# huangwenjie2023/LINR-PCGC

Measured on AMD Instinct MI355X. Metric: encode_sec_per_frame, lower is better.
Workload: dtype f32

## Files before the change

### include/linr_hip.h

```cpp
#ifndef LINR_HIP_H
#define LINR_HIP_H

#include <stddef.h>
#include <stdint.h>

#ifdef __cplusplus
extern "C" {
#endif

#define LINR_ABI_VERSION 13
#define LINR_API __attribute__((visibility("default")))

#define LINR_EINVAL   (-1)
#define LINR_ENOSPC   (-2)
#define LINR_EALIGN   (-3)

#define LINR_RELU      1u
#define LINR_ACCUM     2u
#define LINR_RELU_MASK 4u
#define LINR_NO_BIAS   8u
#define LINR_PAD_ROW  16u

LINR_API int linr_abi_version(void);
LINR_API int64_t linr_param_count(int32_t scale_num, int32_t block_layers);

LINR_API size_t linr_kmap_workspace_bytes(int64_t n);
LINR_API int linr_kmap_build(const int32_t* coords, int64_t n, int32_t* nbr, int64_t ld, int64_t row_base,
                    void* ws, size_t ws_bytes, void* stream);
LINR_API int linr_kmap_compress(const int32_t* nbr, int64_t nbr_ld, int64_t n, int32_t* lo, uint32_t* mask, int64_t ld,
                       void* stream);
LINR_API int linr_kmap_offset_feat(const int32_t* nbr, int64_t ld, int64_t row_base, int64_t n, float* out, void* stream);
LINR_API int linr_octree_occupancy(const int32_t* child, int64_t m, const int32_t* parent, int64_t n, float* occ, void* ws,
                          size_t ws_bytes, void* stream);
LINR_API size_t linr_sort_unique_workspace_bytes(int64_t n);
LINR_API int linr_coords_sort_unique(const int32_t* coords, int64_t n, const int32_t* origin, int32_t shift, int32_t coord_bits, int32_t* out,
                                     int64_t* count, void* ws, size_t ws_bytes, void* stream);
LINR_API int linr_coords_minmax(const int32_t* coords, int64_t n, int32_t* out, void* stream);
LINR_API int linr_octree_level(const int32_t* child, int64_t m, int32_t coord_bits, int32_t* parent, float* occ, int64_t* count, void* ws,
                               size_t ws_bytes, void* stream);
LINR_API int32_t linr_octree_levels_count(int32_t coord_bits, int32_t max_levels);
LINR_API int64_t linr_octree_levels_rows(int64_t m, int32_t coord_bits, int32_t max_levels);
LINR_API size_t linr_octree_levels_workspace_bytes(int64_t m, int32_t coord_bits, int32_t max_levels);
LINR_API int linr_octree_levels(const int32_t* child, int64_t m, const int64_t* m_dev, int32_t coord_bits, int32_t max_levels,
                                int32_t* parents, float* occ, int64_t* counts, void* ws, size_t ws_bytes, void* stream);
LINR_API int linr_kmap_validate(const int32_t* coords, int64_t n, int32_t* bad, void* stream);

LINR_API int linr_spconv_fwd(const float* in, int32_t in_ld, const int32_t* nbr, int64_t nbr_ld, int64_t n,
                    const float* W, const float* bias, int32_t cin, int32_t cout,
                    const float* res, int32_t res_ld, float* out, int32_t out_ld, uint32_t flags, void* stream);
LINR_API int linr_spconv_bwd_data(const float* gout, int32_t gout_ld, const int32_t* nbr, int64_t nbr_ld, int64_t n,
                         const float* W, int32_t cin, int32_t cout,
                         const float* act, int32_t act_ld, float* gin, int32_t gin_ld, uint32_t flags,
                         void* stream);
LINR_API size_t linr_spconv_bwd_weight_workspace_bytes(int64_t n, int32_t cin, int32_t cout);
LINR_API int linr_spconv_bwd_weight(const float* in, int32_t in_ld, const float* gout, int32_t gout_ld,
                           const int32_t* nbr, int64_t nbr_ld, int64_t n, int32_t cin, int32_t cout,
                           float* gW, float* gb, uint32_t flags, void* ws, size_t ws_bytes, void* stream);

LINR_API int linr_spconv_cmap(int32_t bwd, const float* in, int32_t in_ld, const int32_t* lo, const uint32_t* mask,
                     int64_t ld, int64_t n, const float* W, const float* bias, int32_t cin, int32_t cout,
                     const float* res, int32_t res_ld, const float* act, int32_t act_ld, float* out, int32_t out_ld,
                     uint32_t flags, void* stream);
LINR_API int linr_spconv_wide(int32_t bwd, const float* const* in_h, const int32_t* lo, const uint32_t* mask, int64_t ld, int64_t n,
                              const float* W, const float* bias, int32_t cin, int32_t cout, const float* const* res_h,
                              const float* const* act_h, float* const* out_h, uint32_t flags, void* stream);
typedef struct {
    int32_t mode;
    const float* W;
    const float* b;
    const float* const* aux_h;
    float* const* out2_h;
} linr_wide_pw;
LINR_API int linr_spconv_wide_pw(int32_t bwd, const float* const* in_h, const int32_t* lo, const uint32_t* mask, int64_t ld, int64_t n,
                                 const float* W, const float* bias, int32_t cin, int32_t cout, const float* const* res_h,
                                 const float* const* act_h, float* const* out_h, uint32_t flags, const linr_wide_pw* pw, void* stream);
LINR_API size_t linr_spconv_wgrad_wide_slab_bytes(int32_t cin, int32_t cout);
LINR_API int linr_spconv_wgrad_wide(const float* const* in_h, int32_t cin, const float* const* g_h, int32_t cout, const int32_t* nbr,
                                    const int32_t* tile8t, int64_t ld, int64_t n, float* slab, float* gW, float* gb, void* stream);

LINR_API int linr_linear_wide(const float* const* in_h, int32_t cin, int32_t in_blocked, const float* W, int32_t ws_ci, int32_t ws_co,
                              const float* bias, int32_t cout, int32_t out_blocked, const float* const* res_h, const float* const* act_h,
                              float* const* out_h, int64_t n, uint32_t flags, void* stream);
LINR_API size_t linr_linear_wgrad_wide_workspace_bytes(int64_t n, int32_t cin, int32_t cout);
LINR_API int linr_linear_wgrad_wide(const float* const* in_h, int32_t cin, int32_t in_blocked, const float* const* g_h, int32_t cout,
                                    int32_t g_blocked, int64_t n, float* gW, int32_t ws_ci, int32_t ws_co, float* gb, uint32_t flags,
                                    void* ws, size_t ws_bytes, void* stream);

typedef struct {
    int32_t kind, nblocks, cin, cout, ws_ci, ws_co;
    const float* slab;
    float* gW;
    float* gb;
} linr_wide_reduce;
LINR_API int32_t linr_spconv_wgrad_wide_blocks(int32_t cout, int32_t tiled);
LINR_API int linr_spconv_wgrad_wide2(const float* const* inA_h, const float* const* gA_h, const float* const* inB_h, const float* const* gB_h,
                                     int32_t h, const int32_t* tile8t, int64_t n, float* slab, void* stream);
LINR_API int32_t linr_linear_wgrad_wide_blocks(int64_t n);
LINR_API int linr_wide_reduce_many(const linr_wide_reduce* items_h, int32_t count, void* stream);

LINR_API size_t linr_head_wide_workspace_bytes(int64_t n);
LINR_API int linr_bits_finish(const double* partial, int64_t count, double* bits_acc, void* stream);
LINR_API int linr_head_wide_fwd(const float* const* c_h, int32_t C, const float* w1, const float* b1, const float* w2, const float* b2,
                                const float* target, int32_t target_ld, int64_t n, float* p, double* bits_acc, void* ws, size_t ws_bytes,
                                void* stream);
LINR_API size_t linr_head_wide_bwd_slab_bytes(int32_t C, int32_t nstages);
LINR_API int linr_head_wide_bwd(const float* const* c_h, const float* const* p_h, const float* const* target_h, int32_t target_ld,
                                const float* const* w1_h, const float* const* b1_h, const float* const* w2_h, int32_t C, int32_t nstages,
                                float gscale, float* const* gc_h, int64_t n, float* slab, size_t slab_bytes, float* grads, void* stream);

LINR_API int64_t linr_spconv_wgrad_cmap_blocks(void);
LINR_API int linr_spconv_wgrad_cmap(const float* in, int32_t in_ld, const float* gout, int32_t gout_ld, const int32_t* nbr,
                           const int32_t* tile8t, int64_t ld, int64_t n, int32_t cin, int32_t cout, float* slab, void* stream);
LINR_API int linr_slab_reduce(const float* slab, int32_t nblocks, int32_t elems, int32_t split, float* dstA, float* dstB,
                     uint32_t flags, void* stream);
LINR_API size_t linr_kmap_tile8t_bytes(int64_t n);
LINR_API int linr_kmap_tile8t(const int32_t* nbr, int64_t ld, int64_t n, int32_t* tile8t, size_t tile8t_bytes, void* stream);
LINR_API int linr_spconv_bwd_fused(const float* gout, const float* in, const int32_t* lo, const uint32_t* mask, int64_t ld,
                          int64_t n, const float* W, float* gin, float* slab, int32_t nblocks, void* stream);
#define LINR_PROF_KINDS 24
LINR_API int linr_prof_mask(uint32_t mask);
LINR_API int linr_debug_poison(uint32_t kind_mask);
LINR_API int linr_debug_poison_now(void* stream);
LINR_API int linr_prof_enable(int32_t mode);
LINR_API int linr_prof_read(int32_t kind, double* total_ms, int64_t* launches, int64_t* passes);

LINR_API int linr_linear_fwd(const float* in, int32_t in_ld, int64_t n, const float* W, int32_t ws_ci, int32_t ws_co,
                    const float* bias, int32_t cin, int32_t cout, const float* res, int32_t res_ld,
                    float* out, int32_t out_ld, uint32_t flags, void* stream);
LINR_API int linr_linear_bwd_data(const float* gout, int32_t gout_ld, int64_t n, const float* W, int32_t ws_ci,
                         int32_t ws_co, int32_t cin, int32_t cout, const float* act, int32_t act_ld,
                         float* gin, int32_t gin_ld, uint32_t flags, void* stream);
LINR_API size_t linr_linear_bwd_weight_workspace_bytes(int64_t n, int32_t cin, int32_t cout);
LINR_API int linr_linear_bwd_weight(const float* in, int32_t in_ld, const float* gout, int32_t gout_ld, int64_t n,
                           int32_t cin, int32_t cout, float* gW, int32_t ws_ci, int32_t ws_co, float* gb,
                           uint32_t flags, void* ws, size_t ws_bytes, void* stream);
LINR_API int linr_axpy(const float* src, int64_t n, float* dst, int32_t accumulate, void* stream);
LINR_API int linr_sum_many(const float* const* src_h, int32_t count, int64_t n, float* dst, int32_t accumulate, void* stream);

LINR_API size_t linr_bce_workspace_bytes(int64_t n);
LINR_API int linr_bce_bits_fwd(const float* z, const float* target, int32_t target_ld, int64_t n, float* p,
                      double* bits_acc, void* ws, size_t ws_bytes, void* stream);
LINR_API int linr_bce_bits_bwd(const float* p, const float* target, int32_t target_ld, int64_t n, float gscale,
                      float* gz, void* stream);

LINR_API int linr_adam_step(float* params, const float* grads, float* exp_avg, float* exp_avg_sq, int64_t n,
                   double step_size, double bc2_sqrt, double beta1, double beta2, double eps, double weight_decay,
                   void* stream);

#define LINR_FRAME_OCC_PADDED 1
typedef struct linr_frame {
    int64_t rows;
    int32_t n_scales;
    int32_t model_scale_num;
    int32_t block_layers;
    int32_t flags;
    const int64_t* row_off_h;
    const int32_t* scale_idx_h;
    const int32_t* nbr;
    int64_t nbr_ld;
    const int32_t* nbr_lo;
    const uint32_t* nbr_mask;
    const float*   offset_feat;
    const float*   occ;
    const int32_t* nbr8t;
} linr_frame;

LINR_API size_t linr_net_arena_bytes(int64_t rows, int32_t block_layers);
LINR_API int linr_net_forward(const linr_frame* f, const float* params, float* arena, size_t arena_bytes,
                     int32_t stage_begin, int32_t stage_end, float* probs, double* bits_acc, void* stream);
LINR_API int linr_net_backward(const linr_frame* f, const float* params, float* arena, size_t arena_bytes,
                      float gscale, float* grads, void* stream);

LINR_API int linr_net_train_step(const linr_frame* f, float* params, float* arena, size_t arena_bytes, float gscale,
                        float* exp_avg, float* exp_avg_sq, double lr, int64_t step, const int64_t* scale_steps_h,
                        double beta1, double beta2, double eps, double weight_decay, double* bits_acc, void* stream);

LINR_API size_t linr_net_bf16_arena_bytes(int64_t rows, int32_t block_layers);
LINR_API int linr_net_forward_bf16(const linr_frame* f, const uint8_t* codes, float min_param, float max_param, void* arena,
                          size_t arena_bytes, int32_t stage_begin, int32_t stage_end, float* probs, double* bits_acc,
                          void* stream);

LINR_API int64_t linr_wide_bf16_image_elems(int32_t cin, int32_t cout);
LINR_API int linr_wide_bf16_prep(const uint8_t* codes, int64_t n_params, float min_param, float max_param, const int64_t* conv_tab,
                                 int32_t n_conv, int64_t n_img, float* pf, void* img, void* stream);
LINR_API int linr_spconv_wide_bf16(int32_t epi, const uint16_t* in, int64_t in_bs, int32_t cin, const int32_t* lo, const uint32_t* mask,
                                   int64_t ld, int64_t n, const void* img, const float* bias, int32_t cout, const uint16_t* res, int64_t res_bs,
                                   const uint16_t* res2, int64_t res2_bs, const float* pw_w, const float* pw_b, int32_t relu, uint16_t* out,
                                   int64_t out_bs, void* stream);
LINR_API int linr_head_wide_bf16_fwd(const uint16_t* in, int64_t in_bs, int32_t C, const int32_t* lo, const uint32_t* mask, int64_t ld,
                                     int64_t n, const void* img, const float* bias, const float* w1, const float* b1, const float* w2,
                                     const float* b2, const float* target, int32_t t_col, float* p, double* partial, void* stream);
LINR_API int linr_sce_fwd_bf16(const float* pf, const linr_frame* f, uint16_t* x0_padded, void* stream);

LINR_API size_t linr_net_train_bf16_arena_bytes(int64_t rows, int32_t block_layers);
LINR_API int linr_occ_to_bf16(const float* occ, int64_t rows, uint16_t* out_padded, void* stream);
LINR_API int linr_net_forward_train_bf16(const linr_frame* f, const float* params, void* arena, size_t arena_bytes,
                                const uint16_t* occ_bf16, float* probs, double* bits_acc, void* stream);
LINR_API int linr_net_backward_bf16(const linr_frame* f, const float* params, void* arena, size_t arena_bytes,
                           const uint16_t* occ_bf16, float gscale, float* grads, void* stream);
LINR_API int linr_net_train_step_bf16(const linr_frame* f, float* params, void* arena, size_t arena_bytes, const uint16_t* occ_bf16,
                             float gscale, float* exp_avg, float* exp_avg_sq, double lr, int64_t step,
                             const int64_t* scale_steps_h, double beta1, double beta2, double eps, double weight_decay,
                             double* bits_acc, void* stream);
LINR_API int linr_spconv_bwd_fused_bf16(const uint16_t* gout, const uint16_t* in, const int32_t* lo, const uint32_t* mask, int64_t ld,
                               int64_t n, const float* W, uint16_t* gin, float* slab, int32_t nblocks, int32_t* rows_written,
                               void* stream);

LINR_API int linr_net_decode_stages(const linr_frame* f, const float* params, const uint8_t* codes, float min_param,
                           float max_param, void* arena, size_t arena_bytes, const uint8_t* const* streams_h,
                           const int64_t* stream_len_h, float* probs, float* p_pinned, uint8_t* s_pinned, uint8_t* s_dev,
                           void* stream);

LINR_API size_t linr_decode_scale_ws_bytes(int64_t n, int32_t block_layers, int32_t bf16);
LINR_API int linr_decode_scale(const int32_t* coord, int64_t n, int32_t scale_idx, int32_t model_scale_num, int32_t block_layers,
                      int32_t child_bits, const float* params, const uint8_t* codes, float min_param, float max_param,
                      const uint8_t* const* streams_h, const int64_t* stream_len_h, void* ws, size_t ws_bytes,
                      float* p_pinned, uint8_t* s_pinned, int32_t* child_xyz, int64_t child_cap, int64_t* child_n_h,
                      void* stream);

LINR_API int linr_sce_fwd(const float* params, const linr_frame* f, float* mix, float* hid, float* x0, void* stream);
LINR_API int linr_sce_bwd(const float* params, const linr_frame* f, const float* gx0, const float* hid, float* ghid,
                 void* stream);
LINR_API int64_t linr_sce_param_count(int32_t model_scale_num);
LINR_API size_t linr_sce_bwd_params_slab_bytes(int32_t model_scale_num);
LINR_API int linr_sce_bwd_params(const float* params, const linr_frame* f, const float* gx0, const float* hid, float* slab,
                                 size_t slab_bytes, float* grads, void* stream);

LINR_API size_t linr_head_workspace_bytes(int64_t n);
LINR_API int linr_head_fwd(const float* prior, const int32_t* lo, const uint32_t* mask, int64_t ld, int64_t n,
                  const float* Wp, const float* bp, const float* w1, const float* b1, const float* w2, const float* b2,
                  const float* target, int32_t target_ld, float* c_out, float* p_out, double* bits_acc, void* ws,
                  size_t ws_bytes, void* stream);
LINR_API int linr_head_bwd(const float* c, const float* p, const float* target, int32_t target_ld, const float* w1,
                  const float* b1, const float* w2, float gscale, float* gc, int64_t n, float* ghead, void* ws,
                  size_t ws_bytes, void* stream);

typedef struct linr_inception_params {
    const float *w00, *b00;
    const float *w01, *b01;
    const float *w10, *b10;
    const float *w11, *b11;
    const float *w12, *b12;
} linr_inception_params;
LINR_API int linr_inception_fwd(const float* x, const int32_t* lo, const uint32_t* mask, int64_t ld, int64_t n,
                       const linr_inception_params* q, float* H, float* M, float* I, void* stream);
LINR_API int linr_inception_bwd_data(const float* gI, const float* x, const float* H, const float* M, const int32_t* lo,
                            const uint32_t* mask, int64_t ld, int64_t n, const linr_inception_params* q, float* gM,
                            float* gH, float* gX, uint32_t flags, void* stream);
LINR_API int linr_spconv_wgrad_dual44(const float* H, const float* g0, int32_t g0_ld, const float* g1, int32_t g1_ld,
                             const int32_t* nbr, const int32_t* tile8t, int64_t ld, int64_t n, float* slab, void* stream);

LINR_API int linr_inception_bwd_fused(const float* gI, const float* gM, const float* x, const float* H, const int32_t* lo,
                             const uint32_t* mask, int64_t ld, int64_t n, const linr_inception_params* q, float* gH, float* gX,
                             uint32_t flags, float* slab, int32_t nblocks, void* stream);

LINR_API int linr_occ_wgrad7(const float* occ, const float* const* gout7_h, const int32_t* lo, const uint32_t* mask, int64_t ld,
                    int64_t n, float* slab, int32_t nblocks, int32_t* rows_written_h, void* stream);
LINR_API int linr_occ_conv7(const float* occ, const int32_t* lo, const uint32_t* mask, int64_t ld, int64_t n,
                   const float* params, const int64_t* w_off_h, const int64_t* b_off_h, float* out,
                   const int64_t* out_off_h, void* stream);

LINR_API int64_t linr_ac_encode_binary(const float* prob_h, const uint8_t* sym_h, int64_t n, uint8_t* out_h, int64_t cap);
LINR_API int     linr_ac_decode_binary(const float* prob_h, int64_t n, const uint8_t* in_h, int64_t in_len, uint8_t* sym_h);
LINR_API int64_t linr_ac_encode_cdf16(const uint16_t* cdf_h, int32_t lp, int32_t cdf_shared, const int16_t* sym_h,
                             int64_t n, uint8_t* out_h, int64_t cap);
LINR_API int     linr_ac_decode_cdf16(const uint16_t* cdf_h, int32_t lp, int32_t cdf_shared, int64_t n,
                             const uint8_t* in_h, int64_t in_len, int16_t* sym_h);
LINR_API int linr_ac_encode_binary_batch(const float* const* prob_h, const uint8_t* const* sym_h, const int64_t* n,
                                int32_t n_streams, uint8_t* const* out_h, const int64_t* cap,
                                int64_t* out_len, int32_t n_threads);

LINR_API int linr_ply_parse_ascii(const char* text_h, size_t len, int64_t n_rows, int32_t n_cols, int32_t cx, int32_t cy,
                         int32_t cz, int64_t* xyz_h, int64_t* rows_parsed_h);

#ifdef __cplusplus
}
#endif
#endif
```

### linr_pcgc_amd/_lib.py

```python
import ctypes
import os

import torch

_HERE = os.path.dirname(os.path.abspath(__file__))
LIB_PATH = os.environ.get('LINR_HIP_LIB') or os.path.join(_HERE, 'liblinr_hip.so')

LINR_RELU, LINR_ACCUM, LINR_RELU_MASK, LINR_NO_BIAS, LINR_PAD_ROW = 1, 2, 4, 8, 16
LINR_FRAME_OCC_PADDED = 1
ABI_VERSION = 13

c_i32, c_i64, c_u32, c_f32, c_f64 = ctypes.c_int32, ctypes.c_int64, ctypes.c_uint32, ctypes.c_float, ctypes.c_double
c_ptr, c_size = ctypes.c_void_p, ctypes.c_size_t


class LinrWidePw(ctypes.Structure):
    _fields_ = [('mode', ctypes.c_int32), ('W', ctypes.c_void_p), ('b', ctypes.c_void_p), ('aux_h', ctypes.c_void_p), ('out2_h', ctypes.c_void_p)]


class LinrWideReduce(ctypes.Structure):
    _fields_ = [('kind', ctypes.c_int32), ('nblocks', ctypes.c_int32), ('cin', ctypes.c_int32), ('cout', ctypes.c_int32),
                ('ws_ci', ctypes.c_int32), ('ws_co', ctypes.c_int32), ('slab', ctypes.c_void_p), ('gW', ctypes.c_void_p),
                ('gb', ctypes.c_void_p)]


class LinrFrame(ctypes.Structure):
    _fields_ = [('rows', c_i64), ('n_scales', c_i32), ('model_scale_num', c_i32), ('block_layers', c_i32),
                ('flags', c_i32), ('row_off_h', c_ptr),
                ('scale_idx_h', c_ptr), ('nbr', c_ptr), ('nbr_ld', c_i64), ('nbr_lo', c_ptr), ('nbr_mask', c_ptr),
                ('offset_feat', c_ptr), ('occ', c_ptr), ('nbr8t', c_ptr)]


class LinrInceptionParams(ctypes.Structure):
    _fields_ = [(n, ctypes.c_void_p) for n in ('w00', 'b00', 'w01', 'b01', 'w10', 'b10', 'w11', 'b11', 'w12', 'b12')]


_PROTOS = {
    'linr_abi_version': (ctypes.c_int, []),
    'linr_param_count': (c_i64, [c_i32, c_i32]),
    'linr_kmap_workspace_bytes': (c_size, [c_i64]),
    'linr_kmap_build': (ctypes.c_int, [c_ptr, c_i64, c_ptr, c_i64, c_i64, c_ptr, c_size, c_ptr]),
    'linr_kmap_validate': (ctypes.c_int, [c_ptr, c_i64, c_ptr, c_ptr]),
    'linr_spconv_wgrad_cmap_blocks': (ctypes.c_int64, []),
    'linr_spconv_wgrad_cmap': (ctypes.c_int, [c_ptr, c_i32, c_ptr, c_i32, c_ptr, c_ptr, c_i64, c_i64, c_i32, c_i32, c_ptr, c_ptr]),
    'linr_spconv_bwd_fused': (ctypes.c_int, [c_ptr, c_ptr, c_ptr, c_ptr, c_i64, c_i64, c_ptr, c_ptr, c_ptr, c_i32, c_ptr]),
    'linr_inception_bwd_fused': (ctypes.c_int, [c_ptr, c_ptr, c_ptr, c_ptr, c_ptr, c_ptr, c_i64, c_i64,
                                                ctypes.POINTER(LinrInceptionParams), c_ptr, c_ptr, c_u32, c_ptr, c_i32, c_ptr]),
    'linr_slab_reduce': (ctypes.c_int, [c_ptr, c_i32, c_i32, c_i32, c_ptr, c_ptr, c_u32, c_ptr]),
    'linr_axpy': (ctypes.c_int, [c_ptr, c_i64, c_ptr, c_i32, c_ptr]),
    'linr_sum_many': (ctypes.c_int, [c_ptr, c_i32, c_i64, c_ptr, c_i32, c_ptr]),
    'linr_occ_wgrad7': (ctypes.c_int, [c_ptr, c_ptr, c_ptr, c_ptr, c_i64, c_i64, c_ptr, c_i32, c_ptr, c_ptr]),
    'linr_kmap_tile8t_bytes': (c_size, [c_i64]),
    'linr_kmap_tile8t': (ctypes.c_int, [c_ptr, c_i64, c_i64, c_ptr, c_size, c_ptr]),
    'linr_prof_mask': (ctypes.c_int, [c_u32]),
    'linr_prof_enable': (ctypes.c_int, [c_i32]),
    'linr_debug_poison': (ctypes.c_int, [c_u32]),
    'linr_debug_poison_now': (ctypes.c_int, [c_ptr]),
    'linr_prof_read': (ctypes.c_int, [c_i32, c_ptr, c_ptr, c_ptr]),
    'linr_octree_occupancy': (ctypes.c_int, [c_ptr, c_i64, c_ptr, c_i64, c_ptr, c_ptr, ctypes.c_size_t, c_ptr]),
    'linr_sort_unique_workspace_bytes': (ctypes.c_size_t, [c_i64]),
    'linr_coords_sort_unique': (ctypes.c_int, [c_ptr, c_i64, c_ptr, c_i32, c_i32, c_ptr, c_ptr, c_ptr, ctypes.c_size_t, c_ptr]),
    'linr_coords_minmax': (ctypes.c_int, [c_ptr, c_i64, c_ptr, c_ptr]),
    'linr_octree_level': (ctypes.c_int, [c_ptr, c_i64, c_i32, c_ptr, c_ptr, c_ptr, c_ptr, ctypes.c_size_t, c_ptr]),
    'linr_octree_levels_count': (c_i32, [c_i32, c_i32]),
    'linr_octree_levels_rows': (c_i64, [c_i64, c_i32, c_i32]),
    'linr_octree_levels_workspace_bytes': (ctypes.c_size_t, [c_i64, c_i32, c_i32]),
    'linr_octree_levels': (ctypes.c_int, [c_ptr, c_i64, c_ptr, c_i32, c_i32, c_ptr, c_ptr, c_ptr, c_ptr, ctypes.c_size_t, c_ptr]),
    'linr_kmap_offset_feat': (ctypes.c_int, [c_ptr, c_i64, c_i64, c_i64, c_ptr, c_ptr]),
    'linr_kmap_compress': (ctypes.c_int, [c_ptr, c_i64, c_i64, c_ptr, c_ptr, c_i64, c_ptr]),
    'linr_spconv_fwd': (ctypes.c_int, [c_ptr, c_i32, c_ptr, c_i64, c_i64, c_ptr, c_ptr, c_i32, c_i32, c_ptr, c_i32,
                                       c_ptr, c_i32, c_u32, c_ptr]),
    'linr_spconv_bwd_data': (ctypes.c_int, [c_ptr, c_i32, c_ptr, c_i64, c_i64, c_ptr, c_i32, c_i32, c_ptr, c_i32,
                                            c_ptr, c_i32, c_u32, c_ptr]),
    'linr_spconv_wide': (ctypes.c_int, [c_i32, c_ptr, c_ptr, c_ptr, c_i64, c_i64, c_ptr, c_ptr, c_i32, c_i32, c_ptr, c_ptr, c_ptr, ctypes.c_uint32, c_ptr]),
    'linr_spconv_wgrad_wide_slab_bytes': (ctypes.c_size_t, [c_i32, c_i32]),
    'linr_spconv_wgrad_wide': (ctypes.c_int, [c_ptr, c_i32, c_ptr, c_i32, c_ptr, c_ptr, c_i64, c_i64, c_ptr, c_ptr, c_ptr, c_ptr]),
    'linr_linear_wide': (ctypes.c_int, [c_ptr, ctypes.c_int32, ctypes.c_int32, c_ptr, ctypes.c_int32, ctypes.c_int32, c_ptr, ctypes.c_int32,
                                        ctypes.c_int32, c_ptr, c_ptr, c_ptr, c_i64, ctypes.c_uint32, c_ptr]),
    'linr_spconv_wide_pw': (ctypes.c_int, [c_i32, c_ptr, c_ptr, c_ptr, c_i64, c_i64, c_ptr, c_ptr, c_i32, c_i32, c_ptr, c_ptr, c_ptr, c_u32,
                                           ctypes.POINTER(LinrWidePw), c_ptr]),
    'linr_spconv_wgrad_wide2': (ctypes.c_int, [c_ptr, c_ptr, c_ptr, c_ptr, c_i32, c_ptr, c_i64, c_ptr, c_ptr]),
    'linr_spconv_wgrad_wide_blocks': (ctypes.c_int32, [ctypes.c_int32, ctypes.c_int32]),
    'linr_linear_wgrad_wide_blocks': (ctypes.c_int32, [c_i64]),
    'linr_wide_reduce_many': (ctypes.c_int, [ctypes.POINTER(LinrWideReduce), ctypes.c_int32, c_ptr]),
    'linr_head_wide_workspace_bytes': (ctypes.c_size_t, [c_i64]),
    'linr_bits_finish': (ctypes.c_int, [c_ptr, c_i64, c_ptr, c_ptr]),
    'linr_head_wide_fwd': (ctypes.c_int, [c_ptr, ctypes.c_int32, c_ptr, c_ptr, c_ptr, c_ptr, c_ptr, ctypes.c_int32, c_i64, c_ptr, c_ptr, c_ptr,
                                          ctypes.c_size_t, c_ptr]),
    'linr_head_wide_bwd_slab_bytes': (ctypes.c_size_t, [ctypes.c_int32, ctypes.c_int32]),
    'linr_head_wide_bwd': (ctypes.c_int, [c_ptr, c_ptr, c_ptr, ctypes.c_int32, c_ptr, c_ptr, c_ptr, ctypes.c_int32, ctypes.c_int32,
                                          ctypes.c_float, c_ptr, c_i64, c_ptr, ctypes.c_size_t, c_ptr, c_ptr]),
    'linr_linear_wgrad_wide_workspace_bytes': (ctypes.c_size_t, [c_i64, ctypes.c_int32, ctypes.c_int32]),
    'linr_linear_wgrad_wide': (ctypes.c_int, [c_ptr, ctypes.c_int32, ctypes.c_int32, c_ptr, ctypes.c_int32, ctypes.c_int32, c_i64, c_ptr,
                                              ctypes.c_int32, ctypes.c_int32, c_ptr, ctypes.c_uint32, c_ptr, ctypes.c_size_t, c_ptr]),
    'linr_spconv_cmap': (ctypes.c_int, [c_i32, c_ptr, c_i32, c_ptr, c_ptr, c_i64, c_i64, c_ptr, c_ptr, c_i32, c_i32, c_ptr,
                                        c_i32, c_ptr, c_i32, c_ptr, c_i32, c_u32, c_ptr]),
    'linr_spconv_bwd_weight_workspace_bytes': (c_size, [c_i64, c_i32, c_i32]),
    'linr_spconv_bwd_weight': (ctypes.c_int, [c_ptr, c_i32, c_ptr, c_i32, c_ptr, c_i64, c_i64, c_i32, c_i32, c_ptr,
                                              c_ptr, c_u32, c_ptr, c_size, c_ptr]),
    'linr_linear_fwd': (ctypes.c_int, [c_ptr, c_i32, c_i64, c_ptr, c_i32, c_i32, c_ptr, c_i32, c_i32, c_ptr, c_i32,
                                       c_ptr, c_i32, c_u32, c_ptr]),
    'linr_linear_bwd_data': (ctypes.c_int, [c_ptr, c_i32, c_i64, c_ptr, c_i32, c_i32, c_i32, c_i32, c_ptr, c_i32,
                                            c_ptr, c_i32, c_u32, c_ptr]),
    'linr_linear_bwd_weight_workspace_bytes': (c_size, [c_i64, c_i32, c_i32]),
    'linr_linear_bwd_weight': (ctypes.c_int, [c_ptr, c_i32, c_ptr, c_i32, c_i64, c_i32, c_i32, c_ptr, c_i32, c_i32,
                                              c_ptr, c_u32, c_ptr, c_size, c_ptr]),
    'linr_bce_workspace_bytes': (c_size, [c_i64]),
    'linr_bce_bits_fwd': (ctypes.c_int, [c_ptr, c_ptr, c_i32, c_i64, c_ptr, c_ptr, c_ptr, c_size, c_ptr]),
    'linr_bce_bits_bwd': (ctypes.c_int, [c_ptr, c_ptr, c_i32, c_i64, c_f32, c_ptr, c_ptr]),
    'linr_adam_step': (ctypes.c_int, [c_ptr, c_ptr, c_ptr, c_ptr, c_i64, c_f64, c_f64, c_f64, c_f64, c_f64, c_f64,
                                      c_ptr]),
    'linr_net_arena_bytes': (c_size, [c_i64, c_i32]),
    'linr_net_forward': (ctypes.c_int, [ctypes.POINTER(LinrFrame), c_ptr, c_ptr, c_size, c_i32, c_i32, c_ptr, c_ptr,
                                        c_ptr]),
    'linr_net_backward': (ctypes.c_int, [ctypes.POINTER(LinrFrame), c_ptr, c_ptr, c_size, c_f32, c_ptr, c_ptr]),
    'linr_net_train_step': (ctypes.c_int, [ctypes.POINTER(LinrFrame), c_ptr, c_ptr, c_size, c_f32, c_ptr, c_ptr, c_f64,
                                           c_i64, c_ptr, c_f64, c_f64, c_f64, c_f64, c_ptr, c_ptr]),
    'linr_net_bf16_arena_bytes': (c_size, [c_i64, c_i32]),
    'linr_net_forward_bf16': (ctypes.c_int, [ctypes.POINTER(LinrFrame), c_ptr, c_f32, c_f32, c_ptr, c_size, c_i32, c_i32, c_ptr,
                                             c_ptr, c_ptr]),
    'linr_wide_bf16_image_elems': (ctypes.c_int64, [c_i32, c_i32]),
    'linr_wide_bf16_prep': (ctypes.c_int, [c_ptr, c_i64, c_f32, c_f32, c_ptr, c_i32, c_i64, c_ptr, c_ptr, c_ptr]),
    'linr_spconv_wide_bf16': (ctypes.c_int, [c_i32, c_ptr, c_i64, c_i32, c_ptr, c_ptr, c_i64, c_i64, c_ptr, c_ptr, c_i32, c_ptr, c_i64,
                                             c_ptr, c_i64, c_ptr, c_ptr, c_i32, c_ptr, c_i64, c_ptr]),
    'linr_head_wide_bf16_fwd': (ctypes.c_int, [c_ptr, c_i64, c_i32, c_ptr, c_ptr, c_i64, c_i64, c_ptr, c_ptr, c_ptr, c_ptr, c_ptr, c_ptr,
                                               c_ptr, c_i32, c_ptr, c_ptr, c_ptr]),
    'linr_sce_fwd_bf16': (ctypes.c_int, [c_ptr, ctypes.POINTER(LinrFrame), c_ptr, c_ptr]),
    'linr_net_train_bf16_arena_bytes': (c_size, [c_i64, c_i32]),
    'linr_occ_to_bf16': (ctypes.c_int, [c_ptr, c_i64, c_ptr, c_ptr]),
    'linr_net_forward_train_bf16': (ctypes.c_int, [ctypes.POINTER(LinrFrame), c_ptr, c_ptr, c_size, c_ptr, c_ptr, c_ptr, c_ptr]),
    'linr_net_backward_bf16': (ctypes.c_int, [ctypes.POINTER(LinrFrame), c_ptr, c_ptr, c_size, c_ptr, c_f32, c_ptr, c_ptr]),
    'linr_net_train_step_bf16': (ctypes.c_int, [ctypes.POINTER(LinrFrame), c_ptr, c_ptr, c_size, c_ptr, c_f32, c_ptr, c_ptr, c_f64,
                                                c_i64, c_ptr, c_f64, c_f64, c_f64, c_f64, c_ptr, c_ptr]),
    'linr_spconv_bwd_fused_bf16': (ctypes.c_int, [c_ptr, c_ptr, c_ptr, c_ptr, c_i64, c_i64, c_ptr, c_ptr, c_ptr, c_i32, c_ptr, c_ptr]),
    'linr_sce_fwd': (ctypes.c_int, [c_ptr, ctypes.POINTER(LinrFrame), c_ptr, c_ptr, c_ptr, c_ptr]),
    'linr_sce_bwd': (ctypes.c_int, [c_ptr, ctypes.POINTER(LinrFrame), c_ptr, c_ptr, c_ptr, c_ptr]),
    'linr_sce_param_count': (ctypes.c_int64, [ctypes.c_int32]),
    'linr_sce_bwd_params_slab_bytes': (ctypes.c_size_t, [ctypes.c_int32]),
    'linr_sce_bwd_params': (ctypes.c_int, [c_ptr, ctypes.POINTER(LinrFrame), c_ptr, c_ptr, c_ptr, ctypes.c_size_t, c_ptr, c_ptr]),
    'linr_head_workspace_bytes': (c_size, [c_i64]),
    'linr_head_fwd': (ctypes.c_int, [c_ptr, c_ptr, c_ptr, c_i64, c_i64, c_ptr, c_ptr, c_ptr, c_ptr, c_ptr, c_ptr, c_ptr, c_i32,
                                     c_ptr, c_ptr, c_ptr, c_ptr, c_size, c_ptr]),
    'linr_head_bwd': (ctypes.c_int, [c_ptr, c_ptr, c_ptr, c_i32, c_ptr, c_ptr, c_ptr, c_f32, c_ptr, c_i64, c_ptr, c_ptr, c_size,
                                     c_ptr]),
    'linr_inception_fwd': (ctypes.c_int, [c_ptr, c_ptr, c_ptr, c_i64, c_i64, ctypes.POINTER(LinrInceptionParams), c_ptr, c_ptr,
                                          c_ptr, c_ptr]),
    'linr_inception_bwd_data': (ctypes.c_int, [c_ptr, c_ptr, c_ptr, c_ptr, c_ptr, c_ptr, c_i64, c_i64,
                                               ctypes.POINTER(LinrInceptionParams), c_ptr, c_ptr, c_ptr, c_u32, c_ptr]),
    'linr_spconv_wgrad_dual44': (ctypes.c_int, [c_ptr, c_ptr, c_i32, c_ptr, c_i32, c_ptr, c_ptr, c_i64, c_i64, c_ptr, c_ptr]),
    'linr_occ_conv7': (ctypes.c_int, [c_ptr, c_ptr, c_ptr, c_i64, c_i64, c_ptr, c_ptr, c_ptr, c_ptr, c_ptr, c_ptr]),
    'linr_ac_encode_binary': (c_i64, [c_ptr, c_ptr, c_i64, c_ptr, c_i64]),
    'linr_ac_decode_binary': (ctypes.c_int, [c_ptr, c_i64, c_ptr, c_i64, c_ptr]),
    'linr_net_decode_stages': (ctypes.c_int, [ctypes.POINTER(LinrFrame), c_ptr, c_ptr, c_f32, c_f32, c_ptr, c_size, c_ptr, c_ptr, c_ptr,
                                              c_ptr, c_ptr, c_ptr, c_ptr]),
    'linr_decode_scale_ws_bytes': (c_size, [c_i64, c_i32, c_i32]),
    'linr_decode_scale': (ctypes.c_int, [c_ptr, c_i64, c_i32, c_i32, c_i32, c_i32, c_ptr, c_ptr, c_f32, c_f32, c_ptr, c_ptr, c_ptr, c_size,
                                         c_ptr, c_ptr, c_ptr, c_i64, c_ptr, c_ptr]),
    'linr_ac_encode_cdf16': (c_i64, [c_ptr, c_i32, c_i32, c_ptr, c_i64, c_ptr, c_i64]),
    'linr_ac_decode_cdf16': (ctypes.c_int, [c_ptr, c_i32, c_i32, c_i64, c_ptr, c_i64, c_ptr]),
    'linr_ply_parse_ascii': (ctypes.c_int, [c_ptr, c_size, c_i64, c_i32, c_i32, c_i32, c_i32, c_ptr, c_ptr]),
    'linr_ac_encode_binary_batch': (ctypes.c_int, [c_ptr, c_ptr, c_ptr, c_i32, c_ptr, c_ptr, c_ptr, c_i32]),
}

EXPORTS = tuple(_PROTOS)
_lib = None


class LinrError(RuntimeError):
    pass


def lib():
    global _lib
    if _lib is None:
        if not os.path.exists(LIB_PATH):
            raise LinrError('%s not found: build it with linr_pcgc_amd/csrc/build.sh (or __graft_entry__.build()); '
                            'there is no CPU / PyTorch fallback for the coding network' % LIB_PATH)
        handle = ctypes.CDLL(LIB_PATH)
        for name, (res, args) in _PROTOS.items():
            fn = getattr(handle, name)
            fn.restype, fn.argtypes = res, args
        if handle.linr_abi_version() != ABI_VERSION:
            raise LinrError('liblinr_hip.so ABI %d != binding ABI %d' % (handle.linr_abi_version(), ABI_VERSION))
        if os.environ.get('LINR_DEBUG_POISON'):
            handle = _Poisoned(handle)
        _lib = handle
    return _lib


class _Poisoned:
    _HOST = ('linr_ac_', 'linr_prof_', 'linr_debug_', 'linr_abi_version')

    def __init__(self, handle):
        self._h = handle
        handle.linr_debug_poison(0xFFFFFF)

    def __getattr__(self, name):
        fn = getattr(self._h, name)
        if name.startswith(self._HOST) or name.endswith('_bytes'):
            return fn
        h = self._h

        def call(*a):
            import torch
            if torch.cuda.is_available():
                h.linr_debug_poison_now(ctypes.c_void_p(torch.cuda.current_stream().cuda_stream))
            return fn(*a)
        return call


_ERR = {-1: 'LINR_EINVAL (bad argument)', -2: 'LINR_ENOSPC (buffer too small)', -3: 'LINR_EALIGN (misaligned pointer)'}


def check(rc, what):
    if rc != 0:
        raise LinrError('%s failed: %s' % (what, _ERR.get(rc, 'hipError_t %d' % rc)))


def scratch(nbytes, device):
    import torch
    t = torch.empty(int(nbytes), dtype=torch.uint8, device=device)
    if os.environ.get('LINR_DEBUG_POISON'):
        t.fill_(0xFF)
    return t


def current_stream_handle():
    try:
        return torch._C._cuda_getCurrentRawStream(torch._C._cuda_getDevice())
    except AttributeError:
        return torch.cuda.current_stream().cuda_stream
```

### linr_pcgc_amd/codec.py

```python
import glob
import json
import os

import numpy as np
import torch

from .function_utils import pack_bitstream, unpack_bitstream
from .model_codec import Model_Estimate
from .model_core import encode_streams
from .module_utils import octree_level_obj, qscTensor, unique_sorted

ARITH_VERSION = 2


def enc_all_frame_low_xyz(gop):
    chunks = []
    for low in gop.low_xyz:
        mx = int(low.max())
        if int(np.ceil(np.log2(mx + 1))) > 8:
            raise AssertionError('downsampled xyzQ should be less than 8 bit')
        chunks.append(low.cpu().numpy().astype(np.uint8).tobytes())
    chunks.append(np.asarray(gop.coord_mins, dtype=np.int32).reshape(-1).tobytes())
    return pack_bitstream(chunks)


def dec_all_frame_low_xyz(low_byte):
    chunks = unpack_bitstream(low_byte)
    mins = np.frombuffer(chunks.pop(), dtype=np.int32).reshape(-1, 3)
    return [np.frombuffer(c, dtype=np.uint8).reshape(-1, 3) for c in chunks], mins


EXTRA_SIDE_BITS = 40


def model_shape(model):
    return {'scale_num': int(model.scale_num), 'block_layers': int(model.block_layers), 'hidden_channel_conv': int(model.hidden)}


def encode_gop(model, model_ori, gop, bitdepth=8, n_threads=None, precision='f32'):
    if n_threads is None:
        n_threads = max(1, min(16, len(os.sched_getaffinity(0)) if hasattr(os, 'sched_getaffinity') else 8))
    comp = Model_Estimate().compress_model(model, bitdepth, True, model_ori)
    coded_model = comp['new_model']
    coded_model.inference_precision = precision
    side_info = {'mu': comp['mu'], 'b': comp['b'], 'min_param': comp['min_param'], 'max_param': comp['max_param'],
                 'enc_mode': comp['enc_mode'], 'bitdepth': bitdepth}
    if precision != 'f32':
        side_info['precision'] = precision
    side_info['arith_version'] = ARITH_VERSION
    side_info.update(model_shape(model))
    side_info['train_precision'] = getattr(model, 'train_precision', 'f32')
    from concurrent.futures import ThreadPoolExecutor
    workers = 2 if n_threads >= 4 else 1
    per_job = max(1, n_threads // workers)

    def code(p_host, occ_host, row_off, n_scales):
        ps, ss = [], []
        for i in range(n_scales):
            a, b = int(row_off[i]), int(row_off[i + 1])
            for k in range(8):
                ps.append(p_host[k, a:b])
                ss.append(occ_host[k, a:b])
        streams = encode_streams(ps, ss, per_job)
        return [pack_bitstream(streams[8 * i:8 * i + 8]) for i in range(n_scales)]

    RING = 4
    max_rows = max(f.rows for f in gop.frames)
    dev = gop.frames[0].device
    p_pin = [torch.empty(8 * max_rows, dtype=torch.float32, pin_memory=True) for _ in range(RING)]
    o_pin = [torch.empty(8 * max_rows, dtype=torch.uint8, pin_memory=True) for _ in range(RING)]
    copy_stream = torch.cuda.Stream(device=dev)
    jobs, bits_dev, pending = [], [], []

    def hand_over(entry, coder):
        slot, rows, f, keep, ev_c = entry
        ev_c.synchronize()
        p_host = p_pin[slot][:8 * rows].view(8, rows).numpy()
        occ_host = o_pin[slot][:8 * rows].view(8, rows).numpy()
        jobs.append(coder.submit(code, p_host, occ_host, f.row_off, f.n_scales))

    with ThreadPoolExecutor(max_workers=workers) as coder:
        for i, f in enumerate(gop.frames):
            slot = i % RING
            if i >= RING:
                jobs[i - RING].result()
            probs, bits = coded_model.frame_probs(f)
            bits_dev.append(bits)
            occ_t = f.occ.t().to(torch.uint8).contiguous()
            ev_f = torch.cuda.Event()
            ev_f.record()
            with torch.cuda.stream(copy_stream):
                copy_stream.wait_event(ev_f)
                p_pin[slot][:8 * f.rows].view(8, f.rows).copy_(probs, non_blocking=True)
                o_pin[slot][:8 * f.rows].view(8, f.rows).copy_(occ_t, non_blocking=True)
                ev_c = torch.cuda.Event()
                ev_c.record(copy_stream)
            pending.append((slot, f.rows, f, (probs, occ_t), ev_c))
            if len(pending) > 1:
                hand_over(pending.pop(0), coder)
        while pending:
            hand_over(pending.pop(0), coder)
        frames_bytes = [j.result() for j in jobs]
    bits_est = float(torch.stack(bits_dev).sum())
    low = enc_all_frame_low_xyz(gop)
    points = sum(gop.point_nums)
    occ_bits = 8 * sum(len(b) for fb in frames_bytes for b in fb)
    return {'frames': frames_bytes, 'model_bin': comp['final_bytes'], 'side_info': side_info, 'low_enc_bytes': low,
            'point_num': points, 'bits_est': bits_est,
            'bpp': {'point_bpp': occ_bits / points, 'model_bpp': (comp['bit_real'] + EXTRA_SIDE_BITS) / points,
                    'xyzlow_bpp': len(low) * 8 / points,
                    'bpp_all': (occ_bits + comp['bit_real'] + EXTRA_SIDE_BITS + len(low) * 8) / points}}


def decode_one_frame(model, frame_enc_bytes, xyz_low):
    if getattr(model, '_wide', None) is not None:
        return decode_one_frame_stagewise(model, frame_enc_bytes, xyz_low)
    lowx = unique_sorted(xyz_low)
    bits = max(1, int(xyz_low.max()).bit_length()) if xyz_low.numel() else 1
    for s_idx in range(len(frame_enc_bytes) - 1, -1, -1):
        bits = min(bits + 1, 21)
        lowx = model.decode_scale(lowx, s_idx, frame_enc_bytes[s_idx], bits)
    return {'dec_coord': lowx}


def decode_one_frame_stagewise(model, frame_enc_bytes, xyz_low):
    lowx = unique_sorted(xyz_low)
    for s_idx in range(len(frame_enc_bytes) - 1, -1, -1):
        occ_lst = model.decode({'enc_bytes': frame_enc_bytes[s_idx], 'coord': lowx, 'offset_tensor': None,
                                'scale_idx': s_idx})
        lowx = octree_level_obj.upper_layer(lowx, torch.cat(occ_lst, dim=-1))
    return {'dec_coord': lowx}


def decode_gop(model_ori, enc, device='cuda', frames=None, workers=1, timing=None):
    import time
    t_setup = time.time()
    side = dict(enc['side_info'])
    coded_with = int(side.pop('arith_version', 1))
    if coded_with != ARITH_VERSION:
        from ._lib import LinrError
        raise LinrError('this stream was coded with network arithmetic version %d; this build decodes version %d (the fp32 '
                        'accumulation order of the convolutions is part of the stream format: decode with the build that '
                        'encoded it)' % (coded_with, ARITH_VERSION))
    want = {k: side[k] for k in ('scale_num', 'block_layers', 'hidden_channel_conv') if k in side}
    have = model_shape(model_ori)
    if any(int(v) != have[k] for k, v in want.items()):
        raise ValueError('the stream was coded with a model of shape %s; the model handed to the decoder has %s' % (want, have))
    side['final_bytes'] = enc['model_bin']
    model, _ = Model_Estimate().decompress_model(model_ori, side)
    model.inference_precision = side.get('precision', 'f32')
    lows, mins = dec_all_frame_low_xyz(enc['low_enc_bytes'])
    todo = list(range(len(enc['frames'])) if frames is None else frames)
    if timing is not None:
        if device != 'cpu':
            torch.cuda.synchronize()
        timing['setup_s'] = time.time() - t_setup

    def one(i):
        xyz_low = torch.tensor(lows[i].astype(np.int32), device=device)
        dec = decode_one_frame(model, list(enc['frames'][i]), xyz_low)['dec_coord']
        return dec + torch.tensor(mins[i], device=device, dtype=torch.int32)

    if getattr(model, '_wide', None) is not None:
        workers = 1
    if workers <= 1 or len(todo) <= 1:
        return [one(i) for i in todo]
    from concurrent.futures import ThreadPoolExecutor
    main_stream = torch.cuda.current_stream()
    dev_index = torch.cuda.current_device()

    def job(i):
        torch.cuda.set_device(dev_index)
        st = torch.cuda.Stream()
        st.wait_stream(main_stream)
        with torch.cuda.stream(st):
            out = one(i)
        st.synchronize()
        return out

    with ThreadPoolExecutor(max_workers=workers) as pool:
        return list(pool.map(job, todo))


def write_gop(enc, result_dir):
    bins = os.path.join(result_dir, 'bins')
    os.makedirs(bins, exist_ok=True)
    for fi, scales in enumerate(enc['frames']):
        for si, b in enumerate(scales):
            with open(os.path.join(bins, 'frame%s_scale%d.bin' % (str(fi).zfill(4), si)), 'wb') as f:
                f.write(b)
    with open(os.path.join(bins, 'model.bin'), 'wb') as f:
        f.write(enc['model_bin'])
    with open(os.path.join(bins, 'low_enc_bytes.bin'), 'wb') as f:
        f.write(enc['low_enc_bytes'])
    with open(os.path.join(result_dir, 'side_info.json'), 'w') as f:
        json.dump(enc['side_info'], f, indent=4)


def read_gop(result_dir):
    bins = os.path.join(result_dir, 'bins')
    frames, fi = [], 0
    while True:
        files = glob.glob(os.path.join(bins, 'frame%s_scale*.bin' % str(fi).zfill(4)))
        if not files:
            break
        scales = []
        for si in range(len(files)):
            with open(os.path.join(bins, 'frame%s_scale%d.bin' % (str(fi).zfill(4), si)), 'rb') as f:
                scales.append(f.read())
        frames.append(scales)
        fi += 1
    with open(os.path.join(bins, 'model.bin'), 'rb') as f:
        model_bin = f.read()
    with open(os.path.join(bins, 'low_enc_bytes.bin'), 'rb') as f:
        low = f.read()
    with open(os.path.join(result_dir, 'side_info.json')) as f:
        side = json.load(f)
    return {'frames': frames, 'model_bin': model_bin, 'low_enc_bytes': low, 'side_info': side}
```

### linr_pcgc_amd/csrc/ac.cpp

```cpp
#include <cmath>
#include <cstdint>
#include <cstring>
#include <thread>
#include <vector>
#include <atomic>
#if defined(__SSE2__)
#include <emmintrin.h>
#endif
#include "../../include/linr_hip.h"

namespace {

struct BitSink {
    uint8_t* out; int64_t cap; int64_t len = 0; uint32_t acc = 0; int nacc = 0;
    BitSink(uint8_t* o, int64_t c) : out(o), cap(c) {}
    inline void put(uint32_t bit) {
        acc = (acc << 1) | bit;
        if (++nacc == 8) { if (len < cap) out[len] = (uint8_t)acc; ++len; acc = 0; nacc = 0; }
    }
    inline void put_with_pending(uint32_t bit, uint64_t& pending) {
        put(bit);
        for (; pending > 0; --pending) put(bit ^ 1u);
    }
    inline void finish() { while (nacc != 0) put(0); }
};

struct RangeEncoder {
    uint32_t low = 0, high = 0xFFFFFFFFu; uint64_t pending = 0; BitSink sink;
    RangeEncoder(uint8_t* o, int64_t c) : sink(o, c) {}
    inline void encode(uint32_t c_low, uint32_t c_high) {
        const uint64_t span = (uint64_t)high - (uint64_t)low + 1;
        high = (low - 1) + (uint32_t)((span * c_high) >> 16);
        low = low + (uint32_t)((span * c_low) >> 16);
        for (;;) {
            if (high < 0x80000000u) {
                sink.put_with_pending(0, pending);
            } else if (low >= 0x80000000u) {
                sink.put_with_pending(1, pending);
            } else if (low >= 0x40000000u && high < 0xC0000000u) {
                ++pending;
                low = (low << 1) & 0x7FFFFFFFu;
                high = (high << 1) | 0x80000001u;
                continue;
            } else {
                break;
            }
            low <<= 1;
            high = (high << 1) | 1u;
        }
    }
    inline int64_t finish() {
        ++pending;
        sink.put_with_pending(low < 0x40000000u ? 0u : 1u, pending);
        sink.finish();
        return sink.len;
    }
};

struct BitSource {
    const uint8_t* in; int64_t len; int64_t pos = 0; uint64_t buf = 0; int nbuf = 0;
    BitSource(const uint8_t* i, int64_t l) : in(i), len(l) {}
    inline uint32_t bits(int n) {
        while (nbuf <= 56) {
            const uint64_t byte = pos < len ? in[pos] : 0u;
            ++pos;
            buf |= byte << (56 - nbuf);
            nbuf += 8;
        }
        const uint32_t v = (uint32_t)(buf >> (64 - n));
        buf <<= n;
        nbuf -= n;
        return v;
    }
};

struct RangeDecoder {
    uint32_t low = 0, high = 0xFFFFFFFFu, value = 0; BitSource src;
    RangeDecoder(const uint8_t* i, int64_t l) : src(i, l) { value = src.bits(32); }
    inline uint32_t target() const {
        const uint64_t span = (uint64_t)high - (uint64_t)low + 1;
        return (uint32_t)(uint16_t)((((uint64_t)value - (uint64_t)low + 1) * 0x10000u - 1) / span);
    }
    inline void consume(uint32_t c_low, uint32_t c_high) {
        const uint64_t span = (uint64_t)high - (uint64_t)low + 1;
        high = (low - 1) + (uint32_t)((span * c_high) >> 16);
        low = low + (uint32_t)((span * c_low) >> 16);
        for (;;) {
            const uint32_t diff = low ^ high;
            if (diff < 0x80000000u) {
                int n = diff ? __builtin_clz(diff) : 31;
                if (n > 31) n = 31;
                low <<= n;
                high = (high << n) | ((1u << n) - 1u);
                value = (value << n) | src.bits(n);
            } else if (low >= 0x40000000u && high < 0xC0000000u) {
                low = (low << 1) & 0x7FFFFFFFu;
                high = (high << 1) | 0x80000001u;
                value -= 0x40000000u;
                value = (value << 1) | src.bits(1);
            } else {
                break;
            }
        }
    }
};

inline uint32_t binary_c1(float p) {
    const long scaled = lrintf((1.0f - p) * 65534.0f);
    return (uint32_t)((scaled + 1) & 0xFFFF);
}

}

namespace {

struct BitSinkFast {
    uint8_t* out; int64_t cap; int64_t len = 0; uint64_t acc = 0; int nacc = 0;
    BitSinkFast(uint8_t* o, int64_t c) : out(o), cap(c) {}
    inline void put_bits(uint32_t v, int n) {
        acc = (acc << n) | v;
        nacc += n;
        while (nacc >= 8) {
            nacc -= 8;
            if (len < cap) out[len] = (uint8_t)(acc >> nacc);
            ++len;
        }
    }
    inline void put_run(uint32_t bit, uint64_t count) {
        const uint32_t word = bit ? 0xFFFFFFFFu : 0u;
        while (count >= 32) { put_bits(word, 32); count -= 32; }
        if (count) put_bits(word >> (32 - (int)count), (int)count);
    }
    inline void finish() { if (nacc) put_bits(0, 8 - nacc); }
};

constexpr int AC_CHUNK = 256;

inline void c1_block(const float* p, int n, uint32_t* c1) {
    int i = 0;
#if defined(__SSE2__)
    const __m128 one = _mm_set1_ps(1.0f), scale = _mm_set1_ps(65534.0f);
    const __m128i inc = _mm_set1_epi32(1), m16 = _mm_set1_epi32(0xFFFF);
    for (; i + 4 <= n; i += 4) {
        const __m128i v = _mm_cvtps_epi32(_mm_mul_ps(_mm_sub_ps(one, _mm_loadu_ps(p + i)), scale));
        _mm_storeu_si128(reinterpret_cast<__m128i*>(c1 + i), _mm_and_si128(_mm_add_epi32(v, inc), m16));
    }
#endif
    for (; i < n; ++i) c1[i] = binary_c1(p[i]);
}

}

extern "C" int64_t linr_ac_encode_binary(const float* prob_h, const uint8_t* sym_h, int64_t n, uint8_t* out_h, int64_t cap) {
    if (n < 0 || cap < 0 || (n > 0 && (!prob_h || !sym_h)) || (cap > 0 && !out_h)) return LINR_EINVAL;
    BitSinkFast sink(out_h, cap);
    uint32_t low = 0, high = 0xFFFFFFFFu;
    uint64_t pending = 0;
    uint32_t c1[AC_CHUNK];
    for (int64_t base = 0; base < n; base += AC_CHUNK) {
        const int m = (int)(n - base < AC_CHUNK ? n - base : AC_CHUNK);
        c1_block(prob_h + base, m, c1);
        for (int i = 0; i < m; ++i) {
            const uint64_t span = (uint64_t)high - (uint64_t)low + 1;
            const uint32_t t = (uint32_t)((span * c1[i]) >> 16);
            const uint32_t one = sym_h[base + i] ? 0xFFFFFFFFu : 0u;
            const uint32_t lt = low + t;
            high = (high & one) | ((lt - 1u) & ~one);
            low = (lt & one) | (low & ~one);
            for (;;) {
                const uint32_t diff = low ^ high;
                if (diff < 0x80000000u) {
                    int k = diff ? __builtin_clz(diff) : 31;
                    if (k > 31) k = 31;
                    const uint32_t first = low >> 31;
                    if (pending) {
                        sink.put_bits(first, 1);
                        sink.put_run(first ^ 1u, pending);
                        pending = 0;
                        if (k > 1) sink.put_bits((low << 1) >> (33 - k), k - 1);
                    } else {
                        sink.put_bits(low >> (32 - k), k);
                    }
                    low <<= k;
                    high = (high << k) | ((1u << k) - 1u);
                } else if (low >= 0x40000000u && high < 0xC0000000u) {
                    ++pending;
                    low = (low << 1) & 0x7FFFFFFFu;
                    high = (high << 1) | 0x80000001u;
                } else {
                    break;
                }
            }
        }
    }
    ++pending;
    const uint32_t last = low < 0x40000000u ? 0u : 1u;
    sink.put_bits(last, 1);
    sink.put_run(last ^ 1u, pending);
    sink.finish();
    return sink.len <= cap ? sink.len : (int64_t)LINR_ENOSPC;
}

namespace {

struct BitWindow {
    const uint8_t* in; int64_t len; int64_t pos = 0; uint64_t buf = 0; int nbuf = 0;
    BitWindow(const uint8_t* i, int64_t l) : in(i), len(l) {}
    inline void refill() {
        if (__builtin_expect(pos + 8 <= len, 1)) {
            uint64_t w;
            std::memcpy(&w, in + pos, 8);
            buf |= __builtin_bswap64(w) >> nbuf;
            pos += (63 - nbuf) >> 3;
            nbuf |= 56;
        } else {
            while (nbuf <= 56) {
                const uint64_t byte = pos < len ? in[pos] : 0u;
                ++pos;
                buf |= byte << (56 - nbuf);
                nbuf += 8;
            }
        }
    }
    inline uint32_t take(int n) {
        const uint32_t v = (uint32_t)((buf >> 1) >> (63 - n));
        buf <<= n;
        nbuf -= n;
        return v;
    }
};

}

extern "C" int linr_ac_decode_binary(const float* prob_h, int64_t n, const uint8_t* in_h, int64_t in_len, uint8_t* sym_h) {
    if (n < 0 || in_len < 0 || (n > 0 && (!prob_h || !sym_h)) || (in_len > 0 && !in_h)) return LINR_EINVAL;
    BitWindow src(in_h, in_len);
    src.refill();
    uint32_t low = 0, high = 0xFFFFFFFFu, value = src.take(32);
    uint32_t c1[AC_CHUNK];
    for (int64_t base = 0; base < n; base += AC_CHUNK) {
        const int m = (int)(n - base < AC_CHUNK ? n - base : AC_CHUNK);
        c1_block(prob_h + base, m, c1);
        for (int i = 0; i < m; ++i) {
            const uint64_t span = (uint64_t)high - (uint64_t)low + 1;
            const uint32_t t = (uint32_t)((span * c1[i]) >> 16);
            const uint32_t s = (value - low >= t) ? 1u : 0u;
            sym_h[base + i] = (uint8_t)s;
            if (base + i == n - 1) break;
            const uint32_t one = 0u - s;
            const uint32_t lt = low + t;
            high = (high & one) | ((lt - 1u) & ~one);
            low = (lt & one) | (low & ~one);
            while (__builtin_expect((((low ^ high) ^ 0x80000000u) | ((low & ~high) << 1)) & 0x80000000u, 0)) {
                if (src.nbuf < 32) src.refill();
                const uint32_t diff = low ^ high;
                int k = __builtin_clz(diff | 1u);
                low <<= k;
                high = (high << k) | ((1u << k) - 1u);
                value = (value << k) | src.take(k);
                if (src.nbuf < 32) src.refill();
                const int j = __builtin_clz(~((low & ~high) << 1));
                low = (low << j) & 0x7FFFFFFFu;
                high = (high << j) | 0x80000000u | ((1u << j) - 1u);
                value = ((value << j) | src.take(j)) ^ (j ? 0x80000000u : 0u);
            }
        }
    }
    return 0;
}

extern "C" int64_t linr_ac_encode_cdf16(const uint16_t* cdf_h, int32_t lp, int32_t cdf_shared, const int16_t* sym_h,
                                        int64_t n, uint8_t* out_h, int64_t cap) {
    if (n < 0 || cap < 0 || lp < 2 || (n > 0 && (!cdf_h || !sym_h)) || (cap > 0 && !out_h)) return LINR_EINVAL;
    RangeEncoder enc(out_h, cap);
    const int max_symbol = lp - 2;
    for (int64_t i = 0; i < n; ++i) {
        const uint16_t* row = cdf_shared ? cdf_h : cdf_h + i * (int64_t)lp;
        const int s = sym_h[i];
        if (s < 0 || s > max_symbol) return LINR_EINVAL;
        enc.encode(row[s], s == max_symbol ? 0x10000u : (uint32_t)row[s + 1]);
    }
    const int64_t len = enc.finish();
    return len <= cap ? len : (int64_t)LINR_ENOSPC;
}

extern "C" int linr_ac_decode_cdf16(const uint16_t* cdf_h, int32_t lp, int32_t cdf_shared, int64_t n, const uint8_t* in_h,
                                    int64_t in_len, int16_t* sym_h) {
    if (n < 0 || in_len < 0 || lp < 2 || (n > 0 && (!cdf_h || !sym_h)) || (in_len > 0 && !in_h)) return LINR_EINVAL;
    RangeDecoder dec(in_h, in_len);
    const int max_symbol = lp - 2;
    for (int64_t i = 0; i < n; ++i) {
        const uint16_t* row = cdf_shared ? cdf_h : cdf_h + i * (int64_t)lp;
        const uint16_t t = (uint16_t)dec.target();
        int left = 0, right = max_symbol + 1;
        while (left + 1 < right) {
            const int m = (left + right) / 2;
            const uint16_t v = row[m];
            if (v < t) left = m; else if (v > t) right = m; else { left = m; break; }
        }
        sym_h[i] = (int16_t)left;
        if (i == n - 1) break;
        dec.consume(row[left], left == max_symbol ? 0x10000u : (uint32_t)row[left + 1]);
    }
    return 0;
}

extern "C" int linr_ac_encode_binary_batch(const float* const* prob_h, const uint8_t* const* sym_h, const int64_t* n,
                                           int32_t n_streams, uint8_t* const* out_h, const int64_t* cap, int64_t* out_len,
                                           int32_t n_threads) {
    if (n_streams < 0 || (n_streams > 0 && (!prob_h || !sym_h || !n || !out_h || !cap || !out_len))) return LINR_EINVAL;
    if (n_threads < 1) n_threads = 1;
    if (n_threads > n_streams) n_threads = n_streams;
    std::atomic<int> next(0);
    std::atomic<int> err(0);
    auto work = [&]() {
        for (;;) {
            const int i = next.fetch_add(1);
            if (i >= n_streams) return;
            const int64_t r = linr_ac_encode_binary(prob_h[i], sym_h[i], n[i], out_h[i], cap[i]);
            out_len[i] = r;
            if (r < 0) err.store((int)r);
        }
    };
    if (n_threads <= 1) {
        work();
    } else {
        std::vector<std::thread> pool;
        for (int t = 0; t < n_threads; ++t) pool.emplace_back(work);
        for (auto& t : pool) t.join();
    }
    return err.load();
}
```

### linr_pcgc_amd/csrc/common.h

```cpp
#pragma once
#include <hip/hip_runtime.h>
#include <stdint.h>
#include "../../include/linr_hip.h"

#define LINR_BLOCK 256
#define LINR_WAVE 64

static inline int linr_hip_rc(hipError_t e) { return e == hipSuccess ? 0 : (int)e; }
static inline int linr_launch_rc() { return linr_hip_rc(hipGetLastError()); }
#define LINR_TAP(kk) (((kk) / 9) + 3 * (((kk) / 3) % 3) + 9 * ((kk) % 3))

static inline bool linr_aligned16(const void* p) { return (((uintptr_t)p) & 15u) == 0; }
static inline bool linr_rows_fit32(int64_t n, int64_t row_bytes = 32) { return n < ((int64_t)1 << 32) / row_bytes - 1; }
static inline bool linr_cmap_fits32(int64_t ld) { return ld < ((int64_t)1 << 26); }
static inline unsigned linr_grid(int64_t n, int per_block) { return (unsigned)((n + per_block - 1) / per_block); }

static inline int linr_reduce_blocks(int64_t n, int rows_per_tile) {
    int64_t tiles = (n + rows_per_tile - 1) / rows_per_tile;
    int64_t nb = tiles < 512 ? tiles : 512;
    return (int)(nb < 1 ? 1 : nb);
}

struct LinrWgradDst {
    float* base;
    int64_t block_stride;
    int64_t w_off;
    int64_t b_off;
    int cin_valid;
};
struct LinrLinDst {
    float* base;
    int64_t block_stride;
    int64_t w_off;
    int ws_ci, ws_co;
    int64_t b_off;
};
struct LinrAdamRanges {
    int count;
    int64_t begin, len;
    int active[16];
    float step_size[16], bc2_sqrt[16];
};
__device__ __forceinline__ float linr_adam_update(float p, float grad, float& m, float& v, float step_size, float bc2_sqrt, float beta1,
                                                  float omb1, float beta2, float omb2, float eps, float wd) {
#pragma clang fp contract(off)
    const float g = fmaf(wd, p, grad);
    const float mi = m * beta1 + omb1 * g;
    const float vi = v * beta2 + (omb2 * g) * g;
    m = mi;
    v = vi;
    const float denom = sqrtf(vi) / bc2_sqrt + eps;
    return fmaf(-step_size, mi / denom, p);
}
__attribute__((visibility("hidden")))
int linr_adam_launch(float* params, const float* grads, float* exp_avg, float* exp_avg_sq, int64_t n, double step_size,
                     double bc2_sqrt, double beta1, double beta2, double eps, double weight_decay,
                     const LinrAdamRanges* rg, hipStream_t s);
#define LINR_WG_BLOCKS 512

#define LINR_MAXG 8
struct Grp {
    int64_t in[LINR_MAXG], w[LINR_MAXG], b[LINR_MAXG], res[LINR_MAXG], act[LINR_MAXG], out[LINR_MAXG];
    int64_t e0[LINR_MAXG], e1[LINR_MAXG], e2[LINR_MAXG], e3[LINR_MAXG], e4[LINR_MAXG], e5[LINR_MAXG], e6[LINR_MAXG];
    int64_t n[LINR_MAXG];
};

struct LinrCmap { const int32_t* lo; const uint32_t* mask; int64_t ld, n; };

struct ConvGroup {
    const float *in, *W, *bias, *res, *act;
    float* out;
};
struct HeadFwdGroup {
    const float *in, *W, *bias;
    float* c_out;
    const float *w1, *b1, *w2, *b2;
    const float* target;
    float* p_out;
    double* partial;
};
struct HeadBwdGroup {
    const float *c, *p, *target, *w1, *b1, *w2;
    float* gc;
    int64_t w1_off, b1_off, w2_off, b2_off;
};
struct ConvPwGroup {
    const float *A, *w00, *b00, *w10, *b10;
    float* H;
};
struct Dual44FwdGroup {
    const float *H, *w01, *b01, *w11, *b11, *A, *w12, *b12;
    float *M, *I;
};
struct Dual44BwdGroup {
    const float *gI, *gM, *H, *w01, *w11;
    float* gH;
    int64_t w01_off, b01_off, w11_off, b11_off;
};
struct Conv88BwdGroup {
    const float *g, *xin, *W;
    float* out;
    int64_t w_off, b_off;
    const float *w12, *M;
    float* gM;
    int64_t w12_off, b12_off;
};
struct Conv84BwdGroup {
    const float *gH, *A, *gI, *w00, *w10;
    float* gA;
    int64_t w00_off, b00_off, w10_off, b10_off;
};
struct WgradGroup {
    const float *in, *gout;
    int64_t w_off, b_off;
    int cin_live;
};

__attribute__((visibility("hidden")))
int linr_conv3_launch(bool bwd, const float* in, int in_ld, const int32_t* nbr, int64_t nbr_ld, int64_t n,
                      const float* W, const float* bias, int cin, int cout, const float* res, int res_ld,
                      const float* act, int act_ld, float* out, int out_ld, unsigned flags, hipStream_t s);
__attribute__((visibility("hidden")))
int linr_linear_launch(const float* in, int in_ld, int64_t n, const float* W, int ws_ci, int ws_co, const float* bias,
                       int cin, int cout, const float* res, int res_ld, const float* act, int act_ld, float* out,
                       int out_ld, unsigned flags, hipStream_t s);
__attribute__((visibility("hidden")))
int linr_conv3_wgrad_partial(const float* in, int in_ld, const float* gout, int gout_ld, const int32_t* nbr,
                             int64_t nbr_ld, int64_t n, int cin, int cout, LinrWgradDst d, int nblocks, unsigned flags,
                             hipStream_t s);
__attribute__((visibility("hidden")))
int linr_linear_wgrad_partial(const WgradGroup* g, int ng, int in_ld, int gout_ld, int64_t n, int cin, int cout, float* big,
                              int64_t block_stride, int ws_ci, int ws_co, int nblocks, hipStream_t s);
__attribute__((visibility("hidden"))) int linr_lin_blocks(int64_t n);
__attribute__((visibility("hidden")))
int linr_linear_slab_reduce_launch(const float* slab, int nblocks, int64_t stride, int cin, int cout, float* gW, int ws_ci, int ws_co,
                                   float* gb, unsigned flags, hipStream_t s);
__attribute__((visibility("hidden")))
int linr_cconv_launch(bool bwd, LinrCmap m, const ConvGroup* g, int ng, int in_ld, int cin, int cout, int res_ld, int act_ld,
                      int out_ld, unsigned flags, hipStream_t s);
__attribute__((visibility("hidden")))
int linr_cconv_head_launch(LinrCmap m, const HeadFwdGroup* g, int ng, int target_ld, hipStream_t s);
__attribute__((visibility("hidden")))
int linr_head_bwd_launch(const HeadBwdGroup* g, int ng, int target_ld, float gscale, int64_t n, float* big, int64_t block_stride,
                         int nblocks, int* rows_written, hipStream_t s);
__attribute__((visibility("hidden")))
int linr_slab_reduce_launch(const float* big, int nblocks, int64_t total, float* gsum, hipStream_t s);
__attribute__((visibility("hidden")))
int linr_bits_finish_launch(const double* partial, int count, double* bits_acc, hipStream_t s);
__attribute__((visibility("hidden")))
int linr_dual44_fwd_launch(LinrCmap m, const Dual44FwdGroup* g, int ng, hipStream_t s);
__attribute__((visibility("hidden")))
int linr_dual44_bwd_launch(LinrCmap m, const Dual44BwdGroup* g, int ng, hipStream_t s);
__attribute__((visibility("hidden")))
int linr_conv_pw_fwd_launch(LinrCmap m, const ConvPwGroup* g, int ng, hipStream_t s);
__attribute__((visibility("hidden")))
int linr_conv_bwd_gm_launch(LinrCmap m, const Conv88BwdGroup* g, int ng, hipStream_t s);
__attribute__((visibility("hidden")))
int linr_conv_bwd_ga_launch(LinrCmap m, const Conv84BwdGroup* g, int ng, unsigned flags, hipStream_t s);
__attribute__((visibility("hidden")))
int linr_occ_conv7_launch(const float* occ, LinrCmap m, const float* P, const int64_t* w_off, const int64_t* b_off, float* out,
                          const int64_t* out_off, hipStream_t s);
__attribute__((visibility("hidden")))
int linr_conv3_wgrad_mfma(const WgradGroup* g, int ng, int in_ld, int gout_ld, const int32_t* nbr, int64_t nbr_ld, int64_t n,
                          const int32_t* tile8t, int cin, int cout, float* big, int64_t block_stride, int nblocks, hipStream_t s);
__attribute__((visibility("hidden")))
int linr_fused_bwd_rows(int64_t n, int nb, int ngroups);
__attribute__((visibility("hidden")))
int linr_conv88_bwd_wgrad_launch(LinrCmap m, const Conv88BwdGroup* g, int ng, float* big, int64_t block_stride, int nb,
                                 int* rows_written, hipStream_t s);
__attribute__((visibility("hidden")))
int linr_dual44_bwd_wgrad_launch(LinrCmap m, const Dual44BwdGroup* g, int ng, float* big, int64_t block_stride, int nb,
                                 int* rows_written, hipStream_t s);
__attribute__((visibility("hidden")))
int linr_conv84_bwd_wgrad_launch(LinrCmap m, const Conv84BwdGroup* g, int ng, unsigned flags, float* big, int64_t block_stride,
                                 int nb, int* rows_written, hipStream_t s);
__attribute__((visibility("hidden")))
int linr_conv3_wgrad_dual44(const Dual44BwdGroup* g, int ng, int gI_ld, int gM_ld, const int32_t* nbr, int64_t nbr_ld, int64_t n,
                            const int32_t* tile8t, float* big, int64_t block_stride, int nblocks, hipStream_t s);

__attribute__((visibility("hidden"))) void linr_poison_hook(hipStream_t s, int kind);
__attribute__((visibility("hidden")))
int linr_occ_wgrad7_launch(const float* occ, const float* const* g, LinrCmap m, float* big, int64_t block_stride,
                           const int64_t* w_off, const int64_t* b_off, int nb, hipStream_t s, int* rows_written);
```

### linr_pcgc_amd/csrc/fused.hip

```cpp
#include "common.h"
#include "conv_common.h"
#include "head_bwd.h"
#define WG_WAVES 4

__global__ __launch_bounds__(LINR_BLOCK) void kmap_compress_k(const int32_t* __restrict__ nbr, int64_t nbr_ld, int64_t n,
                                                              int32_t* __restrict__ lo, uint32_t* __restrict__ mask,
                                                              int64_t ld) {
    const int64_t row = (int64_t)blockIdx.x * LINR_BLOCK + threadIdx.x;
    if (row >= n) return;
    uint32_t m = 0;
#pragma unroll
    for (int q = 0; q < 9; ++q) {
        const int32_t a = nbr[(int64_t)q * nbr_ld + row];
        const int32_t b = nbr[(int64_t)(q + 9) * nbr_ld + row];
        const int32_t c = nbr[(int64_t)(q + 18) * nbr_ld + row];
        const uint32_t m3 = (a >= 0 ? 1u : 0u) | (b >= 0 ? 2u : 0u) | (c >= 0 ? 4u : 0u);
        lo[(int64_t)q * ld + row] = a >= 0 ? a : (b >= 0 ? b : (c >= 0 ? c : 0));
        m |= m3 << (3 * q);
    }
    mask[row] = m;
}

extern "C" int linr_kmap_compress(const int32_t* nbr, int64_t nbr_ld, int64_t n, int32_t* lo, uint32_t* mask, int64_t ld,
                                  void* stream) {
    if (n < 0 || nbr_ld < n || ld < n) return LINR_EINVAL;
    if (n == 0) return 0;
    if (!nbr || !lo || !mask) return LINR_EINVAL;
    kmap_compress_k<<<linr_grid(n, LINR_BLOCK), LINR_BLOCK, 0, (hipStream_t)stream>>>(nbr, nbr_ld, n, lo, mask, ld);
    return linr_launch_rc();
}

struct HeadArgs {
    const float* w1;
    const float* b1;
    const float* w2;
    const float* b2;
    const float* target;
    int target_ld;
    float* p_out;
    double* partial;
};

#ifndef LINR_CONV_BLOCK
#define LINR_CONV_BLOCK 256
#endif
template <int GIN, int GOUT, bool BWD, int LOADW, int EPI = 0>
__global__ __launch_bounds__(LINR_CONV_BLOCK) void cconv_mfma_k(const float* __restrict__ in, int in_ld,
                                                           const int32_t* __restrict__ lo, const uint32_t* __restrict__ mask,
                                                           int64_t ld, int64_t n, const float* __restrict__ W,
                                                           const float* __restrict__ bias, const float* __restrict__ res,
                                                           int res_ld, const float* __restrict__ act, int act_ld,
                                                           float* __restrict__ out, int out_ld, unsigned flags,
                                                           HeadArgs hd = HeadArgs(), PwArgs pw = PwArgs(), Grp gp = Grp()) {
    static_assert(GOUT == 4 || GOUT == 8, "output channels must fill 1 or 2 MFMA blocks");
    {
        const int gi = blockIdx.y;
        in += gp.in[gi]; W += gp.w[gi]; out += gp.out[gi];
        if (bias) bias += gp.b[gi];
        if (res) res += gp.res[gi];
        if (act) act += gp.act[gi];
        if constexpr (EPI == 1) {
            hd.w1 += gp.e0[gi]; hd.b1 += gp.e1[gi]; hd.w2 += gp.e2[gi]; hd.b2 += gp.e3[gi];
            if (hd.target) hd.target += gp.e4[gi];
            hd.p_out += gp.e5[gi];
            if (hd.partial) hd.partial += gp.e6[gi];
        }
        if constexpr (EPI == 2) { pw.w += gp.e0[gi]; pw.b += gp.e1[gi]; }
        if constexpr (EPI == 3) { pw.w += gp.e0[gi]; pw.aux += gp.e1[gi]; pw.aux_out += gp.e2[gi]; }
        if constexpr (EPI == 4) { pw.w += gp.e0[gi]; pw.aux += gp.e1[gi]; }
    }
    constexpr int HB = GOUT / 4;
    constexpr int KPV = 16 / HB;
    constexpr int NG = (27 + KPV - 1) / KPV;
    const int lane = threadIdx.x & 63;
    float wv[NG][GIN];
    {
        const int blk = lane >> 2, j = lane & 3;
        const int kl = blk / HB, co = 4 * (blk % HB) + j;
#pragma unroll
        for (int g = 0; g < NG; ++g) {
            const int k = g * KPV + kl;
#pragma unroll
            for (int i = 0; i < GIN; ++i)
                wv[g][i] = (k < 27) ? (BWD ? W[(k * GOUT + co) * GIN + i] : W[(k * GIN + i) * GOUT + co]) : 0.0f;
        }
    }
    const int64_t row_raw = (int64_t)blockIdx.x * LINR_CONV_BLOCK + threadIdx.x;
    const bool live = row_raw < n;
    const int64_t row = live ? row_raw : n - 1;
    const char* pad = reinterpret_cast<const char*>(in - in_ld);
    const uint32_t rowbytes = (uint32_t)in_ld * 4u;
    uint32_t off[27];
    decode_offsets<BWD>(lo, mask, ld, row, rowbytes, off);
    f32x4 acc[GOUT / 4];
#pragma unroll
    for (int h = 0; h < GOUT / 4; ++h)
#pragma unroll
        for (int j = 0; j < 4; ++j) acc[h][j] = (bias != nullptr) ? bias[4 * h + j] : 0.0f;
    constexpr int PF = 4;
    float x[PF + 1][LOADW];
#pragma unroll
    for (int u = 0; u < PF; ++u) RowLoadF<LOADW>::run(pad + off[LINR_TAP(u)], x[u]);
    __builtin_amdgcn_sched_barrier(0);
    static_for<27>([&](auto kc) {
        constexpr int kk = decltype(kc)::value;
        constexpr int k = LINR_TAP(kk);
        constexpr int g = k / KPV, ab = (k % KPV) * HB;
        if constexpr (kk + PF < 27) RowLoadF<LOADW>::run(pad + off[LINR_TAP(kk + PF)], x[(kk + PF) % (PF + 1)]);
        __builtin_amdgcn_sched_barrier(0);
#pragma unroll
        for (int i = 0; i < GIN; ++i) {
            acc[0] = __builtin_amdgcn_mfma_f32_4x4x1f32(wv[g][i], x[kk % (PF + 1)][i], acc[0], 4, ab, 0);
            if constexpr (GOUT == 8)
                acc[1] = __builtin_amdgcn_mfma_f32_4x4x1f32(wv[g][i], x[kk % (PF + 1)][i], acc[1], 4, ab + 1, 0);
        }
        __builtin_amdgcn_sched_barrier(0);
    });
    float a[GOUT];
#pragma unroll
    for (int h = 0; h < GOUT / 4; ++h)
#pragma unroll
        for (int j = 0; j < 4; ++j) a[4 * h + j] = acc[h][j];
    if constexpr (EPI == 1) {
        float* op = out + row * out_ld;
        if (live) {
            *reinterpret_cast<float4*>(op) = make_float4(a[0], a[1], a[2], a[3]);
            *reinterpret_cast<float4*>(op + 4) = make_float4(a[4], a[5], a[6], a[7]);
        }
        float z = hd.b2[0];
#pragma unroll
        for (int j = 0; j < 24; ++j) {
            float hj = hd.b1[j];
#pragma unroll
            for (int i = 0; i < 8; ++i) hj = fmaf(a[i], hd.w1[j * 8 + i], hj);
            z = fmaf(fmaxf(hj, 0.0f), hd.w2[j], z);
        }
        const float p = 1.0f / (1.0f + expf(-z));
        if (live) hd.p_out[row] = p;
        if (hd.partial != nullptr) {
            __shared__ double sred[LINR_CONV_BLOCK / 64];
            double nats = 0.0;
            if (live) {
                const float t = hd.target[row * hd.target_ld];
                nats = (double)((t - 1.0f) * fmaxf(logf(1.0f - p), -100.0f) - t * fmaxf(logf(p), -100.0f));
            }
#pragma unroll
            for (int d = 32; d > 0; d >>= 1) nats += __shfl_xor(nats, d, 64);
            if (lane == 0) sred[threadIdx.x >> 6] = nats;
            __syncthreads();
            if (threadIdx.x == 0) {
                double tot = sred[0];
                for (int w = 1; w < LINR_CONV_BLOCK / 64; ++w) tot += sred[w];
                hd.partial[blockIdx.x] = tot;
            }
        }
        return;
    } else {
    if (!live) return;
    if (res != nullptr) {
        const float* r = res + row * res_ld;
#pragma unroll
        for (int o = 0; o < GOUT; ++o) a[o] += r[o];
    }
    float* op = out + row * out_ld;
    if (flags & LINR_ACCUM) {
#pragma unroll
        for (int o = 0; o < GOUT; ++o) a[o] += op[o];
    }
    if constexpr (EPI == 4) {
        const float4 g4 = *reinterpret_cast<const float4*>(pw.aux + row * 8 + 4);
        const float g[4] = {g4.x, g4.y, g4.z, g4.w};
#pragma unroll
        for (int i = 0; i < 8; ++i) {
            float t = 0.0f;
#pragma unroll
            for (int o = 0; o < 4; ++o) t = fmaf(g[o], pw.w[i * 4 + o], t);
            a[i] += t;
        }
    }
    if constexpr (EPI == 3) {
        const float4 m4 = *reinterpret_cast<const float4*>(pw.aux + row * 4);
        const float mv[4] = {m4.x, m4.y, m4.z, m4.w};
        float gm[4];
#pragma unroll
        for (int i = 0; i < 4; ++i) {
            float t = 0.0f;
#pragma unroll
            for (int o = 0; o < 4; ++o) t = fmaf(a[4 + o], pw.w[i * 4 + o], t);
            gm[i] = mv[i] > 0.0f ? t : 0.0f;
        }
        *reinterpret_cast<float4*>(pw.aux_out + row * 4) = make_float4(gm[0], gm[1], gm[2], gm[3]);
    }
    if constexpr (EPI == 2) {
        const char* self = reinterpret_cast<const char*>(in) + (uint32_t)row * ((uint32_t)in_ld * 4u);
        float xc[8];
        RowLoadF<8>::run(self, xc);
        float h1[4];
#pragma unroll
        for (int o = 0; o < 4; ++o) h1[o] = pw.b[o];
#pragma unroll
        for (int i = 0; i < 8; ++i)
#pragma unroll
            for (int o = 0; o < 4; ++o) h1[o] = fmaf(xc[i], pw.w[i * 4 + o], h1[o]);
        *reinterpret_cast<float4*>(op) = make_float4(fmaxf(a[0], 0.0f), fmaxf(a[1], 0.0f), fmaxf(a[2], 0.0f), fmaxf(a[3], 0.0f));
        *reinterpret_cast<float4*>(op + 4) = make_float4(fmaxf(h1[0], 0.0f), fmaxf(h1[1], 0.0f), fmaxf(h1[2], 0.0f), fmaxf(h1[3], 0.0f));
        return;
    }
    if (flags & LINR_RELU_MASK) {
        const float* m = act + row * act_ld;
#pragma unroll
        for (int o = 0; o < GOUT; ++o) a[o] = m[o] > 0.0f ? a[o] : 0.0f;
    }
    if (flags & LINR_RELU) {
#pragma unroll
        for (int o = 0; o < GOUT; ++o) a[o] = fmaxf(a[o], 0.0f);
    }
    if (out_ld % 4 == 0) {
#pragma unroll
        for (int v = 0; v < GOUT / 4; ++v)
            *reinterpret_cast<float4*>(op + 4 * v) = make_float4(a[4 * v], a[4 * v + 1], a[4 * v + 2], a[4 * v + 3]);
    } else {
#pragma unroll
        for (int o = 0; o < GOUT; ++o) op[o] = a[o];
    }
    }
}

extern "C" int linr_spconv_cmap(int32_t bwd, const float* in, int32_t in_ld, const int32_t* lo, const uint32_t* mask, int64_t ld,
                                int64_t n, const float* W, const float* bias, int32_t cin, int32_t cout, const float* res,
                                int32_t res_ld, const float* act, int32_t act_ld, float* out, int32_t out_ld, uint32_t flags,
                                void* stream) {
    if (n < 0 || ld < n || (in_ld != 4 && in_ld != 8)) return LINR_EINVAL;
    if (n == 0) return 0;
    if (!in || !lo || !mask || !W || !out) return LINR_EINVAL;
    if (!linr_aligned16(in) || !linr_aligned16(out)) return LINR_EALIGN;
    const int gin = bwd ? cout : cin, gout = bwd ? cin : cout;
    if (in_ld < gin || out_ld < gout || (gout != 4 && gout != 8)) return LINR_EINVAL;
    if ((flags & LINR_RELU_MASK) && (!act || act_ld < gout)) return LINR_EINVAL;
    if (res && res_ld < gout) return LINR_EINVAL;
    if (!linr_rows_fit32(n, 4 * in_ld)) return LINR_EINVAL;
    const ConvGroup g = {in, W, bias, res, act, out};
    return linr_cconv_launch(bwd != 0, {lo, mask, ld, n}, &g, 1, in_ld, cin, cout, res_ld, act_ld, out_ld, flags, (hipStream_t)stream);
}

extern "C" int64_t linr_spconv_wgrad_cmap_blocks(void) { return LINR_WG_BLOCKS; }

extern "C" int linr_spconv_wgrad_cmap(const float* in, int32_t in_ld, const float* gout, int32_t gout_ld, const int32_t* nbr,
                                      const int32_t* tile8t, int64_t ld, int64_t n, int32_t cin, int32_t cout, float* slab,
                                      void* stream) {
    if (n < 0 || ld < n || in_ld != 8 || gout_ld < cout) return LINR_EINVAL;
    if (n == 0) return 0;
    if (!in || !gout || !nbr || !slab) return LINR_EINVAL;
    if (!linr_aligned16(in)) return LINR_EALIGN;
    if (!((cin == 8 && (cout == 8 || cout == 4)) || (cin < 8 && cin >= 1 && cout == 8))) return LINR_EINVAL;
    if (!linr_rows_fit32(n)) return LINR_EINVAL;
    const int64_t elems = (int64_t)(27 * cin + 1) * cout;
    if (tile8t && !linr_aligned16(tile8t)) return LINR_EALIGN;
    const WgradGroup g = {in, gout, 0, (int64_t)27 * cin * cout, 0};
    return linr_conv3_wgrad_mfma(&g, 1, in_ld, gout_ld, nbr, ld, n, tile8t, cin, cout, slab, elems, LINR_WG_BLOCKS, (hipStream_t)stream);
}

int linr_cconv_head_launch(LinrCmap m, const HeadFwdGroup* g, int ng, int target_ld, hipStream_t s) {
    if (ng < 1 || ng > LINR_MAXG) return LINR_EINVAL;
    if (m.n == 0) return 0;
    Grp gp = Grp();
    for (int i = 0; i < ng; ++i) {
        gp.in[i] = g[i].in - g[0].in; gp.w[i] = g[i].W - g[0].W; gp.b[i] = g[i].bias - g[0].bias; gp.out[i] = g[i].c_out - g[0].c_out;
        gp.e0[i] = g[i].w1 - g[0].w1; gp.e1[i] = g[i].b1 - g[0].b1; gp.e2[i] = g[i].w2 - g[0].w2; gp.e3[i] = g[i].b2 - g[0].b2;
        gp.e4[i] = g[i].target - g[0].target; gp.e5[i] = g[i].p_out - g[0].p_out; gp.e6[i] = g[i].partial - g[0].partial;
    }
    HeadArgs hd = {g[0].w1, g[0].b1, g[0].w2, g[0].b2, g[0].target, target_ld, g[0].p_out, g[0].partial};
    cconv_mfma_k<8, 8, false, 8, 1><<<dim3(linr_grid(m.n, LINR_CONV_BLOCK), ng), LINR_CONV_BLOCK, 0, s>>>(
        g[0].in, 8, m.lo, m.mask, m.ld, m.n, g[0].W, g[0].bias, nullptr, 0, nullptr, 0, g[0].c_out, 8, 0, hd, PwArgs(), gp);
    return linr_launch_rc();
}

struct DualArgs {
    const float* in2; int in2_ld;
    const float* w01; const float* w11;
    const float* b01; const float* b11;
    const float* a_res;
    const float* w12; const float* b12;
    float* m_out;
    const float* act;
};

template <bool BWD>
__global__ __launch_bounds__(LINR_BLOCK) void cconv_dual44_k(const float* __restrict__ in, int in_ld,
                                                             const int32_t* __restrict__ lo, const uint32_t* __restrict__ mask,
                                                             int64_t ld, int64_t n, DualArgs d, float* __restrict__ out,
                                                             Grp gp = Grp()) {
    {
        const int gi = blockIdx.y;
        in += gp.in[gi]; out += gp.out[gi];
        if (d.in2) d.in2 += gp.e0[gi];
        d.w01 += gp.w[gi]; d.w11 += gp.e1[gi];
        if (d.b01) d.b01 += gp.b[gi];
        if (d.b11) d.b11 += gp.e2[gi];
        if (d.a_res) d.a_res += gp.res[gi];
        if (d.w12) d.w12 += gp.e3[gi];
        if (d.b12) d.b12 += gp.e4[gi];
        if (d.m_out) d.m_out += gp.e5[gi];
        if (d.act) d.act += gp.act[gi];
    }
    const int lane = threadIdx.x & 63;
    float wv[4][4];
    {
        const int blk = lane >> 2, j = lane & 3;
        const int kl = blk >> 1;
        const float* Wsel = (blk & 1) ? d.w11 : d.w01;
#pragma unroll
        for (int g = 0; g < 4; ++g) {
            const int k = g * 8 + kl;
#pragma unroll
            for (int i = 0; i < 4; ++i) wv[g][i] = (k < 27) ? (BWD ? Wsel[(k * 4 + j) * 4 + i] : Wsel[(k * 4 + i) * 4 + j]) : 0.0f;
        }
    }
    const int64_t row_raw = (int64_t)blockIdx.x * LINR_BLOCK + threadIdx.x;
    const bool live = row_raw < n;
    const int64_t row = live ? row_raw : n - 1;
    uint32_t off[27];
    decode_offsets<BWD>(lo, mask, ld, row, 1u, off);
    const char* pad0 = reinterpret_cast<const char*>(in - in_ld);
    const uint32_t rb0 = __builtin_amdgcn_readfirstlane(in_ld == 8 ? 5u : 4u);
    const char* pad1 = BWD ? reinterpret_cast<const char*>(d.in2 - d.in2_ld) : pad0 + 16;
    const uint32_t rb1 = BWD ? __builtin_amdgcn_readfirstlane(d.in2_ld == 8 ? 5u : 4u) : rb0;
    f32x4 acc0, acc1;
#pragma unroll
    for (int j = 0; j < 4; ++j) { acc0[j] = BWD ? 0.0f : d.b01[j]; acc1[j] = BWD ? 0.0f : d.b11[j]; }
    constexpr int PF = 3;
    float x0[PF + 1][4], x1[PF + 1][4];
#pragma unroll
    for (int u = 0; u < PF; ++u) {
        RowLoadF<4>::run(pad0 + (off[LINR_TAP(u)] << rb0), x0[u]);
        RowLoadF<4>::run(pad1 + (off[LINR_TAP(u)] << rb1), x1[u]);
    }
    __builtin_amdgcn_sched_barrier(0);
    static_for<27>([&](auto kc) {
        constexpr int kk = decltype(kc)::value;
        constexpr int k = LINR_TAP(kk);
        constexpr int g = k / 8, ab = (k % 8) * 2;
        if constexpr (kk + PF < 27) {
            RowLoadF<4>::run(pad0 + (off[LINR_TAP(kk + PF)] << rb0), x0[(kk + PF) % (PF + 1)]);
            RowLoadF<4>::run(pad1 + (off[LINR_TAP(kk + PF)] << rb1), x1[(kk + PF) % (PF + 1)]);
        }
        __builtin_amdgcn_sched_barrier(0);
#pragma unroll
        for (int i = 0; i < 4; ++i) {
            acc0 = __builtin_amdgcn_mfma_f32_4x4x1f32(wv[g][i], x0[kk % (PF + 1)][i], acc0, 4, ab, 0);
            acc1 = __builtin_amdgcn_mfma_f32_4x4x1f32(wv[g][i], x1[kk % (PF + 1)][i], acc1, 4, ab + 1, 0);
        }
        __builtin_amdgcn_sched_barrier(0);
    });
    if (!live) return;
    float* op = out + row * 8;
    if (BWD) {
        const float4 h0 = *reinterpret_cast<const float4*>(d.act + row * 8);
        const float4 h1 = *reinterpret_cast<const float4*>(d.act + row * 8 + 4);
        *reinterpret_cast<float4*>(op) = make_float4(h0.x > 0.0f ? acc0[0] : 0.0f, h0.y > 0.0f ? acc0[1] : 0.0f,
                                                     h0.z > 0.0f ? acc0[2] : 0.0f, h0.w > 0.0f ? acc0[3] : 0.0f);
        *reinterpret_cast<float4*>(op + 4) = make_float4(h1.x > 0.0f ? acc1[0] : 0.0f, h1.y > 0.0f ? acc1[1] : 0.0f,
                                                         h1.z > 0.0f ? acc1[2] : 0.0f, h1.w > 0.0f ? acc1[3] : 0.0f);
    } else {
        const float4 a0 = *reinterpret_cast<const float4*>(d.a_res + row * 8);
        const float4 a1 = *reinterpret_cast<const float4*>(d.a_res + row * 8 + 4);
        const float m[4] = {fmaxf(acc1[0], 0.0f), fmaxf(acc1[1], 0.0f), fmaxf(acc1[2], 0.0f), fmaxf(acc1[3], 0.0f)};
        *reinterpret_cast<float4*>(d.m_out + row * 4) = make_float4(m[0], m[1], m[2], m[3]);
        float i1[4];
#pragma unroll
        for (int o = 0; o < 4; ++o) i1[o] = d.b12[o];
#pragma unroll
        for (int i = 0; i < 4; ++i)
#pragma unroll
            for (int o = 0; o < 4; ++o) i1[o] = fmaf(m[i], d.w12[i * 4 + o], i1[o]);
        *reinterpret_cast<float4*>(op) = make_float4(acc0[0] + a0.x, acc0[1] + a0.y, acc0[2] + a0.z, acc0[3] + a0.w);
        *reinterpret_cast<float4*>(op + 4) = make_float4(i1[0] + a1.x, i1[1] + a1.y, i1[2] + a1.z, i1[3] + a1.w);
    }
}

int linr_dual44_fwd_launch(LinrCmap m, const Dual44FwdGroup* g, int ng, hipStream_t s) {
    if (ng < 1 || ng > LINR_MAXG) return LINR_EINVAL;
    if (m.n == 0) return 0;
    Grp gp = Grp();
    for (int i = 0; i < ng; ++i) {
        gp.in[i] = g[i].H - g[0].H; gp.w[i] = g[i].w01 - g[0].w01; gp.b[i] = g[i].b01 - g[0].b01; gp.e1[i] = g[i].w11 - g[0].w11;
        gp.e2[i] = g[i].b11 - g[0].b11; gp.res[i] = g[i].A - g[0].A; gp.e3[i] = g[i].w12 - g[0].w12; gp.e4[i] = g[i].b12 - g[0].b12;
        gp.e5[i] = g[i].M - g[0].M; gp.out[i] = g[i].I - g[0].I;
    }
    DualArgs d = {nullptr, 0, g[0].w01, g[0].w11, g[0].b01, g[0].b11, g[0].A, g[0].w12, g[0].b12, g[0].M, nullptr};
    cconv_dual44_k<false><<<dim3(linr_grid(m.n, LINR_BLOCK), ng), LINR_BLOCK, 0, s>>>(g[0].H, 8, m.lo, m.mask, m.ld, m.n, d, g[0].I, gp);
    return linr_launch_rc();
}

int linr_dual44_bwd_launch(LinrCmap m, const Dual44BwdGroup* g, int ng, hipStream_t s) {
    if (ng < 1 || ng > LINR_MAXG) return LINR_EINVAL;
    if (m.n == 0) return 0;
    Grp gp = Grp();
    for (int i = 0; i < ng; ++i) {
        gp.in[i] = g[i].gI - g[0].gI; gp.e0[i] = g[i].gM - g[0].gM; gp.w[i] = g[i].w01 - g[0].w01; gp.e1[i] = g[i].w11 - g[0].w11;
        gp.act[i] = g[i].H - g[0].H; gp.out[i] = g[i].gH - g[0].gH;
    }
    DualArgs d = {g[0].gM, 4, g[0].w01, g[0].w11, nullptr, nullptr, nullptr, nullptr, nullptr, nullptr, g[0].H};
    cconv_dual44_k<true><<<dim3(linr_grid(m.n, LINR_BLOCK), ng), LINR_BLOCK, 0, s>>>(g[0].gI, 8, m.lo, m.mask, m.ld, m.n, d, g[0].gH, gp);
    return linr_launch_rc();
}

int linr_conv_pw_fwd_launch(LinrCmap m, const ConvPwGroup* g, int ng, hipStream_t s) {
    if (ng < 1 || ng > LINR_MAXG) return LINR_EINVAL;
    if (m.n == 0) return 0;
    Grp gp = Grp();
    for (int i = 0; i < ng; ++i) {
        gp.in[i] = g[i].A - g[0].A; gp.w[i] = g[i].w00 - g[0].w00; gp.b[i] = g[i].b00 - g[0].b00; gp.out[i] = g[i].H - g[0].H;
        gp.e0[i] = g[i].w10 - g[0].w10; gp.e1[i] = g[i].b10 - g[0].b10;
    }
    PwArgs pw = {g[0].w10, g[0].b10, nullptr, nullptr};
    cconv_mfma_k<8, 4, false, 8, 2><<<dim3(linr_grid(m.n, LINR_CONV_BLOCK), ng), LINR_CONV_BLOCK, 0, s>>>(
        g[0].A, 8, m.lo, m.mask, m.ld, m.n, g[0].w00, g[0].b00, nullptr, 0, nullptr, 0, g[0].H, 8, 0, HeadArgs(), pw, gp);
    return linr_launch_rc();
}

int linr_conv_bwd_gm_launch(LinrCmap m, const Conv88BwdGroup* g, int ng, hipStream_t s) {
    if (ng < 1 || ng > LINR_MAXG) return LINR_EINVAL;
    if (m.n == 0) return 0;
    Grp gp = Grp();
    for (int i = 0; i < ng; ++i) {
        gp.in[i] = g[i].g - g[0].g; gp.w[i] = g[i].W - g[0].W; gp.out[i] = g[i].out - g[0].out;
// ... 709 lines not shown
```

### linr_pcgc_amd/csrc/net.hip

```cpp
#include "common.h"
#include "conv_common.h"
#include "layout.h"
#include "sce.h"
#include "net_shared.h"
#include <math.h>
#include <stdlib.h>
#include <vector>
#include <mutex>
#include <atomic>

#define TRY(e) do { int rc_ = (e); if (rc_) return rc_; } while (0)

extern "C" int linr_abi_version(void) { return LINR_ABI_VERSION; }

extern "C" int64_t linr_param_count(int32_t scale_num, int32_t block_layers) {
    Layout L;
    return make_layout(L, scale_num, block_layers) ? L.total : (int64_t)LINR_EINVAL;
}

struct Arena {
    int64_t rows;
    float* base;
    int64_t cur;
    int64_t pad_off[200];
// ... 482 lines not shown
        float ms = 0.0f;
        TRY(linr_hip_rc(hipEventElapsedTime(&ms, r.ev0, r.ev1)));
        t += ms;
        np += r.passes;
    }
    *total_ms = t; *launches = (int64_t)g_prof[kind].size(); *passes = np;
    return 0;
}

static LinrCmap cmap(const Ctx& c) { return {c.f->nbr_lo, c.f->nbr_mask, c.nbr_ld, c.R}; }

static bool join_block_in(const Ctx& c) { return c.L.block_in.nl == 1; }

static bool fused_bwd(const Ctx& c) {
    static const int v = getenv("LINR_FUSED_BWD") ? atoi(getenv("LINR_FUSED_BWD")) : 1;
    return v != 0 && linr_cmap_fits32(c.nbr_ld);
}

static int conv3(Ctx& c, bool bwd, const float* in, int in_ld, const float* W, const float* bias, int cin, int cout,
                 const float* res, int res_ld, const float* act, int act_ld, float* out, int out_ld, unsigned flags) {
    ProfScope ps(c.s, bwd ? PK_BWD_DATA : PK_CONV88, 1);
    const ConvGroup g = {in, W, bias, res, act, out};
    return linr_cconv_launch(bwd, cmap(c), &g, 1, in_ld, cin, cout, res_ld, act_ld, out_ld, flags, c.s);
}

static const int32_t* wg_t8t(const Ctx& c) { return c.f->nbr8t; }
static int conv3_wgrad(Ctx& c, const float* in, int in_ld, const float* gout, int gout_ld, int cin, int cout,
                       int64_t w_off, int64_t b_off) {
    ProfScope ps(c.s, PK_WGRAD, 1);
    const WgradGroup g = {in, gout, w_off, b_off, 0};
    return linr_conv3_wgrad_mfma(&g, 1, in_ld, gout_ld, c.f->nbr, c.nbr_ld, c.R, wg_t8t(c), cin, cout, c.A.BIG, c.L.total, c.nb, c.s);
}

static int linear(Ctx& c, const float* in, int in_ld, int64_t n, const float* W, int ws_ci, int ws_co, const float* bias,
                  int cin, int cout, const float* res, int res_ld, const float* act, int act_ld, float* out, int out_ld,
                  unsigned flags) {
    return linr_linear_launch(in, in_ld, n, W, ws_ci, ws_co, bias, cin, cout, res, res_ld, act, act_ld, out, out_ld, flags,
                              c.s);
}

static int linear_wgrad(Ctx& c, const float* in, int in_ld, const float* gout, int gout_ld, int64_t n, int cin, int cout,
                        int64_t w_off, int ws_ci, int ws_co, int64_t b_off) {
    ProfScope ps(c.s, PK_LIN_WGRAD, 1);
    const WgradGroup g = {in, gout, w_off, b_off, 0};
    return linr_linear_wgrad_partial(&g, 1, in_ld, gout_ld, n, cin, cout, c.A.BIG, c.L.total, ws_ci, ws_co, c.nb, c.s);
}

struct LayerBufs { float *H, *M, *I, *gI, *gM, *gH; };
static LayerBufs layer_bufs(Arena& a, int b, int l) {
    if (l == 0) return {a.H[b], a.M[b], a.I[b], a.gI[b], a.gM[b], a.gH[b]};
    return {a.Hx[l - 1], a.Mx[l - 1], a.Ix[l - 1], a.gIx[l - 1], a.gMx[l - 1], a.gHx[l - 1]};
}

static const BlockP& slot_block(const Layout& L, int b) { return b == 0 ? L.block_in : L.outter[b - 1]; }
static ConvPwGroup pw_fwd_group(const float* P, const IncP& q, const float* X, const LayerBufs& t) {
    return {X, P + q.c00_w, P + q.c00_b, P + q.c10_w, P + q.c10_b, t.H};
}
static Dual44FwdGroup dual_fwd_group(const float* P, const IncP& q, const float* X, const LayerBufs& t) {
    return {t.H, P + q.c01_w, P + q.c01_b, P + q.c11_w, P + q.c11_b, X, P + q.c12_w, P + q.c12_b, t.M, t.I};
}
static Conv88BwdGroup tail_bwd_group(const float* P, const BlockP& bp, const IncP& q, const float* gO, const LayerBufs& t) {
    return {gO, t.I, P + bp.b_w, t.gI, bp.b_w, bp.b_b, P + q.c12_w, t.M, t.gM, q.c12_w, q.c12_b};
}
static Dual44BwdGroup dual_bwd_group(const float* P, const IncP& q, const LayerBufs& t) {
    return {t.gI, t.gM, t.H, P + q.c01_w, P + q.c11_w, t.gH, q.c01_w, q.c01_b, q.c11_w, q.c11_b};
}
static Conv84BwdGroup c00_bwd_group(const float* P, const IncP& q, const float* A, const LayerBufs& t, float* gA) {
    return {t.gH, A, t.gI, P + q.c00_w, P + q.c10_w, gA, q.c00_w, q.c00_b, q.c10_w, q.c10_b};
}
static HeadFwdGroup head_fwd_group(Ctx& c, int k, bool bits) {
    const Arena& a = c.A;
    const Layout& L = c.L;
    double* part = bits ? (double*)a.slab + (int64_t)k * linr_grid(c.R, LINR_BLOCK) : nullptr;
    return {a.O[k], c.P + L.pr_w[k], c.P + L.pr_b[k], a.C[k], c.P + L.h0_w[k], c.P + L.h0_b[k], c.P + L.h2_w[k], c.P + L.h2_b[k],
            a.OCC + k, a.P[k], part};
}
static WgradGroup wgrad_of(const Conv88BwdGroup& g) { return {g.xin, g.g, g.w_off, g.b_off, 0}; }
static ConvGroup bwd_data_of(const Conv88BwdGroup& g) { return {g.g, g.W, nullptr, nullptr, nullptr, g.out}; }

static int block_fwd(Ctx& c, const BlockP& bp, const float* in, int in_ld, int b, const float* res) {
    Arena& a = c.A;
    const float* P = c.P;
    TRY(conv3(c, false, in, in_ld, P + bp.a_w, P + bp.a_b, bp.cin, 8, nullptr, 0, nullptr, 0, a.A[b], 8, LINR_RELU));
    const float* X = a.A[b];
    for (int l = 0; l < bp.nl; ++l) {
        const IncP& q = bp.inc[l];
        const LayerBufs t = layer_bufs(a, b, l);
        const ConvPwGroup g0 = pw_fwd_group(P, q, X, t);
        TRY(linr_conv_pw_fwd_launch(cmap(c), &g0, 1, c.s));
        const Dual44FwdGroup g1 = dual_fwd_group(P, q, X, t);
        TRY(linr_dual44_fwd_launch(cmap(c), &g1, 1, c.s));
        X = t.I;
    }
    float* Il = layer_bufs(a, b, bp.nl - 1).I;
    if (bp.nl > 1)
        axpy_k<<<linr_grid(c.R * 8, LINR_BLOCK), LINR_BLOCK, 0, c.s>>>(a.A[b], c.R * 8, Il, 1);
    TRY(conv3(c, false, Il, 8, P + bp.b_w, P + bp.b_b, 8, 8, res, 8, nullptr, 0, a.O[b], 8, 0));
    return 0;
}

static int block_bwd(Ctx& c, const BlockP& bp, const float* in, int in_ld, int b, const float* gO, float* gin) {
    Arena& a = c.A;
    const float* P = c.P;
    const int nl = bp.nl;
    const LayerBufs last = layer_bufs(a, b, nl - 1);
    TRY(conv3_wgrad(c, last.I, 8, gO, 8, 8, 8, bp.b_w, bp.b_b));
    for (int l = nl - 1; l >= 0; --l) {
        const IncP& q = bp.inc[l];
        const LayerBufs t = layer_bufs(a, b, l);
        const float* X = l == 0 ? a.A[b] : layer_bufs(a, b, l - 1).I;
        float* gX = l == 0 ? a.gA[b] : layer_bufs(a, b, l - 1).gI;
        if (l == nl - 1) {
            const Conv88BwdGroup g = tail_bwd_group(P, bp, q, gO, t);
            TRY(linr_conv_bwd_gm_launch(cmap(c), &g, 1, c.s));
        } else
            TRY(linear(c, t.gI + 4, 8, c.R, P + q.c12_w, 1, 4, nullptr, 4, 4, nullptr, 0, t.M, 4, t.gM, 4, LINR_RELU_MASK));
        TRY(linear_wgrad(c, t.M, 4, t.gI + 4, 8, c.R, 4, 4, q.c12_w, 4, 1, q.c12_b));
        const Dual44BwdGroup gd = dual_bwd_group(P, q, t);
        TRY(linr_conv3_wgrad_dual44(&gd, 1, 8, 4, c.f->nbr, c.nbr_ld, c.R, wg_t8t(c), a.BIG, c.L.total, c.nb, c.s));
        TRY(linr_dual44_bwd_launch(cmap(c), &gd, 1, c.s));
        TRY(conv3_wgrad(c, X, 8, t.gH, 8, 8, 4, q.c00_w, q.c00_b));
        TRY(linear_wgrad(c, X, 8, t.gH + 4, 8, c.R, 8, 4, q.c10_w, 4, 1, q.c10_b));
        const bool skip = (l == 0 && nl > 1);
        if (skip)
            TRY(linr_hip_rc(hipMemcpyAsync(gX, last.gI, (size_t)c.R * 8 * sizeof(float), hipMemcpyDeviceToDevice, c.s)));
        const Conv84BwdGroup ga = c00_bwd_group(P, q, l == 0 ? a.A[b] : nullptr, t, gX);
        TRY(linr_conv_bwd_ga_launch(cmap(c), &ga, 1, (l == 0 ? LINR_RELU_MASK : 0u) | (skip ? LINR_ACCUM : 0u), c.s));
    }
    TRY(conv3_wgrad(c, in, in_ld, a.gA[b], 8, bp.cin, 8, bp.a_w, bp.a_b));
    if (gin) TRY(conv3(c, true, a.gA[b], 8, P + bp.a_w, nullptr, bp.cin, 8, nullptr, 0, nullptr, 0, gin, 8, 0));
    return 0;
}

static int check_frame(const linr_frame* f, const void* params, const void* arena, size_t arena_bytes, Ctx& c) {
    if (!params || !arena) return LINR_EINVAL;
    TRY(linr_frame_layout(f, 0, c.L));
    if (f->rows > 0 && (!f->nbr || !f->nbr_lo || !f->nbr_mask || !f->offset_feat || !f->occ)) return LINR_EINVAL;
    if (!linr_rows_fit32(f->rows) || f->nbr_ld < f->rows) return LINR_EINVAL;
    if (arena_bytes < linr_net_arena_bytes(f->rows, c.L.BL)) return LINR_ENOSPC;
    if (!linr_aligned16(arena)) return LINR_EALIGN;
    c.f = f;
    c.P = (const float*)params;
    c.R = f->rows;
    c.nbr_ld = f->nbr_ld;
    c.nb = wg_blocks_for(f->rows);
    make_arena(c.A, f->rows, (float*)arena, c.L.total, c.L.BL);
    if (f->flags & LINR_FRAME_OCC_PADDED) {
        if (!f->occ || !linr_aligned16(f->occ)) return LINR_EINVAL;
        c.A.OCC = const_cast<float*>(f->occ);
    }
    return 0;
}

static int forward_batched(Ctx& c, float* probs, double* bits_acc) {
    Arena& a = c.A;
    const float* P = c.P;
    const Layout& L = c.L;
    const LinrCmap m = cmap(c);
    const int64_t nblk = linr_grid(c.R, LINR_BLOCK);
    const bool join = join_block_in(c);
    const int g0 = join ? 0 : 1, ng = 8 - g0;
    {
        int64_t w_off[7], b_off[7], o_off[7];
        for (int g = 0; g < 7; ++g) { w_off[g] = L.outter[g].a_w; b_off[g] = L.outter[g].a_b; o_off[g] = a.A[g + 1] - a.A[1]; }
        ProfScope ps(c.s, PK_OCC7, 7);
        TRY(linr_occ_conv7_launch(a.OCC, m, P, w_off, b_off, a.A[1], o_off, c.s));
    }
    {
        ConvPwGroup g[8];
        for (int i = 0; i < ng; ++i) g[i] = pw_fwd_group(P, slot_block(L, g0 + i).inc[0], a.A[g0 + i], layer_bufs(a, g0 + i, 0));
        ProfScope ps(c.s, PK_CONVPW_FWD, ng);
        TRY(linr_conv_pw_fwd_launch(m, g, ng, c.s));
    }
    {
        Dual44FwdGroup g[8];
        for (int i = 0; i < ng; ++i) g[i] = dual_fwd_group(P, slot_block(L, g0 + i).inc[0], a.A[g0 + i], layer_bufs(a, g0 + i, 0));
        ProfScope ps(c.s, PK_DUAL_FWD, ng);
        TRY(linr_dual44_fwd_launch(m, g, ng, c.s));
    }
    if (join)
        TRY(conv3(c, false, a.I[0], 8, P + L.block_in.b_w, P + L.block_in.b_b, 8, 8, nullptr, 0, nullptr, 0, a.O[0], 8, 0));
    {
        ConvGroup g[7];
        for (int b = 1; b < 8; ++b) g[b - 1] = {a.I[b], P + L.outter[b - 1].b_w, P + L.outter[b - 1].b_b, a.O[0], nullptr, a.O[b]};
        ProfScope ps(c.s, PK_CONV88, 7);
        TRY(linr_cconv_launch(false, m, g, 7, 8, 8, 8, 8, 0, 8, 0, c.s));
    }
    {
        HeadFwdGroup g[8];
        for (int k = 0; k < 8; ++k) g[k] = head_fwd_group(c, k, bits_acc != nullptr);
        ProfScope ps(c.s, PK_HEAD_FWD, 8);
        TRY(linr_cconv_head_launch(m, g, 8, 8, c.s));
    }
    if (bits_acc) {
        ProfScope ps(c.s, PK_MISC, 0);
        TRY(linr_bits_finish_launch((const double*)a.slab, (int)(8 * nblk), bits_acc, c.s));
    }
    if (probs)
        for (int k = 0; k < 8; ++k)
            TRY(linr_hip_rc(hipMemcpyAsync(probs + (int64_t)k * c.R, a.P[k], (size_t)c.R * sizeof(float), hipMemcpyDeviceToDevice, c.s)));
    return linr_launch_rc();
}

extern "C" int linr_net_forward(const linr_frame* f, const float* params, float* arena, size_t arena_bytes,
                                int32_t stage_begin, int32_t stage_end, float* probs, double* bits_acc, void* stream) {
    Ctx c;
    TRY(check_frame(f, params, arena, arena_bytes, c));
    if (stage_begin < 0 || stage_end > 8 || stage_begin >= stage_end) return LINR_EINVAL;
    c.s = (hipStream_t)stream;
    if (c.R == 0) return 0;
    Arena& a = c.A;
    const float* P = c.P;
    if (!(f->flags & LINR_FRAME_OCC_PADDED))
        TRY(linr_hip_rc(hipMemcpyAsync(a.OCC, f->occ, (size_t)c.R * 8 * sizeof(float), hipMemcpyDeviceToDevice, c.s)));
    const bool all_stages = stage_begin == 0 && stage_end == 8;
    if (stage_begin == 0) {
        PadList pl;
        pl.n = a.npad;
        for (int i = 0; i < a.npad; ++i) { pl.off[i] = a.pad_off[i]; pl.w[i] = a.pad_w[i]; }
        {
            ProfScope ps(c.s, PK_SCE, 1);
            const SceArgs sa = sce_args(c.f, c.L);
            sce_fwd_k<float><<<sa.blk_off[sa.n_scales] + (a.npad + LINR_BLOCK / 32 - 1) / (LINR_BLOCK / 32), LINR_BLOCK, 0, c.s>>>(
                P, f->offset_feat, sa, c.R, nullptr, nullptr, a.X0, a.base, pl);
        }
        if (all_stages && join_block_in(c)) {
            const BlockP& bi = c.L.block_in;
            TRY(conv3(c, false, a.X0, 8, P + bi.a_w, P + bi.a_b, bi.cin, 8, nullptr, 0, nullptr, 0, a.A[0], 8, LINR_RELU));
        } else {
            TRY(block_fwd(c, c.L.block_in, a.X0, 8, 0, nullptr));
        }
    }
    if (all_stages) return forward_batched(c, probs, bits_acc);
    const int64_t nblk = linr_grid(c.R, LINR_BLOCK);
    for (int k = stage_begin; k < stage_end; ++k) {
        if (k > 0) TRY(block_fwd(c, c.L.outter[k - 1], a.OCC, 8, k, a.O[0]));
        const HeadFwdGroup g = head_fwd_group(c, k, bits_acc != nullptr);
        TRY(linr_cconv_head_launch(cmap(c), &g, 1, 8, c.s));
        if (probs)
            TRY(linr_hip_rc(hipMemcpyAsync(probs + (int64_t)k * c.R, a.P[k], (size_t)c.R * sizeof(float),
                                           hipMemcpyDeviceToDevice, c.s)));
    }
    if (bits_acc)
        TRY(linr_bits_finish_launch((const double*)a.slab + (int64_t)stage_begin * nblk, (int)((stage_end - stage_begin) * nblk),
                                    bits_acc, c.s));
    return linr_launch_rc();
}

extern "C" int linr_sce_fwd(const float* params, const linr_frame* f, float* mix, float* hid, float* x0, void* stream) {
    Layout L;
    TRY(linr_frame_layout(f, 0, L));
    if (f->rows == 0) return 0;
    if (!params || !f->offset_feat || !hid || !x0) return LINR_EINVAL;
    if ((mix && !linr_aligned16(mix)) || !linr_aligned16(hid) || !linr_aligned16(x0)) return LINR_EALIGN;
    const SceArgs sa = sce_args(f, L);
    sce_fwd_k<float><<<sa.blk_off[sa.n_scales], LINR_BLOCK, 0, (hipStream_t)stream>>>(params, f->offset_feat, sa, f->rows, mix, hid, x0, nullptr,
                                                                              PadList{{}, {}, 0});
    return linr_launch_rc();
}

extern "C" int linr_sce_bwd(const float* params, const linr_frame* f, const float* gx0, const float* hid, float* ghid,
                            void* stream) {
    Layout L;
    TRY(linr_frame_layout(f, 0, L));
    if (f->rows == 0) return 0;
    if (!params || !gx0 || !hid || !ghid) return LINR_EINVAL;
    if (!linr_aligned16(gx0) || !linr_aligned16(hid) || !linr_aligned16(ghid)) return LINR_EALIGN;
    const SceArgs sa = sce_args(f, L);
    sce_bwd_k<<<sa.blk_off[sa.n_scales], LINR_BLOCK, 0, (hipStream_t)stream>>>(params, sa, f->rows, gx0, hid, ghid);
    return linr_launch_rc();
}

struct SceBwdPlan { SceArgs sa; ZeroRanges zr; ShortRanges sr; EmbArgs ea; int ns; };
static void short_push(ShortRanges& sr, int64_t b, int64_t e, int rows) {
    if (sr.n >= MAX_SHORT) abort();
    sr.b[sr.n] = b; sr.e[sr.n] = e; sr.rows[sr.n] = rows; ++sr.n;
}
static bool sce_bwd_plan(const linr_frame* f, const Layout& L, int nb, const LinrShortRange* sh, int nsh, SceBwdPlan& p) {
    p.sr.n = 0;
    for (int i = 0; i < nsh; ++i)
        if (sh[i].rows < nb) short_push(p.sr, sh[i].b, sh[i].e, sh[i].rows);
    const int64_t total = L.block_in.a_w;
    p.sa = sce_args(f, L);
    p.zr.n = 0; p.zr.prefix = total;
    p.zr.b[p.zr.n] = L.emb; p.zr.e[p.zr.n] = L.emb + (int64_t)L.S * 8; ++p.zr.n;
    p.ns = 0;
    bool present[MAX_SCALES] = {}, distinct = true;
    p.sa.wg_off[0] = 0;
    for (int j = 0; j < f->n_scales; ++j) {
        const int64_t nj = f->row_off_h[j + 1] - f->row_off_h[j];
        int64_t wg = nj > 0 ? (nj + LINR_BLOCK - 1) / LINR_BLOCK : 0;
        if (wg > nb) wg = nb;
        p.sa.wg_off[j + 1] = p.sa.wg_off[j] + (int)wg;
        if (wg == 0) continue;
        const int si = f->scale_idx_h[j];
        if (present[si]) distinct = false;
        present[si] = true;
        if (wg < nb) short_push(p.sr, L.m0_w[si], L.m2_b[si] + 8, (int)wg);
        p.ea.gb1[p.ns] = L.m0_b[si]; p.ea.w1[p.ns] = L.m0_w[si]; p.ea.gemb[p.ns] = L.emb + si * 8; ++p.ns;
    }
    for (int si = 0; si < L.S; ++si)
        if (!present[si]) {
            p.zr.b[p.zr.n] = L.m0_w[si];
            p.zr.e[p.zr.n] = si + 1 < L.S ? L.m0_w[si + 1] : total;
            ++p.zr.n;
        }
    return distinct;
}

#define SCE_SLAB_ROWS 256
extern "C" int64_t linr_sce_param_count(int32_t model_scale_num) {
    Layout L;
    return make_layout(L, model_scale_num, 1) ? L.block_in.a_w : (int64_t)LINR_EINVAL;
}
extern "C" size_t linr_sce_bwd_params_slab_bytes(int32_t model_scale_num) {
    const int64_t t = linr_sce_param_count(model_scale_num);
    return t > 0 ? (size_t)SCE_SLAB_ROWS * (size_t)t * sizeof(float) : 0;
}
extern "C" int linr_sce_bwd_params(const float* params, const linr_frame* f, const float* gx0, const float* hid, float* slab,
                                   size_t slab_bytes, float* grads, void* stream) {
    Layout L;
    TRY(linr_frame_layout(f, 0, L));
    if (!params || !gx0 || !hid || !slab || !grads) return LINR_EINVAL;
    if (f->rows > 0 && !f->offset_feat) return LINR_EINVAL;
    if (!linr_aligned16(gx0) || !linr_aligned16(hid)) return LINR_EALIGN;
    const int64_t total = L.block_in.a_w;
    if (slab_bytes < (size_t)SCE_SLAB_ROWS * (size_t)total * sizeof(float)) return LINR_ENOSPC;
    hipStream_t s = (hipStream_t)stream;
    const int nb = SCE_SLAB_ROWS;
    SceBwdPlan pl;
    if (!sce_bwd_plan(f, L, nb, nullptr, 0, pl)) return LINR_EINVAL;
    if (pl.ns > 0) sce_bwd_all_k<<<pl.sa.wg_off[f->n_scales], SB_WAVES * 64, 0, s>>>(params, f->offset_feat, pl.sa, gx0, hid, slab, total);
    wgrad_reduce_k<<<linr_grid(total, LINR_BLOCK / RED_SPLIT), LINR_BLOCK, 0, s>>>(slab, nb, total, grads, pl.zr, pl.sr);
    if (pl.ns > 0) sce_emb_grad_all_k<<<pl.ns, LINR_WAVE, 0, s>>>(params, grads, pl.ea);
    return linr_launch_rc();
}

int linr_slab_reduce_launch(const float* big, int nblocks, int64_t total, float* gsum, hipStream_t s) {
    if (total <= 0) return 0;
    ZeroRanges zr;
    zr.n = 0; zr.prefix = 0;
    ShortRanges sr;
    sr.n = 0;
    wgrad_reduce_k<<<linr_grid(total, LINR_BLOCK / RED_SPLIT), LINR_BLOCK, 0, s>>>(big, nblocks, total, gsum, zr, sr);
    return linr_launch_rc();
}

struct Ptr8 { const float* p[8]; };
__global__ __launch_bounds__(LINR_BLOCK) void sum8_k(Ptr8 src, int64_t n, float* __restrict__ dst) {
    const int64_t i = (int64_t)blockIdx.x * LINR_BLOCK + threadIdx.x;
    if (i >= n) return;
    float t = src.p[7][i];
#pragma unroll
    for (int k = 6; k >= 0; --k) t = t + src.p[k][i];
    dst[i] = t;
}

static int backward_batched(Ctx& c, float gz_scale) {
    Arena& a = c.A;
    const float* P = c.P;
    const Layout& L = c.L;
    const LinrCmap m = cmap(c);
    {
        {
            HeadBwdGroup g[8];
            for (int k = 0; k < 8; ++k)
                g[k] = {a.C[k], a.P[k], a.OCC + k, P + L.h0_w[k], P + L.h0_b[k], P + L.h2_w[k], a.gC[k], L.h0_w[k], L.h0_b[k], L.h2_w[k], L.h2_b[k]};
            ProfScope ps(c.s, PK_HEAD_BWD, 8);
            int hrows = 0;
            TRY(linr_head_bwd_launch(g, 8, 8, gz_scale, c.R, a.BIG, L.total, c.nb, &hrows, c.s));
            c.note_short(L.h0_w[0], L.h2_b[7] + 1, hrows);
        }
        Conv88BwdGroup pr[8];
        for (int k = 0; k < 8; ++k) pr[k] = {a.gC[k], a.O[k], P + L.pr_w[k], a.gO[k], L.pr_w[k], L.pr_b[k], nullptr, nullptr, nullptr, 0, 0};
        if (fused_bwd(c)) {
            ProfScope ps(c.s, PK_FUSED88, 8);
            int rows = 0;
            TRY(linr_conv88_bwd_wgrad_launch(m, pr, 8, a.BIG, L.total, c.nb, &rows, c.s));
            c.note_short(L.pr_w[0], L.pr_b[7] + 8, rows);
        } else {
        {
            WgradGroup g[8];
            for (int k = 0; k < 8; ++k) g[k] = wgrad_of(pr[k]);
            ProfScope ps(c.s, PK_WGRAD, 8);
            TRY(linr_conv3_wgrad_mfma(g, 8, 8, 8, c.f->nbr, c.nbr_ld, c.R, wg_t8t(c), 8, 8, a.BIG, L.total, c.nb, c.s));
        }
        {
            ConvGroup g[8];
            for (int k = 0; k < 8; ++k) g[k] = bwd_data_of(pr[k]);
            ProfScope ps(c.s, PK_BWD_DATA, 8);
            TRY(linr_cconv_launch(true, m, g, 8, 8, 8, 8, 0, 0, 8, 0, c.s));
        }
        }
        Ptr8 src;
        for (int k = 0; k < 8; ++k) src.p[k] = a.gO[k];
        ProfScope ps(c.s, PK_MISC, 0);
        sum8_k<<<linr_grid(c.R * 8, LINR_BLOCK), LINR_BLOCK, 0, c.s>>>(src, c.R * 8, a.gXG);
    }
    const bool join = join_block_in(c);
// ... 207 lines not shown
```

### linr_pcgc_amd/engine.py

```python
import ctypes

import numpy as np
import torch

from . import _lib, ops
from ._lib import check


class Frame:

    def __init__(self, scales, model_scale_num, device='cuda', validate=True, with_arena=True, block_layers=1):
        device = torch.device(device)
        if device.type != 'cuda':
            raise _lib.LinrError('Frame needs a GPU device: the coding network has no CPU path')
        self.device = device
        self.model_scale_num = int(model_scale_num)
        self.block_layers = int(block_layers)
        for i, s in enumerate(scales):
            c = s['coord']
            n = int(c.shape[0])
            if c.ndim != 2 or c.shape[1] != 3:
                raise ValueError("scale %d: 'coord' must be [N, 3], got %s" % (i, tuple(c.shape)))
            if not 0 <= int(s['scale_idx']) < self.model_scale_num:
                raise ValueError("scale %d: 'scale_idx' %d is outside the model's 0..%d" % (i, int(s['scale_idx']), self.model_scale_num - 1))
            off = s.get('offset_tensor')
            if off is not None and tuple(off.shape) != (n, 7):
                raise ValueError("scale %d: 'offset_tensor' must be [%d, 7], got %s" % (i, n, tuple(off.shape)))
            if s.get('occ') is not None:
                if tuple(s['occ'].shape) != (n, 8):
                    raise ValueError("scale %d: 'occ' must be [%d, 8], got %s" % (i, n, tuple(s['occ'].shape)))
            elif s.get('occ_lst') is not None:
                lst = s['occ_lst']
                if len(lst) != 8 or any(int(torch.as_tensor(o).numel()) != n for o in lst):
                    raise ValueError("scale %d: 'occ_lst' must hold 8 columns of %d values, got %d entries of sizes %s"
                                     % (i, n, len(lst), sorted({int(torch.as_tensor(o).numel()) for o in lst})))
        ns = [int(s['coord'].shape[0]) for s in scales]
        self.row_off = np.zeros(len(scales) + 1, dtype=np.int64)
        self.row_off[1:] = np.cumsum(ns)
        self.rows = int(self.row_off[-1])
        self.scale_idx = np.asarray([int(s['scale_idx']) for s in scales], dtype=np.int32)
        self.n_scales = len(scales)
        R = self.rows
        self.nbr_ld = (R + 63) // 64 * 64
        self.nbr = torch.empty((27, self.nbr_ld), dtype=torch.int32, device=device)
        if self.nbr_ld > R:
            self.nbr[:, R:] = -1
        self.offset_feat = torch.empty((R, 7), dtype=torch.float32, device=device)
        self._occ_buf = torch.empty((R + 1, 8), dtype=torch.float32, device=device)
        self._occ_buf[0].zero_()
        self.occ = self._occ_buf[1:]
        bad = torch.zeros(1, dtype=torch.int32, device=device) if validate else None
        have_occ = [('occ' in s and s['occ'] is not None) or ('occ_lst' in s and s['occ_lst'] is not None) for s in scales]
        if not all(have_occ):
            self.occ.zero_()
        need_feat = []
        L = _lib.lib()
        for i, s in enumerate(scales):
            r0, r1 = int(self.row_off[i]), int(self.row_off[i + 1])
            if r1 == r0:
                continue
            coord = torch.as_tensor(s['coord']).to(device=device, dtype=torch.int32).contiguous()
            if validate:
                check(L.linr_kmap_validate(coord.data_ptr(), r1 - r0, bad.data_ptr(), _stream()), 'linr_kmap_validate')
            ops.kmap_build_into(coord, self.nbr, r0, False)
            if s.get('offset_tensor') is None:
                need_feat.append((r0, r1))
            else:
                self.offset_feat[r0:r1] = torch.as_tensor(s['offset_tensor']).to(device=device, dtype=torch.float32)
            if 'occ' in s and s['occ'] is not None:
                self.occ[r0:r1] = torch.as_tensor(s['occ']).to(device=device, dtype=torch.float32)
            elif 'occ_lst' in s and s['occ_lst'] is not None:
                self.occ[r0:r1] = torch.cat([torch.as_tensor(o).reshape(-1, 1) for o in s['occ_lst']], dim=1).to(
                    device=device, dtype=torch.float32)
        merged = []
        for r0, r1 in need_feat:
            if merged and merged[-1][1] == r0:
                merged[-1][1] = r1
            else:
                merged.append([r0, r1])
        for r0, r1 in merged:
            check(L.linr_kmap_offset_feat(self.nbr.data_ptr(), self.nbr_ld, r0, r1 - r0, self.offset_feat[r0:r1].data_ptr(), _stream()),
                  'linr_kmap_offset_feat')
        self.nbr_lo = torch.empty((9, self.nbr_ld), dtype=torch.int32, device=device)
        self.nbr_mask = torch.empty((self.nbr_ld,), dtype=torch.int32, device=device)
        if self.nbr_ld > R:
            self.nbr_lo[:, R:] = 0
            self.nbr_mask[R:] = 0
        check(_lib.lib().linr_kmap_compress(self.nbr.data_ptr(), self.nbr_ld, R, self.nbr_lo.data_ptr(),
                                            self.nbr_mask.data_ptr(), self.nbr_ld, _stream()), 'linr_kmap_compress')
        nb8t = _lib.lib().linr_kmap_tile8t_bytes(R)
        self.nbr8t = torch.empty(max(4, (nb8t + 3) // 4), dtype=torch.int32, device=device)
        check(_lib.lib().linr_kmap_tile8t(self.nbr.data_ptr(), self.nbr_ld, R, self.nbr8t.data_ptr(), self.nbr8t.numel() * 4,
                                          _stream()), 'linr_kmap_tile8t')
        if validate and int(bad.item()) != 0:
            raise ValueError('coord must be unique, non-negative (< 2^20) and sorted by the x-major ravel key '
                             '(models/module_utils.py:246-256)')
        self.arena = None
        if with_arena:
            self.alloc_arena()
        self._c = _lib.LinrFrame(rows=R, n_scales=self.n_scales, model_scale_num=self.model_scale_num,
                                 block_layers=self.block_layers, flags=_lib.LINR_FRAME_OCC_PADDED,
                                 row_off_h=self.row_off.ctypes.data, scale_idx_h=self.scale_idx.ctypes.data,
                                 nbr=self.nbr.data_ptr(), nbr_ld=self.nbr_ld, nbr_lo=self.nbr_lo.data_ptr(),
                                 nbr_mask=self.nbr_mask.data_ptr(), offset_feat=self.offset_feat.data_ptr(),
                                 occ=self.occ.data_ptr(), nbr8t=self.nbr8t.data_ptr())

    def alloc_arena(self):
        nbytes = _lib.lib().linr_net_arena_bytes(self.rows, self.block_layers)
        self.arena = _lib.scratch(nbytes, self.device)

    def bf16_arena(self):
        if getattr(self, '_arena_bf16', None) is None:
            nbytes = _lib.lib().linr_net_bf16_arena_bytes(self.rows, self.block_layers)
            self._arena_bf16 = _lib.scratch(nbytes + 64, self.device)
        return self._arena_bf16

    def train_bf16_arena(self):
        if getattr(self, 'arena_train_bf16', None) is None:
            nbytes = _lib.lib().linr_net_train_bf16_arena_bytes(self.rows, self.block_layers)
            if nbytes == 0:
                raise _lib.LinrError('the bf16 training executor supports block_layers=1 only')
            self.arena_train_bf16 = _lib.scratch(nbytes + 64, self.device)
        a = self.arena_train_bf16
        base = (a.data_ptr() + 63) & ~63
        return base, a.numel() - (base - a.data_ptr())

    def invalidate_occ(self):
        self._occ_bf16 = None

    def occ_bf16(self):
        if getattr(self, '_occ_bf16', None) is None:
            t = torch.empty((self.rows + 1, 8), dtype=torch.int16, device=self.device)
            check(_lib.lib().linr_occ_to_bf16(self.occ.data_ptr(), self.rows, t.data_ptr(), _stream()), 'linr_occ_to_bf16')
            self._occ_bf16 = t
        return self._occ_bf16.data_ptr()

    def cref(self):
        return ctypes.byref(self._c)

    def scale_slice(self, i):
        return slice(int(self.row_off[i]), int(self.row_off[i + 1]))


def _stream():
    return _lib.current_stream_handle()


def net_forward(frame, flat_params, stage_begin=0, stage_end=8, probs=None, bits=None, arena=None):
    arena = frame.arena if arena is None else arena
    check(_lib.lib().linr_net_forward(frame.cref(), flat_params.data_ptr(), arena.data_ptr(), arena.numel(), stage_begin,
                                      stage_end, 0 if probs is None else probs.data_ptr(),
                                      0 if bits is None else bits.data_ptr(), _stream()), 'linr_net_forward')


def net_forward_bf16(frame, codes, min_param, max_param, stage_begin, stage_end, probs, bits=None):
    arena = frame.bf16_arena()
    base = (arena.data_ptr() + 63) & ~63
    check(_lib.lib().linr_net_forward_bf16(frame.cref(), codes.data_ptr(), float(min_param), float(max_param), base,
                                           arena.numel() - (base - arena.data_ptr()), stage_begin, stage_end, probs.data_ptr(),
                                           0 if bits is None else bits.data_ptr(), _stream()), 'linr_net_forward_bf16')


def net_decode_stages(frame, flat_params, streams_per_scale, probs, p_pinned, s_pinned, s_dev, qcodes=None, qrange=None):
    n = frame.n_scales
    bufs = [np.frombuffer(streams_per_scale[i][k], dtype=np.uint8) for i in range(n) for k in range(8)]
    ptrs = (ctypes.c_void_p * (8 * n))(*[b.ctypes.data if b.size else None for b in bufs])
    lens = (ctypes.c_int64 * (8 * n))(*[int(b.size) for b in bufs])
    if qcodes is None:
        arena, codes, lo, hi = frame.arena, None, 0.0, 0.0
        base, nbytes = arena.data_ptr(), arena.numel()
    else:
        arena = frame.bf16_arena()
        base = (arena.data_ptr() + 63) & ~63
        nbytes = arena.numel() - (base - arena.data_ptr())
        codes, lo, hi = qcodes.data_ptr(), float(qrange[0]), float(qrange[1])
    frame.invalidate_occ()
    check(_lib.lib().linr_net_decode_stages(frame.cref(), None if flat_params is None else flat_params.data_ptr(), codes, lo, hi,
                                            base, nbytes, ptrs, lens, probs.data_ptr(), p_pinned.data_ptr(), s_pinned.data_ptr(),
                                            s_dev.data_ptr(), _stream()), 'linr_net_decode_stages')


def net_backward(frame, flat_params, flat_grads, gscale, arena=None):
    arena = frame.arena if arena is None else arena
    check(_lib.lib().linr_net_backward(frame.cref(), flat_params.data_ptr(), arena.data_ptr(), arena.numel(), float(gscale),
                                       flat_grads.data_ptr(), _stream()), 'linr_net_backward')


def net_train_step(frame, flat_params, exp_avg, exp_avg_sq, gscale, step, lr, beta1, beta2, eps, weight_decay, bits,
                   arena=None, scale_steps=None):
    arena = frame.arena if arena is None else arena
    check(_lib.lib().linr_net_train_step(frame.cref(), flat_params.data_ptr(), arena.data_ptr(), arena.numel(),
                                         float(gscale), exp_avg.data_ptr(), exp_avg_sq.data_ptr(), float(lr), int(step),
                                         None if scale_steps is None else scale_steps.ctypes.data,
                                         beta1, beta2, eps, weight_decay, bits.data_ptr(), _stream()),
          'linr_net_train_step')


def net_forward_train_bf16(frame, flat_params, probs=None, bits=None):
    base, nbytes = frame.train_bf16_arena()
    check(_lib.lib().linr_net_forward_train_bf16(frame.cref(), flat_params.data_ptr(), base, nbytes, frame.occ_bf16(),
                                                 0 if probs is None else probs.data_ptr(), 0 if bits is None else bits.data_ptr(),
                                                 _stream()), 'linr_net_forward_train_bf16')


def net_backward_bf16(frame, flat_params, flat_grads, gscale):
    base, nbytes = frame.train_bf16_arena()
    check(_lib.lib().linr_net_backward_bf16(frame.cref(), flat_params.data_ptr(), base, nbytes, frame.occ_bf16(), float(gscale),
                                            flat_grads.data_ptr(), _stream()), 'linr_net_backward_bf16')


def net_train_step_bf16(frame, flat_params, exp_avg, exp_avg_sq, gscale, step, lr, beta1, beta2, eps, weight_decay, bits,
                        scale_steps=None):
    base, nbytes = frame.train_bf16_arena()
    check(_lib.lib().linr_net_train_step_bf16(frame.cref(), flat_params.data_ptr(), base, nbytes, frame.occ_bf16(),
                                              float(gscale), exp_avg.data_ptr(), exp_avg_sq.data_ptr(), float(lr), int(step),
                                              None if scale_steps is None else scale_steps.ctypes.data,
                                              beta1, beta2, eps, weight_decay, bits.data_ptr(), _stream()),
          'linr_net_train_step_bf16')
```

### linr_pcgc_amd/model_core.py

```python
import time

import numpy as np
import torch
from torch import nn

from . import _lib, engine, ops
from .function_utils import pack_bitstream, unpack_bitstream
from .module_utils import BinaryArithmeticCoding, PointwiseMLP
from .upsample import CNP


class _NetBits(torch.autograd.Function):

    @staticmethod
    def forward(ctx, model, frame, *params):
        bits = torch.zeros(1, dtype=torch.float64, device=frame.device)
        engine.net_forward(frame, model._flat, 0, 8, None, bits)
        ctx.model, ctx.frame = model, frame
        return bits[0].to(torch.float32)

    @staticmethod
    def backward(ctx, gout):
        model, frame = ctx.model, ctx.frame
        tmp = torch.zeros_like(model._flat)
# ... 46 lines not shown
                             'width cannot be loaded' % hidden)
        self.hidden = hidden
        if not 1 <= block_layers <= 4:
            raise ValueError('block_layers must be in 1..4 (main.py:521 default 1), got %d' % block_layers)
        self.block_layers = block_layers
        self.scale_emb = nn.Embedding(self.scale_num, 8)
        self.scale_mlp = nn.ModuleList([PointwiseMLP([8 + in_channel, 16, 8]) for _ in range(self.scale_num)])
        self.upsampler = CNP(in_channels=8, channels=hidden, block_layers=block_layers, outstage=8, instage=1)
        self.sigmoid = nn.Sigmoid()
        self._flat = None
        self._flat_grad = None
        self._plist = []
        self._frame_cache = {}
        self.inference_precision = 'f32'
        self.train_precision = 'f32'
        self._qcodes = None
        self._qrange = None
        self._wide = None
        if hidden != 8:
            from .wide_net import WideNet
            self._wide = WideNet(self, hidden)
        self._flatten()

    def _flatten(self):
        plist = list(self.parameters())
        total = sum(p.numel() for p in plist)
        if plist and plist[0].is_cuda and self.hidden == 8 and total != _lib.lib().linr_param_count(self.scale_num, self.block_layers):
            raise _lib.LinrError('parameter layout mismatch with liblinr_hip.so')
        flat = torch.empty(total, dtype=torch.float32, device=plist[0].device)
        off = 0
        with torch.no_grad():
            for p in plist:
                n = p.numel()
                flat[off:off + n].copy_(p.detach().reshape(-1))
                p.data = flat[off:off + n].view(p.shape)
                p.grad = None
                off += n
        self._flat, self._plist, self._flat_grad = flat, plist, None
        self._frame_cache = {}
        if getattr(self, '_wide', None) is not None:
            self._wide._built = False

    def _apply(self, fn, *args, **kwargs):
        flat = None
        if self._flat is not None and not any(True for _ in self.buffers()):
            with torch.no_grad():
                flat = fn(self._flat)
            if flat.dtype != torch.float32 or flat.numel() != self._flat.numel() or not flat.is_contiguous():
                flat = None
        if flat is None:
            out = super()._apply(fn, *args, **kwargs)
            self._flatten()
            return out
        if flat.is_cuda and self.hidden == 8 and flat.numel() != _lib.lib().linr_param_count(self.scale_num, self.block_layers):
            raise _lib.LinrError('parameter layout mismatch with liblinr_hip.so')
        off = 0
        with torch.no_grad():
            for q in self._plist:
                n = q.numel()
                q.data = flat[off:off + n].view(q.shape)
                q.grad = None
                off += n
        self._flat, self._flat_grad, self._frame_cache = flat, None, {}
        if self._qcodes is not None:
            self._qcodes = self._qcodes.to(flat.device)
        if getattr(self, '_wide', None) is not None:
            self._wide._built = False
        return self

    def _ensure_grad_views(self):
        if self._flat_grad is None or self._flat_grad.device != self._flat.device:
            self._flat_grad = torch.zeros_like(self._flat)
        off = 0
        for p in self._plist:
            n = p.numel()
            if p.grad is None or p.grad.data_ptr() != self._flat_grad.data_ptr() + 4 * off:
                if p.grad is None:
                    self._flat_grad[off:off + n].zero_()
                else:
                    self._flat_grad[off:off + n].copy_(p.grad.reshape(-1))
                p.grad = self._flat_grad[off:off + n].view(p.shape)
            off += n

    def set_quantised(self, codes, min_param, max_param):
        if codes.numel() != self._flat.numel():
            raise ValueError('expected %d codes, got %d' % (self._flat.numel(), codes.numel()))
        self._qcodes = codes.to(device=self._flat.device, dtype=torch.uint8).contiguous()
        self._qrange = (float(min_param), float(max_param))

    def _precision(self, precision):
        precision = self.inference_precision if precision is None else precision
        if precision not in ('f32', 'bf16'):
            raise ValueError("precision must be 'f32' or 'bf16'")
        if precision == 'bf16' and self._qcodes is None:
            raise _lib.LinrError('the bf16 path runs from the 8-bit weight codes: quantise the model first, at bitdepth 8 '
                                 '(Model_Estimate.compress_model(model, 8, derive_new_model=True) / decompress_model)')
        return precision

    def flat_parameters(self):
        return self._flat

    def make_frame(self, scales, validate=True, with_arena=True):
        return engine.Frame(scales, self.scale_num, self._flat.device, validate, with_arena and self._wide is None, self.block_layers)

    def _scale_frame(self, d, need_occ=True):
        coord = d['coord']
        s = {'coord': coord, 'offset_tensor': d.get('offset_tensor'), 'scale_idx': d['scale_idx']}
        if not need_occ:
            return self.make_frame([s])
        occ_lst, off = d.get('occ_lst'), d.get('offset_tensor')
        if occ_lst is None:
            occ_lst = list(d['occ'].split(1, dim=1))
        occ0 = occ_lst[0]
        key = (coord.data_ptr(), tuple(coord.shape), int(d['scale_idx']), None if off is None else (off.data_ptr(), tuple(off.shape)),
               occ0.data_ptr(), len(occ_lst), tuple(tuple(o.shape) for o in occ_lst))
        hit = self._frame_cache.get(key)
        if hit is None:
            if len(self._frame_cache) >= 1024:
                self._frame_cache.pop(next(iter(self._frame_cache)))
            s['occ_lst'] = occ_lst
            hit = (self.make_frame([s]), coord, off, list(occ_lst))
            self._frame_cache[key] = hit
        return hit[0]

    def forward(self, inargs):
        if int(inargs['coord'].shape[0]) == 0:
            return self._flat.sum() * 0.0
        frame = self._scale_frame(inargs)
        if torch.is_grad_enabled() and any(p.requires_grad for p in self._plist):
            return (_WideBits if self._wide is not None else _NetBits).apply(self, frame, *self._plist)
        bits = torch.zeros(1, dtype=torch.float64, device=frame.device)
        self._stage_forward(frame, 0, 8, None, bits, 'f32')
        return bits[0].to(torch.float32)

    def _stage_forward(self, frame, k0, k1, probs, bits, precision):
        if self._wide is not None:
            with torch.no_grad():
                if precision == 'bf16':
                    self._wide.forward_bf16(frame, k0, k1, probs, bits)
                else:
                    self._wide.forward(frame, k0, k1, probs, bits)
        elif precision == 'bf16':
            engine.net_forward_bf16(frame, self._qcodes, self._qrange[0], self._qrange[1], k0, k1, probs, bits)
        else:
            engine.net_forward(frame, self._flat, k0, k1, probs, bits)

    @torch.no_grad()
    def frame_probs(self, frame, precision=None):
        probs = torch.empty((8, frame.rows), dtype=torch.float32, device=frame.device)
        bits = torch.zeros(1, dtype=torch.float64, device=frame.device)
        self._stage_forward(frame, 0, 8, probs, bits, self._precision(precision))
        return probs, bits

    @torch.no_grad()
    def codec(self, inargs):
        st1 = time.time()
        frame = self._scale_frame(inargs)
        probs, bits_t = self.frame_probs(frame)
        p_host = probs.reshape(-1).cpu()
        sym = frame.occ.t().contiguous().reshape(-1).to(torch.int16).cpu()
        bac = BinaryArithmeticCoding()
        st2 = time.time()
        enc_bytes = bac.encode(p_host, sym)
        st3 = time.time()
        recon = bac.decode(p_host, enc_bytes)
        st4 = time.time()
        assert bool((recon == sym).all())
        return {'bits': len(enc_bytes) * 8, 'enc_bytes': enc_bytes, 'enc_time': st3 - st1,
                'dec_time': (st2 - st1) + (st4 - st3), 'bits_t': bits_t[0].to(torch.float32)}

    @torch.no_grad()
    def encode(self, in_args, DBG=False):
        frame = self._scale_frame(in_args)
        probs, _ = self.frame_probs(frame)
        p_host = probs.cpu().numpy()
        occ_host = frame.occ.t().contiguous().cpu().numpy().astype(np.uint8)
        streams = encode_streams([p_host[k] for k in range(8)], [occ_host[k] for k in range(8)])
        if DBG:
            bac = BinaryArithmeticCoding()
            for k in range(8):
                assert (bac.decode(p_host[k], streams[k]).numpy() == occ_host[k]).all()
        enc_bytes = pack_bitstream(streams)
        return {'enc_bytes': enc_bytes, 'bits': len(enc_bytes) * 8, 'x_low': None}

    @torch.no_grad()
    def decode(self, inagrs):
        streams = unpack_bitstream(inagrs['enc_bytes'])
        s = {'coord': inagrs['coord'], 'offset_tensor': inagrs.get('offset_tensor'), 'scale_idx': inagrs['scale_idx']}
        frame = self.make_frame([s], with_arena=self._precision(None) == 'f32')
        return self.decode_frame(frame, [streams])

    @torch.no_grad()
    def decode_scale(self, coord, scale_idx, enc_bytes, child_bits):
        import ctypes
        L = _lib.lib()
        n = int(coord.shape[0])
        if n == 0:
            return coord.new_zeros((0, 3))
        coord = coord.contiguous()
        streams = unpack_bitstream(enc_bytes)
        bufs = [np.frombuffer(b, dtype=np.uint8) for b in streams]
        ptrs = (ctypes.c_void_p * 8)(*[b.ctypes.data if b.size else None for b in bufs])
        lens = (ctypes.c_int64 * 8)(*[int(b.size) for b in bufs])
        bf16 = self._precision(None) == 'bf16'
        need = L.linr_decode_scale_ws_bytes(n, self.block_layers, 1 if bf16 else 0)
        ws = _lib.scratch(need + 256, coord.device)
        base = (ws.data_ptr() + 255) & ~255
        child = torch.empty((8 * n, 3), dtype=torch.int32, device=coord.device)
        p_host, s_host = self._host_buffers(n)
        m = ctypes.c_int64(0)
        codes, lo, hi, params = (self._qcodes.data_ptr(), float(self._qrange[0]), float(self._qrange[1]), None) if bf16 else \
            (None, 0.0, 0.0, self._flat.data_ptr())
        _lib.check(L.linr_decode_scale(coord.data_ptr(), n, int(scale_idx), self.scale_num, self.block_layers, int(child_bits), params,
                                       codes, lo, hi, ptrs, lens, base, need, p_host.data_ptr(), s_host.data_ptr(),
                                       child.data_ptr(), 8 * n, ctypes.byref(m), torch.cuda.current_stream().cuda_stream),
                   'linr_decode_scale')
        return child[:m.value]

    def _host_buffers(self, rows):
        import threading
        tls = self.__dict__.setdefault('_dec_tls', threading.local())
        buf = getattr(tls, 'buf', None)
        if buf is None or buf[0].numel() < rows:
            cap = max(rows, 1 << 16)
            buf = (torch.empty(cap, dtype=torch.float32, pin_memory=True), torch.empty(cap, dtype=torch.uint8, pin_memory=True))
            tls.buf = buf
        return buf

    @torch.no_grad()
    def decode_frame(self, frame, streams_per_scale, precision=None):
        frame.occ.zero_()
        frame.invalidate_occ()
        rows = frame.rows
        probs = torch.empty((8, rows), dtype=torch.float32, device=frame.device)
        s_dev = torch.empty(max(rows, 1), dtype=torch.uint8, device=frame.device)
        p_host, s_host = self._host_buffers(rows)
        precision = self._precision(precision)
        if self._wide is not None:
            L = _lib.lib()
            import ctypes
            for k in range(8):
                self._stage_forward(frame, k, k + 1, probs, None, precision)
                p_host[:rows].copy_(probs[k])
                for i in range(frame.n_scales):
                    r0, r1 = int(frame.row_off[i]), int(frame.row_off[i + 1])
                    if r1 == r0:
                        continue
                    buf = np.frombuffer(streams_per_scale[i][k], dtype=np.uint8)
                    _lib.check(L.linr_ac_decode_binary(ctypes.c_void_p(p_host.data_ptr() + 4 * r0), r1 - r0,
                                                       ctypes.c_void_p(buf.ctypes.data if buf.size else None), int(buf.size),
                                                       ctypes.c_void_p(s_host.data_ptr() + r0)), 'linr_ac_decode_binary')
                frame.occ[:, k].copy_(s_host[:rows].to(frame.device, torch.float32))
            return [frame.occ[:, k:k + 1].clone() for k in range(8)]
        if precision == 'bf16':
            engine.net_decode_stages(frame, None, streams_per_scale, probs, p_host, s_host, s_dev, self._qcodes, self._qrange)
        else:
            engine.net_decode_stages(frame, self._flat, streams_per_scale, probs, p_host, s_host, s_dev)
        return [frame.occ[:, k:k + 1].clone() for k in range(8)]


def encode_streams(probs, symbols, n_threads=8):
    import ctypes
    n = len(probs)
    probs = [np.ascontiguousarray(p, dtype=np.float32).reshape(-1) for p in probs]
    symbols = [np.ascontiguousarray(s, dtype=np.uint8).reshape(-1) for s in symbols]
    outs = [np.empty(2 * p.size + 64, dtype=np.uint8) for p in probs]
    arr_p = (ctypes.c_void_p * n)(*[p.ctypes.data for p in probs])
    arr_s = (ctypes.c_void_p * n)(*[s.ctypes.data for s in symbols])
    arr_o = (ctypes.c_void_p * n)(*[o.ctypes.data for o in outs])
    arr_n = (ctypes.c_int64 * n)(*[p.size for p in probs])
    arr_c = (ctypes.c_int64 * n)(*[o.size for o in outs])
    arr_l = (ctypes.c_int64 * n)()
    _lib.check(_lib.lib().linr_ac_encode_binary_batch(arr_p, arr_s, arr_n, n, arr_o, arr_c, arr_l, n_threads),
               'linr_ac_encode_binary_batch')
    return [outs[i][:arr_l[i]].tobytes() for i in range(n)]


class FlatAdam:

    def __init__(self, model, lr=0.01, betas=(0.9, 0.999), eps=1e-8, weight_decay=1e-4, step_size=32, gamma=0.992):
        self.model = model
        self.lr, self.initial_lr = float(lr), float(lr)
        self.betas, self.eps, self.weight_decay = tuple(betas), float(eps), float(weight_decay)
        self.step_size, self.gamma = int(step_size), float(gamma)
        flat = model.flat_parameters()
        self.exp_avg = torch.zeros_like(flat)
        self.exp_avg_sq = torch.zeros_like(flat)
        self.grad = torch.zeros_like(flat)
        self.t = 0
        self.sched_steps = 0
        self.t_scale = np.zeros(model.scale_num, dtype=np.int64)
        self._segments = None

    def zero_grad(self):
        self.grad.zero_()

    def reset(self):
        self.exp_avg.zero_()
        self.exp_avg_sq.zero_()
        self.grad.zero_()
        self.lr = self.initial_lr
        self.t = 0
        self.sched_steps = 0
        self.t_scale[:] = 0

    def advance(self, frame=None):
        t_scale = self.t_scale.copy()
        if frame is None:
            t_scale += 1
        else:
            present = np.zeros(len(t_scale), dtype=bool)
            for i in range(frame.n_scales):
                if frame.row_off[i + 1] > frame.row_off[i]:
                    present[frame.scale_idx[i]] = True
            t_scale[present | (t_scale > 0)] += 1
        return self.t + 1, t_scale

    def _param_segments(self):
        if self._segments is None:
            segs, off = [], 0
            for own, p in zip(self._scale_of_param(), self.model._plist):
                n = p.numel()
                if segs and segs[-1][2] == own:
                    segs[-1][1] = off + n
                else:
                    segs.append([off, off + n, own])
                off += n
            self._segments = [tuple(x) for x in segs]
        return self._segments

    def step(self, frame=None):
        t, t_scale = self.advance(frame)
        flat = self.model.flat_parameters()
        runs = []
        for b, e, own in self._param_segments():
            ts = t if own < 0 else int(t_scale[own])
            if ts < 1:
                continue
            if runs and runs[-1][1] == b and runs[-1][2] == ts:
                runs[-1][1] = e
            else:
                runs.append([b, e, ts])
        for b, e, ts in runs:
            ops.adam_step(flat[b:e], self.grad[b:e], self.exp_avg[b:e], self.exp_avg_sq[b:e], ts, self.lr,
                          self.betas[0], self.betas[1], self.eps, self.weight_decay)
        self.t, self.t_scale = t, t_scale

    def scheduler_step(self):
        self.sched_steps += 1
        if self.sched_steps % self.step_size == 0:
            self.lr *= self.gamma

    def clamp_lr(self, min_lr):
        if self.lr < min_lr:
            self.lr = min_lr

    def _scale_of_param(self):
        out = []
        for name, _ in self.model.named_parameters():
            out.append(int(name.split('.')[1]) if name.startswith('scale_mlp.') else -1)
        return out

    def state_dict(self):
        state, off = {}, 0
        owner = self._scale_of_param()
        for i, p in enumerate(self.model._plist):
            n = p.numel()
            t = self.t if owner[i] < 0 else int(self.t_scale[owner[i]])
            if t > 0:
                state[i] = {'step': torch.tensor(float(t)), 'exp_avg': self.exp_avg[off:off + n].view(p.shape).clone(),
                            'exp_avg_sq': self.exp_avg_sq[off:off + n].view(p.shape).clone()}
            off += n
        group = {'lr': self.lr, 'betas': self.betas, 'eps': self.eps, 'weight_decay': self.weight_decay,
                 'amsgrad': False, 'maximize': False, 'foreach': None, 'capturable': False,
                 'initial_lr': self.initial_lr, 'params': list(range(len(self.model._plist)))}
        return {'state': state, 'param_groups': [group]}

    def load_state_dict(self, sd):
        g = sd['param_groups'][0]
        self.lr = float(g['lr'])
        self.initial_lr = float(g.get('initial_lr', self.initial_lr))
        self.betas, self.eps, self.weight_decay = tuple(g['betas']), float(g['eps']), float(g['weight_decay'])
        off = 0
        steps = set()
        owner = self._scale_of_param()
        self.t_scale[:] = 0
        self.exp_avg.zero_()
        self.exp_avg_sq.zero_()
        for i, p in enumerate(self.model._plist):
            n = p.numel()
            st = sd['state'].get(i)
            if st is not None:
                self.exp_avg[off:off + n].copy_(st['exp_avg'].reshape(-1))
                self.exp_avg_sq[off:off + n].copy_(st['exp_avg_sq'].reshape(-1))
                t = int(float(st['step']))
                if owner[i] < 0:
                    steps.add(t)
                else:
                    if self.t_scale[owner[i]] not in (0, t):
                        raise ValueError('step counts differ inside scale_mlp.%d' % owner[i])
                    self.t_scale[owner[i]] = t
            off += n
        if len(steps) > 1:
            raise ValueError('step counts of the shared parameters differ; the fused Adam keeps one counter for them')
        self.t = steps.pop() if steps else 0


def train_step(model, opt, frame, point_num, out=None):
    bits = torch.zeros(1, dtype=torch.float64, device=frame.device) if out is None else out
    if model._wide is not None:
        if model.train_precision != 'f32':
            raise _lib.LinrError('the bf16 training executor exists for hidden_channel_conv=8 only')
        with torch.no_grad(), model._wide.lock:
            tape = model._wide.forward(frame, 0, 8, None, bits, keep=True, pool=True)
            model._ensure_grad_views()
            model._flat_grad.zero_()
            if tape is not None:
                model._wide.backward(frame, tape, 1.0 / float(point_num), pool=True)
            opt.grad.copy_(model._flat_grad)
            opt.step(frame)
        opt.scheduler_step()
        return bits
    t, t_scale = opt.advance(frame)
    if model.train_precision == 'bf16':
        if model.block_layers != 1:
            raise _lib.LinrError('the bf16 training executor supports block_layers=1 only')
        engine.net_train_step_bf16(frame, model.flat_parameters(), opt.exp_avg, opt.exp_avg_sq, 1.0 / float(point_num), t,
# ... 10 lines not shown
```

### linr_pcgc_amd/ops.py

```python
import torch

from . import _lib
from ._lib import LINR_ACCUM, LINR_NO_BIAS, LINR_PAD_ROW, LINR_RELU, LINR_RELU_MASK, check


def _stream():
    return _lib.current_stream_handle()


def _dev(t, dtype, name):
    if not t.is_cuda:
        raise _lib.LinrError('%s must be a GPU tensor: the coding network has no CPU path' % name)
    if t.dtype != dtype or not t.is_contiguous():
        raise ValueError('%s must be contiguous %s' % (name, dtype))
    return t


def _ptr(t):
    return 0 if t is None else t.data_ptr()


def kmap_build(coords, validate=True):
    _dev(coords, torch.int32, 'coords')
    n = coords.shape[0]
    nbr = torch.empty((27, n), dtype=torch.int32, device=coords.device)
    kmap_build_into(coords, nbr, 0, validate)
    return nbr


def kmap_build_into(coords, nbr, row_base, validate=True):
    L = _lib.lib()
    n = coords.shape[0]
    if n == 0:
        return
    if validate:
        bad = torch.zeros(1, dtype=torch.int32, device=coords.device)
        check(L.linr_kmap_validate(coords.data_ptr(), n, bad.data_ptr(), _stream()), 'linr_kmap_validate')
        if int(bad.item()) != 0:
            raise ValueError('coord must be unique, non-negative (< 2^20) and sorted by the x-major ravel key '
                             '(models/module_utils.py:246-256)')
    ws = _lib.scratch(L.linr_kmap_workspace_bytes(n), coords.device)
    check(L.linr_kmap_build(coords.data_ptr(), n, nbr.data_ptr(), nbr.shape[1], row_base, ws.data_ptr(), ws.numel(),
                            _stream()), 'linr_kmap_build')


def spconv_fwd(x, nbr, kernel, bias, res=None, relu=False, out=None, pad_row=False):
    n, cin, cout = nbr.shape[1], kernel.shape[1], kernel.shape[2]
    if out is None:
        out = torch.empty((n, cout), dtype=torch.float32, device=x.device)
    flags = (LINR_RELU if relu else 0) | (LINR_PAD_ROW if pad_row else 0)
    check(_lib.lib().linr_spconv_fwd(x.data_ptr(), x.stride(0), nbr.data_ptr(), nbr.stride(0), n, kernel.data_ptr(),
                                     bias.data_ptr(), cin, cout, _ptr(res), 0 if res is None else res.stride(0),
                                     out.data_ptr(), out.stride(0), flags, _stream()), 'linr_spconv_fwd')
    return out


def spconv_bwd_data(gout, nbr, kernel, act=None, out=None, accumulate=False, pad_row=False):
    n, cin = nbr.shape[1], kernel.shape[1]
    cout = kernel.shape[2]
    if out is None:
        out = torch.empty((n, cin), dtype=torch.float32, device=gout.device)
    flags = (LINR_ACCUM if accumulate else 0) | (LINR_RELU_MASK if act is not None else 0) | \
            (LINR_PAD_ROW if pad_row else 0)
    check(_lib.lib().linr_spconv_bwd_data(gout.data_ptr(), gout.stride(0), nbr.data_ptr(), nbr.stride(0), n,
                                          kernel.data_ptr(), cin, cout, _ptr(act),
                                          0 if act is None else act.stride(0), out.data_ptr(), out.stride(0), flags,
                                          _stream()), 'linr_spconv_bwd_data')
    return out


def spconv_bwd_weight(x, gout, nbr, cin, cout, pad_row=False):
    n = nbr.shape[1]
    L = _lib.lib()
    gw = torch.empty((27, cin, cout), dtype=torch.float32, device=x.device)
    gb = torch.empty((1, cout), dtype=torch.float32, device=x.device)
    ws = _lib.scratch(max(L.linr_spconv_bwd_weight_workspace_bytes(n, cin, cout), 4), x.device)
    check(L.linr_spconv_bwd_weight(x.data_ptr(), x.stride(0), gout.data_ptr(), gout.stride(0), nbr.data_ptr(),
                                   nbr.stride(0), n, cin, cout, gw.data_ptr(), gb.data_ptr(), LINR_PAD_ROW if pad_row else 0,
                                   ws.data_ptr(),
                                   ws.numel(), _stream()), 'linr_spconv_bwd_weight')
    return gw, gb


def linear_fwd(x, weight, bias, cin, cout, layout, res=None, relu=False, out=None):
    n = x.shape[0]
    ws_ci, ws_co = (cout, 1) if layout == 'me' else (1, cin)
    if out is None:
        out = torch.empty((n, cout), dtype=torch.float32, device=x.device)
    flags = (LINR_RELU if relu else 0) | (LINR_NO_BIAS if bias is None else 0)
    check(_lib.lib().linr_linear_fwd(x.data_ptr(), x.stride(0), n, weight.data_ptr(), ws_ci, ws_co, _ptr(bias), cin, cout,
                                     _ptr(res), 0 if res is None else res.stride(0), out.data_ptr(), out.stride(0),
                                     flags, _stream()), 'linr_linear_fwd')
    return out


def linear_bwd_data(gout, weight, cin, cout, layout, act=None, out=None, accumulate=False):
    n = gout.shape[0]
    ws_ci, ws_co = (cout, 1) if layout == 'me' else (1, cin)
    if out is None:
        out = torch.empty((n, cin), dtype=torch.float32, device=gout.device)
    flags = (LINR_ACCUM if accumulate else 0) | (LINR_RELU_MASK if act is not None else 0)
    check(_lib.lib().linr_linear_bwd_data(gout.data_ptr(), gout.stride(0), n, weight.data_ptr(), ws_ci, ws_co, cin, cout,
                                          _ptr(act), 0 if act is None else act.stride(0), out.data_ptr(),
                                          out.stride(0), flags, _stream()), 'linr_linear_bwd_data')
    return out


def linear_bwd_weight(x, gout, cin, cout, layout):
    n = x.shape[0]
    L = _lib.lib()
    ws_ci, ws_co = (cout, 1) if layout == 'me' else (1, cin)
    gw = torch.empty((cin, cout) if layout == 'me' else (cout, cin), dtype=torch.float32, device=x.device)
    gb = torch.empty((cout,), dtype=torch.float32, device=x.device)
    ws = _lib.scratch(max(L.linr_linear_bwd_weight_workspace_bytes(n, cin, cout), 4), x.device)
    check(L.linr_linear_bwd_weight(x.data_ptr(), x.stride(0), gout.data_ptr(), gout.stride(0), n, cin, cout,
                                   gw.data_ptr(), ws_ci, ws_co, gb.data_ptr(), 0, ws.data_ptr(), ws.numel(),
                                   _stream()), 'linr_linear_bwd_weight')
    return gw, gb


def bce_bits_fwd(z, target):
    n = z.shape[0]
    L = _lib.lib()
    p = torch.empty((n,), dtype=torch.float32, device=z.device)
    bits = torch.zeros(1, dtype=torch.float64, device=z.device)
    ws = _lib.scratch(max(L.linr_bce_workspace_bytes(n), 8), z.device)
    check(L.linr_bce_bits_fwd(z.data_ptr(), target.data_ptr(), target.stride(0), n, p.data_ptr(), bits.data_ptr(),
                              ws.data_ptr(), ws.numel(), _stream()), 'linr_bce_bits_fwd')
    return p, bits


def bce_bits_bwd(p, target, gscale):
    n = p.shape[0]
    gz = torch.empty((n,), dtype=torch.float32, device=p.device)
    check(_lib.lib().linr_bce_bits_bwd(p.data_ptr(), target.data_ptr(), target.stride(0), n, gscale, gz.data_ptr(),
                                       _stream()), 'linr_bce_bits_bwd')
    return gz


def adam_step(params, grads, exp_avg, exp_avg_sq, step, lr, beta1=0.9, beta2=0.999, eps=1e-8, weight_decay=1e-4):
    bc1 = 1.0 - beta1 ** step
    bc2_sqrt = (1.0 - beta2 ** step) ** 0.5
    check(_lib.lib().linr_adam_step(params.data_ptr(), grads.data_ptr(), exp_avg.data_ptr(), exp_avg_sq.data_ptr(),
                                    params.numel(), lr / bc1, bc2_sqrt, beta1, beta2, eps, weight_decay, _stream()),
          'linr_adam_step')


def kmap_compress(nbr, n=None):
    ld = nbr.shape[1]
    n = ld if n is None else n
    lo = torch.zeros((9, ld), dtype=torch.int32, device=nbr.device)
    mask = torch.zeros((ld,), dtype=torch.int32, device=nbr.device)
    check(_lib.lib().linr_kmap_compress(nbr.data_ptr(), nbr.stride(0), n, lo.data_ptr(), mask.data_ptr(), ld, _stream()),
          'linr_kmap_compress')
    return lo, mask


def spconv_cmap(x, lo, mask, n, kernel, bias=None, bwd=False, res=None, act=None, relu=False, out=None, accumulate=False):
    cin, cout = kernel.shape[1], kernel.shape[2]
    width = cin if bwd else cout
    if out is None:
        out = torch.empty((n, width), dtype=torch.float32, device=x.device)
    flags = (LINR_RELU if relu else 0) | (LINR_ACCUM if accumulate else 0) | (LINR_RELU_MASK if act is not None else 0) | \
        LINR_PAD_ROW
    check(_lib.lib().linr_spconv_cmap(1 if bwd else 0, x.data_ptr(), x.stride(0), lo.data_ptr(), mask.data_ptr(),
                                      lo.stride(0), n, kernel.data_ptr(), _ptr(bias), cin, cout, _ptr(res),
                                      0 if res is None else res.stride(0), _ptr(act), 0 if act is None else act.stride(0),
                                      out.data_ptr(), out.stride(0), flags, _stream()), 'linr_spconv_cmap')
    return out


def _ptr_array(blocks):
    import ctypes
    return (ctypes.c_void_p * len(blocks))(*[b.data_ptr() for b in blocks])


def spconv_wide(xs, lo, mask, n, kernel, bias=None, bwd=False, res=None, act=None, relu=False, outs=None, accumulate=False, pw=None):
    import ctypes
    cin, cout = kernel.shape[1], kernel.shape[2]
    npb = (cin if bwd else cout) // 8
    if outs is None:
        outs = [torch.empty((n, 8), dtype=torch.float32, device=xs[0].device) for _ in range(npb)]
    flags = (LINR_RELU if relu else 0) | (LINR_ACCUM if accumulate else 0) | (LINR_RELU_MASK if act is not None else 0)
    args = (1 if bwd else 0, _ptr_array(xs), lo.data_ptr(), mask.data_ptr(), lo.stride(0), n, kernel.data_ptr(), _ptr(bias), cin, cout,
            None if res is None else _ptr_array(res), None if act is None else _ptr_array(act), _ptr_array(outs), flags)
    if pw is None:
        check(_lib.lib().linr_spconv_wide(*args, _stream()), 'linr_spconv_wide')
    else:
        mode, w, b, aux, out2 = pw
        aux_a = None if aux is None else _ptr_array(aux)
        out_a = None if out2 is None else _ptr_array(out2)
        st = _lib.LinrWidePw(mode, w.data_ptr(), _ptr(b), None if aux_a is None else ctypes.cast(aux_a, ctypes.c_void_p),
                             None if out_a is None else ctypes.cast(out_a, ctypes.c_void_p))
        check(_lib.lib().linr_spconv_wide_pw(*args, ctypes.byref(st), _stream()), 'linr_spconv_wide_pw')
    return outs


def spconv_wgrad_wide(xs, gouts, nbr, tile8t, n, cin, cout, gw=None, gb=None, defer=None):
    L = _lib.lib()
    dev = xs[0].device
    if gw is None:
        gw = torch.empty((27, cin, cout), dtype=torch.float32, device=dev)
    if gb is None:
        gb = torch.empty((cout,), dtype=torch.float32, device=dev)
    assert gw.is_contiguous() and gb.is_contiguous()
    slab = _lib.scratch(L.linr_spconv_wgrad_wide_slab_bytes(cin, cout), dev)
    deferred = defer is not None and n > 0
    check(L.linr_spconv_wgrad_wide(_ptr_array(xs), cin, _ptr_array(gouts), cout, nbr.data_ptr(), _ptr(tile8t), nbr.stride(0), n,
                                   slab.data_ptr(), None if deferred else gw.data_ptr(), gb.data_ptr(), _stream()), 'linr_spconv_wgrad_wide')
    if deferred:
        nblk = int(L.linr_spconv_wgrad_wide_blocks(cout, 1 if tile8t is not None else 0))
        defer.append((_lib.LinrWideReduce(0, nblk, cin, cout, 0, 0, slab.data_ptr(), gw.data_ptr(), gb.data_ptr()), slab, gw, gb))
    return gw, gb


def spconv_wgrad_wide2(xsA, gsA, gwA, gbA, xsB, gsB, gwB, gbB, tile8t, n, defer):
    L = _lib.lib()
    nb = len(xsA)
    h = 8 * nb
    stride = 2 * nb * nb * 1736
    slab = _lib.scratch(256 * stride * 4, xsA[0].device)
    check(L.linr_spconv_wgrad_wide2(_ptr_array(xsA), _ptr_array(gsA), _ptr_array(xsB), _ptr_array(gsB), h, tile8t.data_ptr(), n,
                                    slab.data_ptr(), _stream()), 'linr_spconv_wgrad_wide2')
    for cv, (gw, gb) in enumerate(((gwA, gbA), (gwB, gbB))):
        assert gw.is_contiguous() and gb.is_contiguous()
        defer.append((_lib.LinrWideReduce(0, 256, h, h, stride, 0, slab.data_ptr() + 4 * cv * nb * nb * 1736, gw.data_ptr(), gb.data_ptr()),
                      slab, gw, gb))


def wide_reduce_many(deferred):
    if not deferred:
        return
    arr = (_lib.LinrWideReduce * len(deferred))(*[d[0] for d in deferred])
    check(_lib.lib().linr_wide_reduce_many(arr, len(deferred), _stream()), 'linr_wide_reduce_many')
    deferred.clear()


def linear_wide(xs, cin, w, ws_ci, ws_co, bias, cout, outs, in_blocked=True, out_blocked=True, res=None, act=None, relu=False,
                accumulate=False):
    n = xs[0].shape[0]
    flags = (LINR_RELU if relu else 0) | (LINR_ACCUM if accumulate else 0) | (LINR_RELU_MASK if act is not None else 0) | \
        (_lib.LINR_NO_BIAS if bias is None else 0)
    check(_lib.lib().linr_linear_wide(_ptr_array(xs), cin, 1 if in_blocked else 0, w.data_ptr(), ws_ci, ws_co, _ptr(bias), cout,
                                      1 if out_blocked else 0, None if res is None else _ptr_array(res),
                                      None if act is None else _ptr_array(act), _ptr_array(outs), n, flags, _stream()), 'linr_linear_wide')
    return outs


def linear_wgrad_wide(xs, cin, gouts, cout, gw, ws_ci, ws_co, gb, in_blocked=True, g_blocked=True, accumulate=False, defer=None):
    L = _lib.lib()
    n = xs[0].shape[0]
    ws = _lib.scratch(max(L.linr_linear_wgrad_wide_workspace_bytes(n, cin, cout), 4), xs[0].device)
    deferred = defer is not None and n > 0 and not accumulate
    check(L.linr_linear_wgrad_wide(_ptr_array(xs), cin, 1 if in_blocked else 0, _ptr_array(gouts), cout, 1 if g_blocked else 0, n,
                                   None if deferred else gw.data_ptr(), ws_ci, ws_co, _ptr(gb), LINR_ACCUM if accumulate else 0,
                                   ws.data_ptr(), ws.numel(), _stream()), 'linr_linear_wgrad_wide')
    if deferred:
        defer.append((_lib.LinrWideReduce(1, int(L.linr_linear_wgrad_wide_blocks(n)), cin, cout, ws_ci, ws_co, ws.data_ptr(), gw.data_ptr(),
                                          _ptr(gb)), ws, gw, gb))


def head_wide_fwd(cs, w1, b1, w2, b2, target, p, bits=None, partial=None):
    L = _lib.lib()
    n, C = cs[0].shape[0], 8 * len(cs)
    ws = partial
    if bits is not None and ws is None:
        ws = _lib.scratch(max(L.linr_head_wide_workspace_bytes(n), 8), cs[0].device)
    check(L.linr_head_wide_fwd(_ptr_array(cs), C, w1.data_ptr(), b1.data_ptr(), w2.data_ptr(), b2.data_ptr(), _ptr(target),
                               1 if target is None else target.stride(0), n, p.data_ptr(), _ptr(bits) if partial is None else None,
                               _ptr(ws), 0 if ws is None else ws.numel() * ws.element_size(), _stream()), 'linr_head_wide_fwd')
    return p


def bits_finish(partial, count, bits):
    check(_lib.lib().linr_bits_finish(partial.data_ptr(), count, bits.data_ptr(), _stream()), 'linr_bits_finish')


def head_wide_bwd(cs, ps, targets, w1s, b1s, w2s, gscale, gcs, grads):
    import ctypes
    L = _lib.lib()
    ns, nb = len(ps), len(cs[0])
    n, C = cs[0][0].shape[0], 8 * nb

    def arr(ts):
        return (ctypes.c_void_p * len(ts))(*[t.data_ptr() for t in ts])
    slab = _lib.scratch(L.linr_head_wide_bwd_slab_bytes(C, ns), cs[0][0].device)
    assert grads.is_contiguous() and grads.numel() == ns * (24 * C + 49)
    check(L.linr_head_wide_bwd(arr([b for c in cs for b in c]), arr(ps), arr(targets), targets[0].stride(0), arr(w1s), arr(b1s), arr(w2s),
                               C, ns, float(gscale), arr([b for g in gcs for b in g]), n, slab.data_ptr(), slab.numel(), grads.data_ptr(),
                               _stream()), 'linr_head_wide_bwd')
# ... 153 lines not shown
```

Baseline: 0.01692.

## Fuse coder quantization into head kernel and stream compact codes to host

Adds a codec epilogue to the fused head conv kernel that writes 16-bit arithmetic-coder thresholds and uint8 symbols directly instead of float probabilities. A new native frame-encode entry runs the full forward, then issues the device-to-host copies on a copy stream from C++, and a new batch arithmetic encoder consumes the precomputed thresholds. The aim is to halve probability transfer bytes, drop the separate occupancy transpose/cast and Python-side event juggling, and skip host-side probability-to-threshold conversion. It relies on the device rounding matching the host c1_block exactly, or bitstreams could diverge.

After: 0.01695, median of 2. Within noise of the previous version (+0.2%).

```diff
diff --git a/include/linr_hip.h b/include/linr_hip.h
--- a/include/linr_hip.h
+++ b/include/linr_hip.h
@@ -8,7 +8,7 @@
 extern "C" {
 #endif
 
-#define LINR_ABI_VERSION 13
+#define LINR_ABI_VERSION 14
 #define LINR_API __attribute__((visibility("default")))
 
 #define LINR_EINVAL   (-1)
@@ -273,6 +273,15 @@
 LINR_API int linr_ply_parse_ascii(const char* text_h, size_t len, int64_t n_rows, int32_t n_cols, int32_t cx, int32_t cy,
                          int32_t cz, int64_t* xyz_h, int64_t* rows_parsed_h);
 
+LINR_API int64_t linr_ac_encode_binary_c1(const uint16_t* c1_h, const uint8_t* sym_h, int64_t n, uint8_t* out_h, int64_t cap);
+LINR_API int linr_ac_encode_binary_c1_batch(const uint16_t* const* c1_h, const uint8_t* const* sym_h, const int64_t* n,
+                                   int32_t n_streams, uint8_t* const* out_h, const int64_t* cap,
+                                   int64_t* out_len, int32_t n_threads);
+LINR_API int linr_c1_from_probs(const float* p_dev, int64_t n, uint16_t* c1_dev, void* stream);
+LINR_API int linr_net_encode_frame(const linr_frame* f, const float* params, float* arena, size_t arena_bytes, uint16_t* c1_dev,
+                          uint8_t* sym_dev, uint16_t* c1_pinned, uint8_t* sym_pinned, double* bits_acc, void* stream,
+                          void* copy_stream, void* copied_event);
+
 #ifdef __cplusplus
 }
 #endif
diff --git a/linr_pcgc_amd/_lib.py b/linr_pcgc_amd/_lib.py
--- a/linr_pcgc_amd/_lib.py
+++ b/linr_pcgc_amd/_lib.py
@@ -8,7 +8,7 @@
 
 LINR_RELU, LINR_ACCUM, LINR_RELU_MASK, LINR_NO_BIAS, LINR_PAD_ROW = 1, 2, 4, 8, 16
 LINR_FRAME_OCC_PADDED = 1
-ABI_VERSION = 13
+ABI_VERSION = 14
 
 c_i32, c_i64, c_u32, c_f32, c_f64 = ctypes.c_int32, ctypes.c_int64, ctypes.c_uint32, ctypes.c_float, ctypes.c_double
 c_ptr, c_size = ctypes.c_void_p, ctypes.c_size_t
@@ -160,6 +160,11 @@
     'linr_ac_decode_cdf16': (ctypes.c_int, [c_ptr, c_i32, c_i32, c_i64, c_ptr, c_i64, c_ptr]),
     'linr_ply_parse_ascii': (ctypes.c_int, [c_ptr, c_size, c_i64, c_i32, c_i32, c_i32, c_i32, c_ptr, c_ptr]),
     'linr_ac_encode_binary_batch': (ctypes.c_int, [c_ptr, c_ptr, c_ptr, c_i32, c_ptr, c_ptr, c_ptr, c_i32]),
+    'linr_ac_encode_binary_c1': (c_i64, [c_ptr, c_ptr, c_i64, c_ptr, c_i64]),
+    'linr_ac_encode_binary_c1_batch': (ctypes.c_int, [c_ptr, c_ptr, c_ptr, c_i32, c_ptr, c_ptr, c_ptr, c_i32]),
+    'linr_c1_from_probs': (ctypes.c_int, [c_ptr, c_i64, c_ptr, c_ptr]),
+    'linr_net_encode_frame': (ctypes.c_int, [ctypes.POINTER(LinrFrame), c_ptr, c_ptr, c_size, c_ptr, c_ptr, c_ptr, c_ptr, c_ptr, c_ptr,
+                                             c_ptr, c_ptr]),
 }
 
 EXPORTS = tuple(_PROTOS)
diff --git a/linr_pcgc_amd/codec.py b/linr_pcgc_amd/codec.py
--- a/linr_pcgc_amd/codec.py
+++ b/linr_pcgc_amd/codec.py
@@ -7,7 +7,8 @@
 
 from .function_utils import pack_bitstream, unpack_bitstream
 from .model_codec import Model_Estimate
-from .model_core import encode_streams
+from . import _lib
+from .model_core import encode_streams, encode_streams_c1
 from .module_utils import octree_level_obj, qscTensor, unique_sorted
 
 ARITH_VERSION = 2
@@ -54,54 +55,71 @@
     workers = 2 if n_threads >= 4 else 1
     per_job = max(1, n_threads // workers)
 
-    def code(p_host, occ_host, row_off, n_scales):
-        ps, ss = [], []
+    direct = coded_model.has_frame_encoder(precision) and not os.environ.get('LINR_CODEC_PYTHON_PATH')
+    encode = encode_streams_c1 if direct else encode_streams
+
+    def code(v_host, occ_host, row_off, n_scales):
+        vs, ss = [], []
         for i in range(n_scales):
             a, b = int(row_off[i]), int(row_off[i + 1])
             for k in range(8):
-                ps.append(p_host[k, a:b])
+                vs.append(v_host[k, a:b])
                 ss.append(occ_host[k, a:b])
-        streams = encode_streams(ps, ss, per_job)
+        streams = encode(vs, ss, per_job)
         return [pack_bitstream(streams[8 * i:8 * i + 8]) for i in range(n_scales)]
 
     RING = 4
     max_rows = max(f.rows for f in gop.frames)
     dev = gop.frames[0].device
-    p_pin = [torch.empty(8 * max_rows, dtype=torch.float32, pin_memory=True) for _ in range(RING)]
+    v_pin = [torch.empty(8 * max_rows, dtype=torch.int16 if direct else torch.float32, pin_memory=True) for _ in range(RING)]
     o_pin = [torch.empty(8 * max_rows, dtype=torch.uint8, pin_memory=True) for _ in range(RING)]
     copy_stream = torch.cuda.Stream(device=dev)
-    jobs, bits_dev, pending = [], [], []
+    jobs, pending = [], []
+    bits_dev = torch.zeros((len(gop.frames), 1), dtype=torch.float64, device=dev)
+    if direct:
+        v_dev = [_lib.scratch(16 * max_rows, dev) for _ in range(RING)]
+        o_dev = [_lib.scratch(8 * max_rows, dev) for _ in range(RING)]
+        copied = [torch.cuda.Event() for _ in range(RING)]
+        for ev in copied:
+            ev.record(copy_stream)
 
     def hand_over(entry, coder):
         slot, rows, f, keep, ev_c = entry
         ev_c.synchronize()
-        p_host = p_pin[slot][:8 * rows].view(8, rows).numpy()
+        v_host = v_pin[slot][:8 * rows].view(8, rows).numpy()
+        if direct:
+            v_host = v_host.view(np.uint16)
         occ_host = o_pin[slot][:8 * rows].view(8, rows).numpy()
-        jobs.append(coder.submit(code, p_host, occ_host, f.row_off, f.n_scales))
+        jobs.append(coder.submit(code, v_host, occ_host, f.row_off, f.n_scales))
 
     with ThreadPoolExecutor(max_workers=workers) as coder:
         for i, f in enumerate(gop.frames):
             slot = i % RING
             if i >= RING:
                 jobs[i - RING].result()
-            probs, bits = coded_model.frame_probs(f)
-            bits_dev.append(bits)
-            occ_t = f.occ.t().to(torch.uint8).contiguous()
-            ev_f = torch.cuda.Event()
-            ev_f.record()
-            with torch.cuda.stream(copy_stream):
-                copy_stream.wait_event(ev_f)
-                p_pin[slot][:8 * f.rows].view(8, f.rows).copy_(probs, non_blocking=True)
-                o_pin[slot][:8 * f.rows].view(8, f.rows).copy_(occ_t, non_blocking=True)
-                ev_c = torch.cuda.Event()
-                ev_c.record(copy_stream)
-            pending.append((slot, f.rows, f, (probs, occ_t), ev_c))
+            if direct:
+                coded_model.encode_frame_codes(f, v_dev[slot], o_dev[slot], v_pin[slot], o_pin[slot], bits_dev[i], copy_stream,
+                                               copied[slot])
+                pending.append((slot, f.rows, f, None, copied[slot]))
+            else:
+                probs, bits = coded_model.frame_probs(f)
+                bits_dev[i].copy_(bits)
+                occ_t = f.occ.t().to(torch.uint8).contiguous()
+                ev_f = torch.cuda.Event()
+                ev_f.record()
+                with torch.cuda.stream(copy_stream):
+                    copy_stream.wait_event(ev_f)
+                    v_pin[slot][:8 * f.rows].view(8, f.rows).copy_(probs, non_blocking=True)
+                    o_pin[slot][:8 * f.rows].view(8, f.rows).copy_(occ_t, non_blocking=True)
+                    ev_c = torch.cuda.Event()
+                    ev_c.record(copy_stream)
+                pending.append((slot, f.rows, f, (probs, occ_t), ev_c))
             if len(pending) > 1:
                 hand_over(pending.pop(0), coder)
         while pending:
             hand_over(pending.pop(0), coder)
         frames_bytes = [j.result() for j in jobs]
-    bits_est = float(torch.stack(bits_dev).sum())
+    bits_est = float(bits_dev.sum())
     low = enc_all_frame_low_xyz(gop)
     points = sum(gop.point_nums)
     occ_bits = 8 * sum(len(b) for fb in frames_bytes for b in fb)
diff --git a/linr_pcgc_amd/csrc/ac.cpp b/linr_pcgc_amd/csrc/ac.cpp
--- a/linr_pcgc_amd/csrc/ac.cpp
+++ b/linr_pcgc_amd/csrc/ac.cpp
@@ -151,19 +151,19 @@
 
 }
 
-extern "C" int64_t linr_ac_encode_binary(const float* prob_h, const uint8_t* sym_h, int64_t n, uint8_t* out_h, int64_t cap) {
-    if (n < 0 || cap < 0 || (n > 0 && (!prob_h || !sym_h)) || (cap > 0 && !out_h)) return LINR_EINVAL;
-    BitSinkFast sink(out_h, cap);
+namespace {
+
+struct BinaryEncoder {
+    BitSinkFast sink;
     uint32_t low = 0, high = 0xFFFFFFFFu;
     uint64_t pending = 0;
-    uint32_t c1[AC_CHUNK];
-    for (int64_t base = 0; base < n; base += AC_CHUNK) {
-        const int m = (int)(n - base < AC_CHUNK ? n - base : AC_CHUNK);
-        c1_block(prob_h + base, m, c1);
-        for (int i = 0; i < m; ++i) {
+    BinaryEncoder(uint8_t* o, int64_t c) : sink(o, c) {}
+    template <class T>
+    inline void run(const T* c1, const uint8_t* sym, int64_t m) {
+        for (int64_t i = 0; i < m; ++i) {
             const uint64_t span = (uint64_t)high - (uint64_t)low + 1;
-            const uint32_t t = (uint32_t)((span * c1[i]) >> 16);
-            const uint32_t one = sym_h[base + i] ? 0xFFFFFFFFu : 0u;
+            const uint32_t t = (uint32_t)((span * (uint32_t)c1[i]) >> 16);
+            const uint32_t one = sym[i] ? 0xFFFFFFFFu : 0u;
             const uint32_t lt = low + t;
             high = (high & one) | ((lt - 1u) & ~one);
             low = (lt & one) | (low & ~one);
@@ -193,12 +193,60 @@
             }
         }
     }
-    ++pending;
-    const uint32_t last = low < 0x40000000u ? 0u : 1u;
-    sink.put_bits(last, 1);
-    sink.put_run(last ^ 1u, pending);
-    sink.finish();
-    return sink.len <= cap ? sink.len : (int64_t)LINR_ENOSPC;
+    inline int64_t finish() {
+        ++pending;
+        const uint32_t last = low < 0x40000000u ? 0u : 1u;
+        sink.put_bits(last, 1);
+        sink.put_run(last ^ 1u, pending);
+        sink.finish();
+        return sink.len <= sink.cap ? sink.len : (int64_t)LINR_ENOSPC;
+    }
+};
+
+template <class F>
+int encode_batch(int32_t n_streams, int32_t n_threads, int64_t* out_len, F one) {
+    if (n_threads < 1) n_threads = 1;
+    if (n_threads > n_streams) n_threads = n_streams;
+    std::atomic<int> next(0);
+    std::atomic<int> err(0);
+    auto work = [&]() {
+        for (;;) {
+            const int i = next.fetch_add(1);
+            if (i >= n_streams) return;
+            const int64_t r = one(i);
+            out_len[i] = r;
+            if (r < 0) err.store((int)r);
+        }
+    };
+    if (n_threads <= 1) {
+        work();
+    } else {
+        std::vector<std::thread> pool;
+        for (int t = 0; t < n_threads; ++t) pool.emplace_back(work);
+        for (auto& t : pool) t.join();
+    }
+    return err.load();
+}
+
+}
+
+extern "C" int64_t linr_ac_encode_binary(const float* prob_h, const uint8_t* sym_h, int64_t n, uint8_t* out_h, int64_t cap) {
+    if (n < 0 || cap < 0 || (n > 0 && (!prob_h || !sym_h)) || (cap > 0 && !out_h)) return LINR_EINVAL;
+    BinaryEncoder enc(out_h, cap);
+    uint32_t c1[AC_CHUNK];
+    for (int64_t base = 0; base < n; base += AC_CHUNK) {
+        const int m = (int)(n - base < AC_CHUNK ? n - base : AC_CHUNK);
+        c1_block(prob_h + base, m, c1);
+        enc.run(c1, sym_h + base, m);
+    }
+    return enc.finish();
+}
+
+extern "C" int64_t linr_ac_encode_binary_c1(const uint16_t* c1_h, const uint8_t* sym_h, int64_t n, uint8_t* out_h, int64_t cap) {
+    if (n < 0 || cap < 0 || (n > 0 && (!c1_h || !sym_h)) || (cap > 0 && !out_h)) return LINR_EINVAL;
+    BinaryEncoder enc(out_h, cap);
+    enc.run(c1_h, sym_h, n);
+    return enc.finish();
 }
 
 namespace {
@@ -309,25 +357,14 @@
                                            int32_t n_streams, uint8_t* const* out_h, const int64_t* cap, int64_t* out_len,
                                            int32_t n_threads) {
     if (n_streams < 0 || (n_streams > 0 && (!prob_h || !sym_h || !n || !out_h || !cap || !out_len))) return LINR_EINVAL;
-    if (n_threads < 1) n_threads = 1;
-    if (n_threads > n_streams) n_threads = n_streams;
-    std::atomic<int> next(0);
-    std::atomic<int> err(0);
-    auto work = [&]() {
-        for (;;) {
-            const int i = next.fetch_add(1);
-            if (i >= n_streams) return;
-            const int64_t r = linr_ac_encode_binary(prob_h[i], sym_h[i], n[i], out_h[i], cap[i]);
-            out_len[i] = r;
-            if (r < 0) err.store((int)r);
-        }
-    };
-    if (n_threads <= 1) {
-        work();
-    } else {
-        std::vector<std::thread> pool;
-        for (int t = 0; t < n_threads; ++t) pool.emplace_back(work);
-        for (auto& t : pool) t.join();
-    }
-    return err.load();
-}
+    return encode_batch(n_streams, n_threads, out_len,
+                        [&](int i) { return linr_ac_encode_binary(prob_h[i], sym_h[i], n[i], out_h[i], cap[i]); });
+}
+
+extern "C" int linr_ac_encode_binary_c1_batch(const uint16_t* const* c1_h, const uint8_t* const* sym_h, const int64_t* n,
+                                              int32_t n_streams, uint8_t* const* out_h, const int64_t* cap, int64_t* out_len,
+                                              int32_t n_threads) {
+    if (n_streams < 0 || (n_streams > 0 && (!c1_h || !sym_h || !n || !out_h || !cap || !out_len))) return LINR_EINVAL;
+    return encode_batch(n_streams, n_threads, out_len,
+                        [&](int i) { return linr_ac_encode_binary_c1(c1_h[i], sym_h[i], n[i], out_h[i], cap[i]); });
+}
diff --git a/linr_pcgc_amd/csrc/common.h b/linr_pcgc_amd/csrc/common.h
--- a/linr_pcgc_amd/csrc/common.h
+++ b/linr_pcgc_amd/csrc/common.h
@@ -79,6 +79,13 @@
     float* p_out;
     double* partial;
 };
+struct CodecOut { uint16_t* c1; uint8_t* sym; };
+__device__ __forceinline__ uint32_t linr_c1_of(float p) {
+#pragma clang fp contract(off)
+    const float d = 1.0f - p;
+    const float scaled = d * 65534.0f;
+    return (uint32_t)(__float2int_rn(scaled) + 1) & 0xFFFFu;
+}
 struct HeadBwdGroup {
     const float *c, *p, *target, *w1, *b1, *w2;
     float* gc;
@@ -141,6 +148,8 @@
 __attribute__((visibility("hidden")))
 int linr_cconv_head_launch(LinrCmap m, const HeadFwdGroup* g, int ng, int target_ld, hipStream_t s);
 __attribute__((visibility("hidden")))
+int linr_cconv_head_codec_launch(LinrCmap m, const HeadFwdGroup* g, int ng, int target_ld, CodecOut co, hipStream_t s);
+__attribute__((visibility("hidden")))
 int linr_head_bwd_launch(const HeadBwdGroup* g, int ng, int target_ld, float gscale, int64_t n, float* big, int64_t block_stride,
                          int nblocks, int* rows_written, hipStream_t s);
 __attribute__((visibility("hidden")))
diff --git a/linr_pcgc_amd/csrc/fused.hip b/linr_pcgc_amd/csrc/fused.hip
--- a/linr_pcgc_amd/csrc/fused.hip
+++ b/linr_pcgc_amd/csrc/fused.hip
@@ -51,7 +51,8 @@
                                                            const float* __restrict__ bias, const float* __restrict__ res,
                                                            int res_ld, const float* __restrict__ act, int act_ld,
                                                            float* __restrict__ out, int out_ld, unsigned flags,
-                                                           HeadArgs hd = HeadArgs(), PwArgs pw = PwArgs(), Grp gp = Grp()) {
+                                                           HeadArgs hd = HeadArgs(), PwArgs pw = PwArgs(), Grp gp = Grp(),
+                                                           CodecOut co = CodecOut()) {
     static_assert(GOUT == 4 || GOUT == 8, "output channels must fill 1 or 2 MFMA blocks");
     {
         const int gi = blockIdx.y;
@@ -59,7 +60,7 @@
         if (bias) bias += gp.b[gi];
         if (res) res += gp.res[gi];
         if (act) act += gp.act[gi];
-        if constexpr (EPI == 1) {
+        if constexpr (EPI == 1 || EPI == 5) {
             hd.w1 += gp.e0[gi]; hd.b1 += gp.e1[gi]; hd.w2 += gp.e2[gi]; hd.b2 += gp.e3[gi];
             if (hd.target) hd.target += gp.e4[gi];
             hd.p_out += gp.e5[gi];
@@ -68,6 +69,7 @@
         if constexpr (EPI == 2) { pw.w += gp.e0[gi]; pw.b += gp.e1[gi]; }
         if constexpr (EPI == 3) { pw.w += gp.e0[gi]; pw.aux += gp.e1[gi]; pw.aux_out += gp.e2[gi]; }
         if constexpr (EPI == 4) { pw.w += gp.e0[gi]; pw.aux += gp.e1[gi]; }
+        if constexpr (EPI == 5) { co.c1 += (int64_t)gi * n; co.sym += (int64_t)gi * n; }
     }
     constexpr int HB = GOUT / 4;
     constexpr int KPV = 16 / HB;
@@ -121,7 +123,7 @@
     for (int h = 0; h < GOUT / 4; ++h)
 #pragma unroll
         for (int j = 0; j < 4; ++j) a[4 * h + j] = acc[h][j];
-    if constexpr (EPI == 1) {
+    if constexpr (EPI == 1 || EPI == 5) {
         float* op = out + row * out_ld;
         if (live) {
             *reinterpret_cast<float4*>(op) = make_float4(a[0], a[1], a[2], a[3]);
@@ -136,7 +138,14 @@
             z = fmaf(fmaxf(hj, 0.0f), hd.w2[j], z);
         }
         const float p = 1.0f / (1.0f + expf(-z));
-        if (live) hd.p_out[row] = p;
+        if constexpr (EPI == 5) {
+            if (live) {
+                co.c1[row] = (uint16_t)linr_c1_of(p);
+                co.sym[row] = (uint8_t)hd.target[row * hd.target_ld];
+            }
+        } else {
+            if (live) hd.p_out[row] = p;
+        }
         if (hd.partial != nullptr) {
             __shared__ double sred[LINR_CONV_BLOCK / 64];
             double nats = 0.0;
@@ -272,6 +281,22 @@
     HeadArgs hd = {g[0].w1, g[0].b1, g[0].w2, g[0].b2, g[0].target, target_ld, g[0].p_out, g[0].partial};
     cconv_mfma_k<8, 8, false, 8, 1><<<dim3(linr_grid(m.n, LINR_CONV_BLOCK), ng), LINR_CONV_BLOCK, 0, s>>>(
         g[0].in, 8, m.lo, m.mask, m.ld, m.n, g[0].W, g[0].bias, nullptr, 0, nullptr, 0, g[0].c_out, 8, 0, hd, PwArgs(), gp);
+    return linr_launch_rc();
+}
+
+int linr_cconv_head_codec_launch(LinrCmap m, const HeadFwdGroup* g, int ng, int target_ld, CodecOut co, hipStream_t s) {
+    if (ng < 1 || ng > LINR_MAXG || !co.c1 || !co.sym) return LINR_EINVAL;
+    if (m.n == 0) return 0;
+    Grp gp = Grp();
+    for (int i = 0; i < ng; ++i) {
+        if (!g[i].target || !g[i].partial) return LINR_EINVAL;
+        gp.in[i] = g[i].in - g[0].in; gp.w[i] = g[i].W - g[0].W; gp.b[i] = g[i].bias - g[0].bias; gp.out[i] = g[i].c_out - g[0].c_out;
+        gp.e0[i] = g[i].w1 - g[0].w1; gp.e1[i] = g[i].b1 - g[0].b1; gp.e2[i] = g[i].w2 - g[0].w2; gp.e3[i] = g[i].b2 - g[0].b2;
+        gp.e4[i] = g[i].target - g[0].target; gp.e6[i] = g[i].partial - g[0].partial;
+    }
+    HeadArgs hd = {g[0].w1, g[0].b1, g[0].w2, g[0].b2, g[0].target, target_ld, nullptr, g[0].partial};
+    cconv_mfma_k<8, 8, false, 8, 5><<<dim3(linr_grid(m.n, LINR_CONV_BLOCK), ng), LINR_CONV_BLOCK, 0, s>>>(
+        g[0].in, 8, m.lo, m.mask, m.ld, m.n, g[0].W, g[0].bias, nullptr, 0, nullptr, 0, g[0].c_out, 8, 0, hd, PwArgs(), gp, co);
     return linr_launch_rc();
 }
 
diff --git a/linr_pcgc_amd/csrc/net.hip b/linr_pcgc_amd/csrc/net.hip
--- a/linr_pcgc_amd/csrc/net.hip
+++ b/linr_pcgc_amd/csrc/net.hip
@@ -658,7 +658,7 @@
     return 0;
 }
 
-static int forward_batched(Ctx& c, float* probs, double* bits_acc) {
+static int forward_batched(Ctx& c, float* probs, double* bits_acc, const CodecOut* codec = nullptr) {
     Arena& a = c.A;
     const float* P = c.P;
     const Layout& L = c.L;
@@ -696,7 +696,8 @@
         HeadFwdGroup g[8];
         for (int k = 0; k < 8; ++k) g[k] = head_fwd_group(c, k, bits_acc != nullptr);
         ProfScope ps(c.s, PK_HEAD_FWD, 8);
-        TRY(linr_cconv_head_launch(m, g, 8, 8, c.s));
+        if (codec) TRY(linr_cconv_head_codec_launch(m, g, 8, 8, *codec, c.s));
+        else TRY(linr_cconv_head_launch(m, g, 8, 8, c.s));
     }
     if (bits_acc) {
         ProfScope ps(c.s, PK_MISC, 0);
@@ -708,13 +709,8 @@
     return linr_launch_rc();
 }
 
-extern "C" int linr_net_forward(const linr_frame* f, const float* params, float* arena, size_t arena_bytes,
-                                int32_t stage_begin, int32_t stage_end, float* probs, double* bits_acc, void* stream) {
-    Ctx c;
-    TRY(check_frame(f, params, arena, arena_bytes, c));
-    if (stage_begin < 0 || stage_end > 8 || stage_begin >= stage_end) return LINR_EINVAL;
-    c.s = (hipStream_t)stream;
-    if (c.R == 0) return 0;
+static int forward_stages(Ctx& c, int stage_begin, int stage_end, float* probs, double* bits_acc, const CodecOut* codec = nullptr) {
+    const linr_frame* f = c.f;
     Arena& a = c.A;
     const float* P = c.P;
     if (!(f->flags & LINR_FRAME_OCC_PADDED))
@@ -737,7 +733,8 @@
             TRY(block_fwd(c, c.L.block_in, a.X0, 8, 0, nullptr));
         }
     }
-    if (all_stages) return forward_batched(c, probs, bits_acc);
+    if (all_stages) return forward_batched(c, probs, bits_acc, codec);
+    if (codec) return LINR_EINVAL;
     const int64_t nblk = linr_grid(c.R, LINR_BLOCK);
     for (int k = stage_begin; k < stage_end; ++k) {
         if (k > 0) TRY(block_fwd(c, c.L.outter[k - 1], a.OCC, 8, k, a.O[0]));
@@ -751,6 +748,53 @@
         TRY(linr_bits_finish_launch((const double*)a.slab + (int64_t)stage_begin * nblk, (int)((stage_end - stage_begin) * nblk),
                                     bits_acc, c.s));
     return linr_launch_rc();
+}
+
+extern "C" int linr_net_forward(const linr_frame* f, const float* params, float* arena, size_t arena_bytes,
+                                int32_t stage_begin, int32_t stage_end, float* probs, double* bits_acc, void* stream) {
+    Ctx c;
+    TRY(check_frame(f, params, arena, arena_bytes, c));
+    if (stage_begin < 0 || stage_end > 8 || stage_begin >= stage_end) return LINR_EINVAL;
+    c.s = (hipStream_t)stream;
+    if (c.R == 0) return 0;
+    return forward_stages(c, stage_begin, stage_end, probs, bits_acc);
+}
+
+__global__ __launch_bounds__(LINR_BLOCK) void c1_from_probs_k(const float* __restrict__ p, int64_t n, uint16_t* __restrict__ c1) {
+    const int64_t i = (int64_t)blockIdx.x * LINR_BLOCK + threadIdx.x;
+    if (i < n) c1[i] = (uint16_t)linr_c1_of(p[i]);
+}
+
+extern "C" int linr_c1_from_probs(const float* p_dev, int64_t n, uint16_t* c1_dev, void* stream) {
+    if (n < 0 || n > (int64_t)0x7FFFFFFF * LINR_BLOCK) return LINR_EINVAL;
+    if (n == 0) return 0;
+    if (!p_dev || !c1_dev) return LINR_EINVAL;
+    c1_from_probs_k<<<linr_grid(n, LINR_BLOCK), LINR_BLOCK, 0, (hipStream_t)stream>>>(p_dev, n, c1_dev);
+    return linr_launch_rc();
+}
+
+extern "C" int linr_net_encode_frame(const linr_frame* f, const float* params, float* arena, size_t arena_bytes, uint16_t* c1_dev,
+                                     uint8_t* sym_dev, uint16_t* c1_pinned, uint8_t* sym_pinned, double* bits_acc, void* stream,
+                                     void* copy_stream, void* copied_event) {
+    Ctx c;
+    TRY(check_frame(f, params, arena, arena_bytes, c));
+    if (!bits_acc || !copied_event) return LINR_EINVAL;
+    if (c.R > 0 && (!c1_dev || !sym_dev || !c1_pinned || !sym_pinned)) return LINR_EINVAL;
+    c.s = (hipStream_t)stream;
+    const hipStream_t cs = (hipStream_t)copy_stream;
+    if (c.R > 0) {
+        const CodecOut co = {c1_dev, sym_dev};
+        TRY(forward_stages(c, 0, 8, nullptr, bits_acc, &co));
+        hipEvent_t done;
+        TRY(linr_hip_rc(hipEventCreateWithFlags(&done, hipEventDisableTiming)));
+        int rc = linr_hip_rc(hipEventRecord(done, c.s));
+        if (!rc) rc = linr_hip_rc(hipStreamWaitEvent(cs, done, 0));
+        (void)hipEventDestroy(done);
+        TRY(rc);
+        TRY(linr_hip_rc(hipMemcpyAsync(c1_pinned, c1_dev, (size_t)c.R * 8 * sizeof(uint16_t), hipMemcpyDeviceToHost, cs)));
+        TRY(linr_hip_rc(hipMemcpyAsync(sym_pinned, sym_dev, (size_t)c.R * 8, hipMemcpyDeviceToHost, cs)));
+    }
+    return linr_hip_rc(hipEventRecord((hipEvent_t)copied_event, cs));
 }
 
 extern "C" int linr_sce_fwd(const float* params, const linr_frame* f, float* mix, float* hid, float* x0, void* stream) {
diff --git a/linr_pcgc_amd/engine.py b/linr_pcgc_amd/engine.py
--- a/linr_pcgc_amd/engine.py
+++ b/linr_pcgc_amd/engine.py
@@ -161,6 +161,13 @@
                                            0 if bits is None else bits.data_ptr(), _stream()), 'linr_net_forward_bf16')
 
 
+def net_encode_frame(frame, flat_params, c1_dev, sym_dev, c1_pinned, sym_pinned, bits, copy_stream, copied_event, arena=None):
+    arena = frame.arena if arena is None else arena
+    check(_lib.lib().linr_net_encode_frame(frame.cref(), flat_params.data_ptr(), arena.data_ptr(), arena.numel(), c1_dev.data_ptr(),
+                                           sym_dev.data_ptr(), c1_pinned.data_ptr(), sym_pinned.data_ptr(), bits.data_ptr(), _stream(),
+                                           copy_stream.cuda_stream, copied_event.cuda_event), 'linr_net_encode_frame')
+
+
 def net_decode_stages(frame, flat_params, streams_per_scale, probs, p_pinned, s_pinned, s_dev, qcodes=None, qrange=None):
     n = frame.n_scales
     bufs = [np.frombuffer(streams_per_scale[i][k], dtype=np.uint8) for i in range(n) for k in range(8)]
diff --git a/linr_pcgc_amd/model_core.py b/linr_pcgc_amd/model_core.py
--- a/linr_pcgc_amd/model_core.py
+++ b/linr_pcgc_amd/model_core.py
@@ -222,6 +222,15 @@
         self._stage_forward(frame, 0, 8, probs, bits, self._precision(precision))
         return probs, bits
 
+    def has_frame_encoder(self, precision=None):
+        return self._wide is None and self._precision(precision) == 'f32'
+
+    @torch.no_grad()
+    def encode_frame_codes(self, frame, c1_dev, sym_dev, c1_pinned, sym_pinned, bits, copy_stream, copied_event):
+        if not self.has_frame_encoder():
+            raise _lib.LinrError('encode_frame_codes needs the fp32 executor at hidden_channel_conv 8')
+        engine.net_encode_frame(frame, self._flat, c1_dev, sym_dev, c1_pinned, sym_pinned, bits, copy_stream, copied_event)
+
     @torch.no_grad()
     def codec(self, inargs):
         st1 = time.time()
@@ -330,9 +339,17 @@
 
 
 def encode_streams(probs, symbols, n_threads=8):
+    return _encode_streams('linr_ac_encode_binary_batch', np.float32, probs, symbols, n_threads)
+
+
+def encode_streams_c1(c1, symbols, n_threads=8):
+    return _encode_streams('linr_ac_encode_binary_c1_batch', np.uint16, c1, symbols, n_threads)
+
+
+def _encode_streams(entry, dtype, probs, symbols, n_threads):
     import ctypes
     n = len(probs)
-    probs = [np.ascontiguousarray(p, dtype=np.float32).reshape(-1) for p in probs]
+    probs = [np.ascontiguousarray(p, dtype=dtype).reshape(-1) for p in probs]
     symbols = [np.ascontiguousarray(s, dtype=np.uint8).reshape(-1) for s in symbols]
     outs = [np.empty(2 * p.size + 64, dtype=np.uint8) for p in probs]
     arr_p = (ctypes.c_void_p * n)(*[p.ctypes.data for p in probs])
@@ -341,8 +358,7 @@
     arr_n = (ctypes.c_int64 * n)(*[p.size for p in probs])
     arr_c = (ctypes.c_int64 * n)(*[o.size for o in outs])
     arr_l = (ctypes.c_int64 * n)()
-    _lib.check(_lib.lib().linr_ac_encode_binary_batch(arr_p, arr_s, arr_n, n, arr_o, arr_c, arr_l, n_threads),
-               'linr_ac_encode_binary_batch')
+    _lib.check(getattr(_lib.lib(), entry)(arr_p, arr_s, arr_n, n, arr_o, arr_c, arr_l, n_threads), entry)
     return [outs[i][:arr_l[i]].tobytes() for i in range(n)]
 
 
diff --git a/linr_pcgc_amd/ops.py b/linr_pcgc_amd/ops.py
--- a/linr_pcgc_amd/ops.py
+++ b/linr_pcgc_amd/ops.py
@@ -136,6 +136,12 @@
     check(_lib.lib().linr_bce_bits_bwd(p.data_ptr(), target.data_ptr(), target.stride(0), n, gscale, gz.data_ptr(),
                                        _stream()), 'linr_bce_bits_bwd')
     return gz
+
+
+def c1_from_probs(p):
+    c1 = torch.empty(p.shape, dtype=torch.int16, device=p.device)
+    check(_lib.lib().linr_c1_from_probs(p.data_ptr(), p.numel(), c1.data_ptr(), _stream()), 'linr_c1_from_probs')
+    return c1
 
 
 def adam_step(params, grads, exp_avg, exp_avg_sq, step, lr, beta1=0.9, beta2=0.999, eps=1e-8, weight_decay=1e-4):
```
